# MaartenGr/PolyFuzz

Measured on NVIDIA H100. Metric: scored string pairs/sec (TF-IDF char-trigram top-10, top-k index bit-exact vs CPU ref), higher is better.
Workload: dtype f64

## Files before the change

include/pfz.h:

```cpp
#ifndef PFZ_H
#define PFZ_H
#include <stdint.h>
#ifdef __cplusplus
extern "C" {
#endif

#define PFZ_ABI_VERSION 1

#define PFZ_FLAG_CLEAN         1
#define PFZ_FLAG_REMOVE_SPACE  2

#define PFZ_METRIC_LEV       0
#define PFZ_METRIC_INDEL     1
#define PFZ_METRIC_NORM_LEV  2
#define PFZ_METRIC_RATIO     3
#define PFZ_METRIC_JARO      4
#define PFZ_METRIC_JARO_WINKLER 5
#define PFZ_METRIC_OSA       6
#define PFZ_METRIC_NORM_OSA  7
#define PFZ_METRIC_DL        8
#define PFZ_METRIC_NORM_DL   9

int         pfz_abi_version(void);
const char *pfz_last_error(void);
int64_t     pfz_launch_count(void);
int pfz_device_info(int32_t *sm_count, int32_t *smem_per_block_optin, int32_t *cc_major, int32_t *cc_minor);

int pfz_int_alu_probe(int32_t iters, uint32_t *scratch, int64_t *lane_ops_host, void *stream);


int pfz_alphabet_mark(const uint32_t *blob, int64_t n_chars, uint8_t *present, void *stream);

#define PFZ_WARP_ROW_SLOTS 256
#define PFZ_MAX_ROW_SLOTS  8192
int pfz_ngram_rows(const uint32_t *blob, const int64_t *offsets, int32_t n_rows,
                   int32_t ngram_lo, int32_t ngram_hi, int32_t flags,
                   const uint32_t *sym_table, uint32_t base,
                   const int64_t *occ_ptr, const int32_t *long_rows, int32_t n_long,
                   uint64_t *codes, int32_t *tf, int32_t *row_cnt, void *stream);

int pfz_df_dense(const uint64_t *codes, const int64_t *occ_ptr, const int32_t *row_cnt, int32_t n_rows,
                 int32_t *df_dense, void *stream);
int pfz_vocab_compact_dense(const int32_t *df_dense, int64_t code_space, uint64_t *vocab_keys, int32_t *df,
                            int32_t *rank_dense, int32_t *n_vocab_dev, void *ws, void *stream);

int pfz_gather_codes(const uint64_t *codes, const int64_t *occ_ptr, const int32_t *row_cnt, int32_t n_rows,
                     uint64_t *keys, int64_t *cursor_dev, void *stream);
int pfz_sort_u64(uint64_t *keys, int64_t n_pow2, void *stream);
int pfz_vocab_from_sorted(const uint64_t *sorted_keys, int64_t n_keys_cap, const int64_t *n_keys_dev,
                          uint64_t *vocab_keys, int32_t *df, int32_t *n_vocab_dev, void *ws, void *stream);

int pfz_idf_lookup(const int32_t *df, const int32_t *n_vocab_dev, int64_t cap, const double *table, int64_t n_table, double *idf, void *stream);

int pfz_tfidf_emit(const uint64_t *codes, const int32_t *tf, const int64_t *occ_ptr, const int32_t *row_cnt,
                   int32_t n_rows, const int32_t *rank_dense, const uint64_t *vocab_keys, int32_t n_vocab,
                   const double *idf, int32_t *indptr, int32_t *indices, double *data, void *ws, void *stream);

int64_t pfz_scan_ws_bytes(int64_t n);


#define PFZ_INDEX_BANK_ORDER   1
#define PFZ_INDEX_BANK_ORDER32 2
int pfz_index_build(const int32_t *indptr, const int32_t *indices, const double *data, int32_t n_rows,
                    int32_t n_vocab, int32_t tile, int32_t n_tiles, int32_t flags,
                    int32_t *seg, uint16_t *post_idx, double *post_val, float *post_val32 ,
                    float *term_maxw ,
                    void *ws, void *stream);

#define PFZ_K2_LIST  1
#define PFZ_K2_DENSE 2
#define PFZ_K2_DENSE32 3
int pfz_spcos_topk(const int32_t *a_indptr, const int32_t *a_indices, const double *a_data, int32_t n_from,
                   const int32_t *seg, const uint16_t *post_idx, const double *post_val,
                   const float *post_val32, const int32_t *b_indptr, const int32_t *b_indices, const double *b_data,
                   const float *term_maxw,
                   int32_t n_vocab, int32_t tile, int32_t n_tiles, int32_t n_to,
                   int32_t k, double min_similarity, int32_t self_match,
                   int64_t from_index_base, int64_t to_index_base, int32_t n_splits,
                   const double *excl_val, const int32_t *excl_idx,
                   int32_t *top_idx, double *top_val, int32_t *row_counter, int32_t variant, void *stream);

int64_t pfz_spcos_block_ws_bytes(int32_t n_from, int64_t nnz_cap_from, int32_t n_vocab, int32_t n_splits);
int64_t pfz_spcos_block_gcnt_offset(int32_t n_from, int64_t nnz_cap_from, int32_t n_vocab, int32_t n_splits);
int pfz_index_pack_q26(const uint16_t *post_idx, const double *post_val, const int32_t *nnz_dev, void *post_pk, void *stream);
int pfz_index_pack_q15(const uint16_t *post_idx, const double *post_val, const int32_t *nnz_dev, int32_t tile, void *post_pk, void *stream);
int pfz_spcos_topk_block(const int32_t *a_indptr, const int32_t *a_indices, const double *a_data, int32_t n_from, int64_t nnz_cap_from,
                         const int32_t *seg, const void *post_pk, const int32_t *b_indptr, const int32_t *b_indices, const double *b_data,
                         int32_t n_vocab, int32_t tile, int32_t n_tiles, int32_t n_to, int32_t k, double min_similarity, int32_t self_match,
                         int64_t from_index_base, int64_t to_index_base, int32_t n_splits, int32_t block_rows, int32_t acc_bits,
                         int32_t *top_idx, double *top_val, int32_t *err_flag_dev, void *ws, void *stream);

int pfz_spcos_topk_hash(const int32_t *a_indptr, const int32_t *a_indices, const double *a_data, int32_t n_from, const int32_t *seg,
                        const void *post_pk, const int32_t *b_indptr, const int32_t *b_indices, const double *b_data, int32_t tile,
                        int32_t n_tiles, int32_t n_to, int32_t k, double min_similarity, int32_t self_match, int64_t from_index_base,
                        int64_t to_index_base, int32_t n_splits, int32_t table_slots, const double *excl_val, const int32_t *excl_idx,
                        int32_t *top_idx, double *top_val, int32_t *row_counter, int32_t *err_flag_dev, void *stream);

int pfz_topk_merge(const int32_t *idx, const double *val, int32_t n_lists, int32_t n_from, int32_t k_in,
                   int32_t k_out, int32_t *out_idx, double *out_val, void *stream);


int pfz_lev_pack(const uint32_t *to_blob, const int64_t *to_offsets, const int32_t *order, int32_t n_to,
                 const uint8_t *sym_table, const int64_t *grp_word_off, uint32_t *packed, int32_t *slen, void *stream);

int pfz_lev_argbest(const uint32_t *from_blob, const int64_t *from_offsets, int32_t n_from, const int32_t *from_ids,
                    int32_t n_ids, int32_t n_words, const uint8_t *sym_table, const uint32_t *packed,
                    const int64_t *grp_word_off, const int32_t *slen, const int32_t *sorig, int32_t n_to,
                    int32_t metric, double score_cutoff, int32_t exclude_self, int64_t self_shift, int32_t n_splits,
                    int32_t *part_idx, double *part_score, int32_t *part_dist, int32_t *matrix, int64_t matrix_ld,
                    int32_t *counter, void *stream);
int pfz_lev_merge(const int32_t *part_idx, const double *part_score, const int32_t *part_dist, int32_t n_splits,
                  int32_t n_from, int32_t *best_idx, double *best_score, int32_t *best_dist, void *stream);

int pfz_lev_topk(const uint32_t *from_blob, const int64_t *from_offsets, int32_t n_from, const int32_t *from_ids,
                 int32_t n_ids, int32_t n_words, const uint8_t *sym_table, const uint32_t *packed,
                 const int64_t *grp_word_off, const int32_t *slen, const int32_t *sorig, int32_t n_to,
                 int32_t metric, double score_cutoff, int32_t exclude_self, int64_t self_shift, int32_t n_splits,
                 int32_t k, int32_t *part_idx, double *part_score, int32_t *counter, void *stream);

int pfz_dl_argbest(const uint32_t *from_blob, const int64_t *from_offsets, int32_t n_from, const int32_t *from_ids,
                   int32_t n_ids, int32_t n_words, const uint8_t *sym_table, const uint32_t *packed,
                   const int64_t *grp_word_off, const int32_t *slen, const int32_t *sorig, int32_t n_to,
                   int32_t metric, double score_cutoff, int32_t exclude_self, int64_t self_shift, int32_t n_splits,
                   int32_t *part_idx, double *part_score, int32_t *part_dist, int32_t *matrix, int64_t matrix_ld,
                   const double *gate, int32_t *counter, void *stream);
int pfz_dl_topk(const uint32_t *from_blob, const int64_t *from_offsets, int32_t n_from, const int32_t *from_ids,
                int32_t n_ids, int32_t n_words, const uint8_t *sym_table, const uint32_t *packed,
                const int64_t *grp_word_off, const int32_t *slen, const int32_t *sorig, int32_t n_to,
                int32_t metric, double score_cutoff, int32_t exclude_self, int64_t self_shift, int32_t n_splits,
                int32_t k, int32_t *part_idx, double *part_score, const double *gate, int32_t *counter, void *stream);

int pfz_fuzz_argbest(const void *const *ptrs, int32_t n_ptrs, int32_t n_from, int32_t n_ids, int32_t n_words, int32_t n_to,
                     int32_t scorer, double score_cutoff, int32_t exclude_self, int64_t self_shift, int32_t n_splits, void *stream);

int pfz_tok_side(const int32_t *blob, const int64_t *offsets, int32_t n, int64_t n_chars, int32_t *n_all, int32_t *vocab_blob,
                 int64_t *vocab_off, int32_t *tok_ptr, int32_t *tok_ids, int64_t *s_off, int32_t *s_blob, int64_t *u_off,
                 int32_t *u_blob, int64_t *counts_host, void *stream);
int pfz_tok_union(const int32_t *a_blob, const int64_t *a_off, int32_t n_a, const int32_t *b_blob, const int64_t *b_off, int32_t n_b,
                  int32_t *map_a, int32_t *map_b, int32_t *u_blob, int64_t *u_off, int32_t *n_u, void *stream);
int pfz_tok_remap(const int32_t *tok_ptr, const int32_t *ids_in, int32_t n, const int32_t *map, int32_t *ids_out, uint64_t *sig,
                  void *stream);

int pfz_fuzz_topk(const void *const *ptrs, int32_t n_ptrs, int32_t n_from, int32_t n_ids, int32_t n_words, int32_t n_to,
                  int32_t scorer, double score_cutoff, int32_t exclude_self, int64_t self_shift, int32_t n_splits, int32_t k,
                  void *stream);


int pfz_rows_to_bf16(const void *x, int32_t is_f64, int64_t ld, int32_t n_rows, int32_t d, int32_t d_pad,
                     int32_t normalize, void *out_bf16, void *stream);

int pfz_dense_cos_topk(const void *x_bf16, const void *y_bf16, int32_t n_from, int32_t n_to, int32_t d, int32_t k,
                       double min_similarity, int32_t self_match, int64_t from_index_base, int64_t to_index_base,
                       int32_t n_splits, int32_t *top_idx, double *top_val, void *stream);

int pfz_rows_prep_exact(const void *x, int32_t is_f64, int64_t ld, int32_t n_rows, int32_t d, int32_t d_pad,
                        double *out_f64, void *out_f16, double *norm16, double *err16, double *maxima, void *stream);

int pfz_dense_cos_topk_f16(const void *x_f16, const void *y_f16, int32_t n_from, int32_t n_to, int32_t d, int32_t k,
                           double min_similarity, int32_t self_match, int64_t from_index_base, int64_t to_index_base,
                           int32_t n_splits, int32_t *top_idx, double *top_val, void *stream);

int pfz_dense_exact_rescore(const double *x_f64, const double *y_f64, int32_t n_from, int32_t n_to, int32_t d_pad, int32_t k,
                            int32_t k_cand, const int32_t *cand_idx, const double *cand_val, const double *x_norm16,
                            const double *x_err16, const double *y_maxima, double min_similarity, int32_t self_match,
                            int64_t from_index_base, int64_t to_index_base, int32_t *top_idx, double *top_val,
                            int32_t *fb_rows, int32_t *fb_count, void *stream);

int64_t pfz_dense_exact_fallback_ws_bytes(int32_t n_from, int32_t n_to, int32_t k);
int pfz_dense_exact_fallback(const double *x_f64, const double *y_f64, int32_t n_from, int32_t n_to, int32_t d_pad, int32_t k,
                             double min_similarity, int32_t self_match, int64_t from_index_base, int64_t to_index_base,
                             const int32_t *fb_rows, const int32_t *fb_count, int32_t *top_idx, double *top_val, void *ws,
                             void *stream);

int pfz_dense_topn_bound(const int32_t *list_idx, const double *list_val, int32_t n_lists, int32_t n_from, int32_t k_list,
                         int32_t k, int32_t exact, const double *x_norm16, const double *x_err16, const double *y_maxima,
                         int32_t d_pad, double min_similarity, float *row_thr, void *stream);

int pfz_dense_cos_cand(const void *x_bf16, const void *y_bf16, int32_t n_from, int32_t n_to, int32_t d, double min_similarity,
                       const float *row_thr, int64_t to_index_base, int32_t n_splits, int32_t cap, int32_t *cand_idx,
                       double *cand_val, int32_t *cand_count, void *stream);
int pfz_dense_cos_cand_f16(const void *x_f16, const void *y_f16, int32_t n_from, int32_t n_to, int32_t d, double min_similarity,
                           const float *row_thr, int64_t to_index_base, int32_t n_splits, int32_t cap, int32_t *cand_idx,
                           double *cand_val, int32_t *cand_count, void *stream);

int pfz_dense_topn_exact_rescore(const double *x_f64, const double *y_f64, int32_t n_rows, int32_t d_pad, const int32_t *row_map,
                                 int64_t to_index_base, int32_t cap, const int32_t *cand_idx, double *cand_val,
                                 const int32_t *cand_count, void *stream);

int pfz_dense_topn_select(const int32_t *cand_idx, const double *cand_val, const int32_t *cand_count, int32_t n_rows, int32_t cap,
                          int32_t k, double min_similarity, int32_t self_match, int64_t from_index_base, const int32_t *row_map,
                          int32_t *top_idx, double *top_val, void *stream);

int pfz_frame_tail_count(const int32_t *top_idx, const double *top_val, int32_t n, int32_t k, const int64_t *to_offsets, double *sims,
                         int32_t *lens_pos, uint32_t *bitmap, void *ws, void *stream);
int pfz_frame_tail_copy(const int32_t *top_idx, int32_t n, int32_t k, const int32_t *to_blob, const int64_t *to_offsets, const int32_t *pos,
                        int64_t *offsets, uint8_t *data, void *stream);

#ifdef __cplusplus
}
#endif
#endif
```

polyfuzz_b200/_lib.py:

```python
import ctypes
import os

_HERE = os.path.dirname(os.path.abspath(__file__))
_LIB_PATH = os.path.join(_HERE, "libpfz.so")
_lib = None

c_i32, c_i64, c_u32, c_f64, c_vp = ctypes.c_int32, ctypes.c_int64, ctypes.c_uint32, ctypes.c_double, ctypes.c_void_p

_PROTOS = {
    "pfz_abi_version": [],
    "pfz_last_error": [],
    "pfz_launch_count": [],
    "pfz_device_info": [c_vp, c_vp, c_vp, c_vp],
    "pfz_scan_ws_bytes": [c_i64],
    "pfz_int_alu_probe": [c_i32, c_vp, c_vp, c_vp],
    "pfz_alphabet_mark": [c_vp, c_i64, c_vp, c_vp],
    "pfz_ngram_rows": [c_vp, c_vp, c_i32, c_i32, c_i32, c_i32, c_vp, c_u32, c_vp, c_vp, c_i32, c_vp, c_vp, c_vp, c_vp],
    "pfz_df_dense": [c_vp, c_vp, c_vp, c_i32, c_vp, c_vp],
    "pfz_vocab_compact_dense": [c_vp, c_i64, c_vp, c_vp, c_vp, c_vp, c_vp, c_vp],
    "pfz_gather_codes": [c_vp, c_vp, c_vp, c_i32, c_vp, c_vp, c_vp],
    "pfz_sort_u64": [c_vp, c_i64, c_vp],
    "pfz_vocab_from_sorted": [c_vp, c_i64, c_vp, c_vp, c_vp, c_vp, c_vp, c_vp],
    "pfz_idf_lookup": [c_vp, c_vp, c_i64, c_vp, c_i64, c_vp, c_vp],
    "pfz_tfidf_emit": [c_vp, c_vp, c_vp, c_vp, c_i32, c_vp, c_vp, c_i32, c_vp, c_vp, c_vp, c_vp, c_vp, c_vp],
    "pfz_index_build": [c_vp, c_vp, c_vp, c_i32, c_i32, c_i32, c_i32, c_i32, c_vp, c_vp, c_vp, c_vp, c_vp, c_vp, c_vp],
    "pfz_spcos_topk": [c_vp, c_vp, c_vp, c_i32, c_vp, c_vp, c_vp, c_vp, c_vp, c_vp, c_vp, c_vp, c_i32, c_i32, c_i32, c_i32, c_i32, c_f64, c_i32,
                       c_i64, c_i64, c_i32, c_vp, c_vp, c_vp, c_vp, c_vp, c_i32, c_vp],
    "pfz_topk_merge": [c_vp, c_vp, c_i32, c_i32, c_i32, c_i32, c_vp, c_vp, c_vp],
    "pfz_spcos_topk_hash": [c_vp, c_vp, c_vp, c_i32, c_vp, c_vp, c_vp, c_vp, c_vp, c_i32, c_i32, c_i32, c_i32, c_f64, c_i32, c_i64, c_i64, c_i32,
                            c_i32, c_vp, c_vp, c_vp, c_vp, c_vp, c_vp, c_vp],
    "pfz_spcos_block_ws_bytes": [c_i32, c_i64, c_i32, c_i32],
    "pfz_spcos_block_gcnt_offset": [c_i32, c_i64, c_i32, c_i32],
    "pfz_index_pack_q26": [c_vp, c_vp, c_vp, c_vp, c_vp],
    "pfz_index_pack_q15": [c_vp, c_vp, c_vp, c_i32, c_vp, c_vp],
    "pfz_spcos_topk_block": [c_vp, c_vp, c_vp, c_i32, c_i64, c_vp, c_vp, c_vp, c_vp, c_vp, c_i32, c_i32, c_i32, c_i32, c_i32, c_f64, c_i32,
                             c_i64, c_i64, c_i32, c_i32, c_i32, c_vp, c_vp, c_vp, c_vp, c_vp],
    "pfz_lev_pack": [c_vp, c_vp, c_vp, c_i32, c_vp, c_vp, c_vp, c_vp, c_vp],
    "pfz_lev_argbest": [c_vp, c_vp, c_i32, c_vp, c_i32, c_i32, c_vp, c_vp, c_vp, c_vp, c_vp, c_i32, c_i32, c_f64, c_i32, c_i64,
                        c_i32, c_vp, c_vp, c_vp, c_vp, c_i64, c_vp, c_vp],
    "pfz_lev_merge": [c_vp, c_vp, c_vp, c_i32, c_i32, c_vp, c_vp, c_vp, c_vp],
    "pfz_fuzz_argbest": [c_vp, c_i32, c_i32, c_i32, c_i32, c_i32, c_i32, c_f64, c_i32, c_i64, c_i32, c_vp],
    "pfz_lev_topk": [c_vp, c_vp, c_i32, c_vp, c_i32, c_i32, c_vp, c_vp, c_vp, c_vp, c_vp, c_i32, c_i32, c_f64, c_i32, c_i64,
                     c_i32, c_i32, c_vp, c_vp, c_vp, c_vp],
    "pfz_dl_argbest": [c_vp, c_vp, c_i32, c_vp, c_i32, c_i32, c_vp, c_vp, c_vp, c_vp, c_vp, c_i32, c_i32, c_f64, c_i32, c_i64,
                       c_i32, c_vp, c_vp, c_vp, c_vp, c_i64, c_vp, c_vp, c_vp],
    "pfz_dl_topk": [c_vp, c_vp, c_i32, c_vp, c_i32, c_i32, c_vp, c_vp, c_vp, c_vp, c_vp, c_i32, c_i32, c_f64, c_i32, c_i64,
                    c_i32, c_i32, c_vp, c_vp, c_vp, c_vp, c_vp],
    "pfz_fuzz_topk":[c_vp, c_i32, c_i32, c_i32, c_i32, c_i32, c_i32, c_f64, c_i32, c_i64, c_i32, c_i32, c_vp],
    "pfz_tok_side": [c_vp, c_vp, c_i32, c_i64, c_vp, c_vp, c_vp, c_vp, c_vp, c_vp, c_vp, c_vp, c_vp, c_vp, c_vp],
    "pfz_tok_union": [c_vp, c_vp, c_i32, c_vp, c_vp, c_i32, c_vp, c_vp, c_vp, c_vp, c_vp, c_vp],
    "pfz_tok_remap": [c_vp, c_vp, c_i32, c_vp, c_vp, c_vp, c_vp],
    "pfz_frame_tail_count": [c_vp, c_vp, c_i32, c_i32, c_vp, c_vp, c_vp, c_vp, c_vp, c_vp],
    "pfz_frame_tail_copy": [c_vp, c_i32, c_i32, c_vp, c_vp, c_vp, c_vp, c_vp, c_vp],
    "pfz_rows_to_bf16": [c_vp, c_i32, c_i64, c_i32, c_i32, c_i32, c_i32, c_vp, c_vp],
    "pfz_dense_cos_topk": [c_vp, c_vp, c_i32, c_i32, c_i32, c_i32, c_f64, c_i32, c_i64, c_i64, c_i32, c_vp, c_vp, c_vp],
    "pfz_rows_prep_exact": [c_vp, c_i32, c_i64, c_i32, c_i32, c_i32, c_vp, c_vp, c_vp, c_vp, c_vp, c_vp],
    "pfz_dense_cos_topk_f16": [c_vp, c_vp, c_i32, c_i32, c_i32, c_i32, c_f64, c_i32, c_i64, c_i64, c_i32, c_vp, c_vp, c_vp],
    "pfz_dense_exact_rescore": [c_vp, c_vp, c_i32, c_i32, c_i32, c_i32, c_i32, c_vp, c_vp, c_vp, c_vp, c_vp, c_f64, c_i32, c_i64, c_i64,
                                c_vp, c_vp, c_vp, c_vp, c_vp],
    "pfz_dense_exact_fallback_ws_bytes": [c_i32, c_i32, c_i32],
    "pfz_dense_exact_fallback": [c_vp, c_vp, c_i32, c_i32, c_i32, c_i32, c_f64, c_i32, c_i64, c_i64, c_vp, c_vp, c_vp, c_vp, c_vp, c_vp],
    "pfz_dense_topn_bound": [c_vp, c_vp, c_i32, c_i32, c_i32, c_i32, c_i32, c_vp, c_vp, c_vp, c_i32, c_f64, c_vp, c_vp],
    "pfz_dense_cos_cand": [c_vp, c_vp, c_i32, c_i32, c_i32, c_f64, c_vp, c_i64, c_i32, c_i32, c_vp, c_vp, c_vp, c_vp],
    "pfz_dense_cos_cand_f16": [c_vp, c_vp, c_i32, c_i32, c_i32, c_f64, c_vp, c_i64, c_i32, c_i32, c_vp, c_vp, c_vp, c_vp],
    "pfz_dense_topn_exact_rescore": [c_vp, c_vp, c_i32, c_i32, c_vp, c_i64, c_i32, c_vp, c_vp, c_vp, c_vp],
    "pfz_dense_topn_select": [c_vp, c_vp, c_vp, c_i32, c_i32, c_i32, c_f64, c_i32, c_i64, c_vp, c_vp, c_vp, c_vp],
}
_RESTYPES = {"pfz_last_error": ctypes.c_char_p, "pfz_scan_ws_bytes": c_i64, "pfz_launch_count": c_i64, "pfz_spcos_block_ws_bytes": c_i64,
             "pfz_spcos_block_gcnt_offset": c_i64,
             "pfz_dense_exact_fallback_ws_bytes": c_i64}


def exported_names():
    return list(_PROTOS)


def lib_path():
    return _LIB_PATH


def load():
    global _lib
    if _lib is not None:
        return _lib
    if not os.path.exists(_LIB_PATH):
        raise RuntimeError(f"{_LIB_PATH} not found: build it with `python -m polyfuzz_b200.build` "
                           "(polyfuzz_b200 has no CPU fallback)")
    lib = ctypes.CDLL(_LIB_PATH)
    for name, args in _PROTOS.items():
        fn = getattr(lib, name)
        fn.argtypes = args
        fn.restype = _RESTYPES.get(name, ctypes.c_int)
    _lib = lib
    return lib


def call(name, *args):
    lib = load()
    rc = getattr(lib, name)(*args)
    if rc != 0:
        raise RuntimeError(f"{name} failed: {lib.pfz_last_error().decode(errors='replace')}")


def launch_count():
    return int(load().pfz_launch_count())
```

polyfuzz_b200/csrc/pfz_core.cu:

```cuda
#include <stdarg.h>
#include "pfz_common.cuh"

namespace pfz {
static thread_local char g_err[1024] = "";
unsigned long long g_launches = 0;
void set_error(const char *fmt, ...) {
    va_list ap; va_start(ap, fmt);
    vsnprintf(g_err, sizeof(g_err), fmt, ap);
    va_end(ap);
}

constexpr int SCAN_THREADS = 512;
constexpr int SCAN_ITEMS = 8;
constexpr int SCAN_TILE = SCAN_THREADS * SCAN_ITEMS;

__global__ void __launch_bounds__(SCAN_THREADS) scan_tile_kernel(const int32_t *__restrict__ in, int32_t *__restrict__ out,
                                                               int64_t n, int32_t *__restrict__ sums) {
    __shared__ int32_t warp_tot[SCAN_THREADS / 32];
    const int64_t base = (int64_t)blockIdx.x * SCAN_TILE + (int64_t)threadIdx.x * SCAN_ITEMS;
    int32_t v[SCAN_ITEMS];
    int32_t tsum = 0;
#pragma unroll
    for (int i = 0; i < SCAN_ITEMS; ++i) {
        v[i] = (base + i < n) ? in[base + i] : 0;
        tsum += v[i];
    }
    int32_t incl = warp_incl_scan(tsum);
    const int lane = threadIdx.x & 31, w = threadIdx.x >> 5;
    if (lane == 31) warp_tot[w] = incl;
    __syncthreads();
    if (w == 0) {
        int32_t t = (lane < SCAN_THREADS / 32) ? warp_tot[lane] : 0;
        int32_t ti = warp_incl_scan(t);
        if (lane < SCAN_THREADS / 32) warp_tot[lane] = ti - t;
        if (lane == 31 && sums) sums[blockIdx.x] = ti;
    }
    __syncthreads();
    int32_t run = warp_tot[w] + incl - tsum;
#pragma unroll
    for (int i = 0; i < SCAN_ITEMS; ++i) {
        if (base + i < n) out[base + i] = run;
        run += v[i];
    }
}

__global__ void __launch_bounds__(SCAN_THREADS) scan_add_kernel(int32_t *__restrict__ out, int64_t n,
                                                              const int32_t *__restrict__ offs) {
    const int32_t add = offs[blockIdx.x];
    const int64_t base = (int64_t)blockIdx.x * SCAN_TILE + (int64_t)threadIdx.x * SCAN_ITEMS;
#pragma unroll
    for (int i = 0; i < SCAN_ITEMS; ++i)
        if (base + i < n) out[base + i] += add;
}

static int64_t n_tiles_of(int64_t n) { return (n + SCAN_TILE - 1) / SCAN_TILE; }

int scan_exclusive_i32(const int32_t *in, int32_t *out, int64_t n, void *ws, cudaStream_t st) {
    if (n <= 0) return 0;
    const int64_t nt = n_tiles_of(n);
    if (nt == 1) {
        scan_tile_kernel<<<1, SCAN_THREADS, 0, st>>>(in, out, n, nullptr);
        PFZ_LAUNCH_OK();
        return 0;
    }
    int32_t *sums = reinterpret_cast<int32_t *>(ws);
    char *next_ws = reinterpret_cast<char *>(ws) + ((nt * 4 + 255) / 256) * 256;
    scan_tile_kernel<<<(unsigned)nt, SCAN_THREADS, 0, st>>>(in, out, n, sums);
    PFZ_LAUNCH_OK();
    if (scan_exclusive_i32(sums, sums, nt, next_ws, st)) return 1;
    scan_add_kernel<<<(unsigned)nt, SCAN_THREADS, 0, st>>>(out, n, sums);
    PFZ_LAUNCH_OK();
    return 0;
}

__global__ void __launch_bounds__(256) int_alu_probe_kernel(uint32_t *__restrict__ out, int iters, uint32_t seed) {
    uint32_t a[8];
    const uint32_t b = seed ^ (threadIdx.x * 2654435761u), c = seed * 3u + blockIdx.x;
#pragma unroll
    for (int i = 0; i < 8; ++i) a[i] = b + i * 977u;
    for (int it = 0; it < iters; ++it) {
#pragma unroll
        for (int u = 0; u < 4; ++u) {
#pragma unroll
            for (int i = 0; i < 8; ++i) asm volatile("lop3.b32 %0, %0, %1, %2, 0x96;" : "+r"(a[i]) : "r"(b), "r"(c));
#pragma unroll
            for (int i = 0; i < 8; ++i) asm volatile("add.u32 %0, %0, %1;" : "+r"(a[i]) : "r"(c));
        }
    }
    uint32_t x = 0;
#pragma unroll
    for (int i = 0; i < 8; ++i) x ^= a[i];
    out[(size_t)blockIdx.x * blockDim.x + threadIdx.x] = x;
}
}

extern "C" {

int pfz_int_alu_probe(int32_t iters, uint32_t *scratch, int64_t *lane_ops_host, void *stream) {
    int dev = 0, sms = 0;
    PFZ_CUDA_OK(cudaGetDevice(&dev));
    PFZ_CUDA_OK(cudaDeviceGetAttribute(&sms, cudaDevAttrMultiProcessorCount, dev));
    const int blocks = sms * 8;
    pfz::int_alu_probe_kernel<<<blocks, 256, 0, pfz::as_stream(stream)>>>(scratch, iters, 12345u);
    PFZ_LAUNCH_OK();
    if (lane_ops_host) *lane_ops_host = (int64_t)blocks * 256 * (int64_t)iters * 64;
    return 0;
}

int pfz_abi_version(void) { return PFZ_ABI_VERSION; }
const char *pfz_last_error(void) { return pfz::g_err; }
int64_t pfz_launch_count(void) { return (int64_t)__atomic_load_n(&pfz::g_launches, __ATOMIC_RELAXED); }

int64_t pfz_scan_ws_bytes(int64_t n) {
    int64_t total = 256;
    while (n > pfz::SCAN_TILE) {
        n = pfz::n_tiles_of(n);
        total += ((n * 4 + 255) / 256) * 256;
    }
    return total;
}

int pfz_device_info(int32_t *sm_count, int32_t *smem_optin, int32_t *cc_major, int32_t *cc_minor) {
    int dev = 0;
    PFZ_CUDA_OK(cudaGetDevice(&dev));
    int v = 0;
    PFZ_CUDA_OK(cudaDeviceGetAttribute(&v, cudaDevAttrMultiProcessorCount, dev)); *sm_count = v;
    PFZ_CUDA_OK(cudaDeviceGetAttribute(&v, cudaDevAttrMaxSharedMemoryPerBlockOptin, dev)); *smem_optin = v;
    PFZ_CUDA_OK(cudaDeviceGetAttribute(&v, cudaDevAttrComputeCapabilityMajor, dev)); *cc_major = v;
    PFZ_CUDA_OK(cudaDeviceGetAttribute(&v, cudaDevAttrComputeCapabilityMinor, dev)); *cc_minor = v;
    return 0;
}
}
```

polyfuzz_b200/csrc/pfz_spcos.cu:

```cuda
#include <stdlib.h>
#include "pfz_common.cuh"

namespace pfz {

__global__ void index_count_kernel(const int32_t *__restrict__ indptr, const int32_t *__restrict__ indices, int n_rows, int tile, int n_tiles,
                                   int32_t *__restrict__ cnt) {
    const int lane = lane_id();
    const int gw = (blockIdx.x * blockDim.x + threadIdx.x) >> 5, nw = (gridDim.x * blockDim.x) >> 5;
    for (int r = gw; r < n_rows; r += nw) {
        const int tau = r / tile;
        for (int p = indptr[r] + lane; p < indptr[r + 1]; p += 32)
            atomicAdd(&cnt[(int64_t)indices[p] * n_tiles + tau], 1);
    }
}

__global__ void index_fill_kernel(const int32_t *__restrict__ indptr, const int32_t *__restrict__ indices, const double *__restrict__ data,
                                  int n_rows, int tile, int n_tiles, const int32_t *__restrict__ seg, int32_t *__restrict__ cur,
                                  uint16_t *__restrict__ post_idx, double *__restrict__ post_val, int *__restrict__ term_maxw_bits) {
    const int lane = lane_id();
    const int gw = (blockIdx.x * blockDim.x + threadIdx.x) >> 5, nw = (gridDim.x * blockDim.x) >> 5;
    for (int r = gw; r < n_rows; r += nw) {
        const int tau = r / tile;
        for (int p = indptr[r] + lane; p < indptr[r + 1]; p += 32) {
            const int64_t c = (int64_t)indices[p] * n_tiles + tau;
            const int pos = seg[c] + atomicAdd(&cur[c], 1);
            post_idx[pos] = (uint16_t)(r - tau * tile);
            post_val[pos] = data[p];
            if (term_maxw_bits) atomicMax(&term_maxw_bits[indices[p]], __float_as_int(__double2float_ru(data[p])));
        }
    }
}

constexpr int BANK_ORDER_MAX = 512;
template <int MOD>
__global__ void __launch_bounds__(128) index_bank_order_kernel(const int32_t *__restrict__ seg, int64_t ncell, uint16_t *__restrict__ post_idx,
                                                               double *__restrict__ post_val) {
    __shared__ uint16_t s_idx[4][BANK_ORDER_MAX];
    __shared__ uint16_t s_rank[4][BANK_ORDER_MAX];
    __shared__ double s_val[4][BANK_ORDER_MAX];
    __shared__ int s_cnt[4][MOD];
    const int lane = lane_id(), w = threadIdx.x >> 5;
    const int64_t gw = ((int64_t)blockIdx.x * blockDim.x + threadIdx.x) >> 5, nw = ((int64_t)gridDim.x * blockDim.x) >> 5;
    for (int64_t c0 = gw * 32; c0 < ncell; c0 += nw * 32) {
        int s = 0, len = 0;
        if (c0 + lane < ncell) { s = seg[c0 + lane]; len = seg[c0 + lane + 1] - s; }
        unsigned todo = __ballot_sync(FULL, len > MOD && len <= BANK_ORDER_MAX);
        while (todo) {
            const int src = __ffs(todo) - 1; todo &= todo - 1;
            const int cs = __shfl_sync(FULL, s, src), cl = __shfl_sync(FULL, len, src);
            if (lane < MOD) s_cnt[w][lane] = 0;
            __syncwarp();
            for (int q = lane; q < cl; q += 32) {
                const uint16_t j = post_idx[cs + q];
                s_idx[w][q] = j; s_val[w][q] = post_val[cs + q];
                s_rank[w][q] = (uint16_t)atomicAdd(&s_cnt[w][j & (MOD - 1)], 1);
            }
            __syncwarp();
            int cnt[MOD];
#pragma unroll
            for (int r = 0; r < MOD; ++r) cnt[r] = s_cnt[w][r];
            for (int q = lane; q < cl; q += 32) {
                const int r = s_idx[w][q] & (MOD - 1), i = s_rank[w][q];
                int pos = 0;
#pragma unroll
                for (int r2 = 0; r2 < MOD; ++r2) pos += min(cnt[r2], i) + ((r2 < r && cnt[r2] > i) ? 1 : 0);
                post_idx[cs + pos] = s_idx[w][q];
                post_val[cs + pos] = s_val[w][q];
            }
            __syncwarp();
        }
    }
}

__global__ void to_f32_kernel(const double *__restrict__ x, int64_t n_minus, const int32_t *__restrict__ n_ptr, float *__restrict__ y) {
    const int64_t n = n_ptr ? (int64_t)*n_ptr : n_minus;
    for (int64_t i = (int64_t)blockIdx.x * blockDim.x + threadIdx.x; i < n; i += (int64_t)gridDim.x * blockDim.x) y[i] = (float)x[i];
}

__device__ __forceinline__ bool key_before(double sa, int ia, double sb, int ib) {
    return (sa > sb) || (sa == sb && ia < ib);
}

struct SpcosParams {
    const int32_t *a_indptr; const int32_t *a_indices; const double *a_data; int n_from;
    const int32_t *seg; const uint16_t *post_idx; const double *post_val;
    const float *post_val32; const int32_t *b_indptr; const int32_t *b_indices; const double *b_data;
    const float *term_maxw; float prune_alpha;
    int n_vocab, tile, n_tiles, n_to;
    int k; double min_sim; int self_match; int64_t from_base, to_base;
    int n_splits; const double *excl_val; const int32_t *excl_idx;
    int32_t *top_idx; double *top_val; int32_t *row_counter;
};

template <int WARPS>
__global__ void __launch_bounds__(WARPS * 32) spcos_list_kernel(const SpcosParams P) {
    extern __shared__ __align__(16) unsigned char dyn[];
    const int lane = lane_id();
    const int w = threadIdx.x >> 5;
    const unsigned lt = (1u << lane) - 1u;
    double *acc = reinterpret_cast<double *>(dyn) + (size_t)w * P.tile;
    uint16_t *touched = reinterpret_cast<uint16_t *>(dyn + (size_t)WARPS * P.tile * 8) + (size_t)w * P.tile;
    for (int q = lane; q < P.tile; q += 32) acc[q] = 0.0;
    __syncwarp();

    const int split = blockIdx.y;
    const int tiles_per = (P.n_tiles + P.n_splits - 1) / P.n_splits;
    const int tau_lo = split * tiles_per;
    const int tau_hi = min(P.n_tiles, tau_lo + tiles_per);
    int32_t *counter = P.row_counter + split;

    for (;;) {
        int i = 0;
        if (lane == 0) i = atomicAdd(counter, 1);
        i = __shfl_sync(FULL, i, 0);
        if (i >= P.n_from) break;

        const int a0 = P.a_indptr[i];
        const int m = P.a_indptr[i + 1] - a0;
        double tv = P.min_sim; int ti = -1;
        double kv = P.min_sim; int ki = -1;
        double xv = 0.0; int xi = -1; bool has_x = false;
        if (P.excl_val) { xv = P.excl_val[i]; xi = P.excl_idx[i]; has_x = xi >= 0; }
        const int64_t self_j = P.from_base + i - P.to_base;

        for (int tau = tau_lo; tau < tau_hi; ++tau) {
            int ntouched = 0;
            for (int tb = 0; tb < m; tb += 32) {
                const int kk = tb + lane;
                int s = 0, len = 0; double v = 0.0;
                if (kk < m) {
                    const int t = P.a_indices[a0 + kk];
                    v = P.a_data[a0 + kk];
                    const int64_t c = (int64_t)t * P.n_tiles + tau;
                    s = P.seg[c];
                    len = P.seg[c + 1] - s;
                }
                unsigned live = __ballot_sync(FULL, len > 0);
                while (live) {
                    const int src = __ffs(live) - 1; live &= live - 1;
                    const int ss = __shfl_sync(FULL, s, src);
                    const int sl = __shfl_sync(FULL, len, src);
                    const double sv = shfl_d(v, src);
                    for (int c0 = 0; c0 < sl; c0 += 32) {
                        const int q = c0 + lane;
                        bool first = false; int jl = 0;
                        if (q < sl) {
                            jl = P.post_idx[ss + q];
                            const double prod = __dmul_rn(sv, P.post_val[ss + q]);
                            const double old = acc[jl];
                            acc[jl] = __dadd_rn(old, prod);
                            first = (old == 0.0);
                        }
                        const unsigned fm = __ballot_sync(FULL, first);
                        if (first) touched[ntouched + __popc(fm & lt)] = (uint16_t)jl;
                        ntouched += __popc(fm);
                    }
                    __syncwarp();
                }
            }
            for (int c0 = 0; c0 < ntouched; c0 += 32) {
                const int q = c0 + lane;
                double sc = 0.0; int j = -1; bool cand = false;
                if (q < ntouched) {
                    const int jl = touched[q];
                    sc = acc[jl];
                    acc[jl] = 0.0;
                    const int jloc = tau * P.tile + jl;
                    j = (int)(P.to_base + jloc);
                    cand = key_before(sc, j, kv, ki);
                    if (P.self_match && (int64_t)jloc == self_j) cand = false;
                    if (has_x && !key_before(xv, xi, sc, j)) cand = false;
                }
                unsigned cm = __ballot_sync(FULL, cand);
                while (cm) {
                    const int src = __ffs(cm) - 1; cm &= cm - 1;
                    const double cs = shfl_d(sc, src);
                    const int cj = __shfl_sync(FULL, j, src);
                    if (!key_before(cs, cj, kv, ki)) continue;
                    const bool stays = (lane < P.k) && key_before(tv, ti, cs, cj);
                    const int pos = __popc(__ballot_sync(FULL, stays));
                    const double uv = __shfl_up_sync(FULL, tv, 1);
                    const int ui = __shfl_up_sync(FULL, ti, 1);
                    if (lane > pos) { tv = uv; ti = ui; }
                    else if (lane == pos) { tv = cs; ti = cj; }
                    kv = shfl_d(tv, P.k - 1);
                    ki = __shfl_sync(FULL, ti, P.k - 1);
                }
            }
            __syncwarp();
        }
        if (lane < P.k) {
            const size_t o = ((size_t)split * P.n_from + i) * P.k + lane;
            P.top_idx[o] = ti;
            P.top_val[o] = (ti >= 0) ? tv : 0.0;
        }
    }
}


struct __align__(16) WorkItem { int off; int cnt; double v; };

__device__ __forceinline__ unsigned smem_u32(const void *p) { return (unsigned)__cvta_generic_to_shared(p); }
__device__ __forceinline__ void lds_item(unsigned a, unsigned &off, int &cnt, double &v) {
    unsigned lo, hi;
    asm volatile("ld.shared.v4.b32 {%0, %1, %2, %3}, [%4];" : "=r"(off), "=r"(cnt), "=r"(lo), "=r"(hi) : "r"(a) : "memory");
    v = __hiloint2double((int)hi, (int)lo);
}
__device__ __forceinline__ void ldg_posting(const uint16_t *pi, const double *pv, int lane, int cnt, unsigned dummy, unsigned &jl, double &w) {
    asm volatile("{ .reg .pred p; setp.lt.s32 p, %2, %3; mov.u32 %0, %4; mov.f64 %1, 0d0000000000000000;\n\t"
                 "@p ld.global.nc.u16 %0, [%5]; @p ld.global.nc.f64 %1, [%6]; }"
                 : "=&r"(jl), "=&d"(w) : "r"(lane), "r"(cnt), "r"(dummy), "l"(pi), "l"(pv) : "memory");
}
__device__ __forceinline__ void rmw_posting(unsigned acc_s, unsigned flags_s, unsigned row, unsigned dummy, double v, double w, double thr,
                                            unsigned &any) {
    asm volatile("{ .reg .pred p, q, r; .reg .f64 o, n, pr; .reg .b16 one; .reg .u32 a, f;\n\t"
                 "setp.ne.u32 p, %3, %4; mov.f64 o, 0d0000000000000000;\n\t"
                 "shl.b32 a, %3, 3; add.u32 a, a, %1; add.u32 f, %2, %3;\n\t"
                 "@p ld.shared.f64 o, [a];\n\t"
                 "mul.rn.f64 pr, %5, %6; add.rn.f64 n, o, pr;\n\t"
                 "@p st.shared.f64 [a], n;\n\t"
                 "setp.gt.f64 q, o, %7; setp.gt.and.f64 r, n, %7, !q; mov.b16 one, 1;\n\t"
                 "@r st.shared.u8 [f], one; selp.u32 %0, 1, %0, r; }"
                 : "+r"(any) : "r"(acc_s), "r"(flags_s), "r"(row), "r"(dummy), "d"(v), "d"(w), "d"(thr) : "memory");
}
// ... 258 lines not shown
                                    if (lane > pos) lv = up; else if (lane == pos) lv = ca;
                                    kth = __shfl_sync(FULL, lv, K - 1);
                                    a = (lane == src) ? -2.f : a;
                                    cm = __ballot_sync(FULL, a > kth);
                                }
                            }
                        }
                        gate = fmaxf(gate, float_floor(fmax((double)kth - K2_MARGIN - (double)ub_ne, 0.0)));
                    }
                }
                for (int w00 = 0; w00 < T; w00 += 512) {
                  uint4 fb = make_uint4(0u, 0u, 0u, 0u);
                  const int q16 = w00 + lane * 16;
                  if (q16 < T) {
                      fb = *reinterpret_cast<const uint4 *>(flags + q16);
                      if (fb.x | fb.y | fb.z | fb.w) *reinterpret_cast<uint4 *>(flags + q16) = make_uint4(0u, 0u, 0u, 0u);
                  }
                  if (!__any_sync(FULL, (fb.x | fb.y | fb.z | fb.w) != 0u)) continue;
#pragma unroll
                  for (int wsel = 0; wsel < 4; ++wsel) {
                    unsigned bits = wsel == 0 ? fb.x : wsel == 1 ? fb.y : wsel == 2 ? fb.z : fb.w;
                    const int q4 = q16 + wsel * 4;
                    while (__ballot_sync(FULL, bits != 0u)) {
                        if (APPROX) {
                            bool take = false; int jloc = 0;
                            if (bits) {
                                const int b8 = (__ffs(bits) - 1) >> 3; bits &= ~(0xffu << (b8 * 8));
                                const int jl = q4 + b8;
                                jloc = tau * T + jl;
                                take = reinterpret_cast<const float *>(acc)[jl] > gate;
                            }
                            const unsigned tm = __ballot_sync(FULL, take);
                            if (take) cand[ncand + __popc(tm & ((1u << lane) - 1u))] = jloc;
                            ncand += __popc(tm);
                            __syncwarp();
                            if (ncand >= 32) {
                                score_round(32);
                                __syncwarp();
                                const int rest = ncand - 32;
                                int mv = 0;
                                if (lane < rest) mv = cand[32 + lane];
                                __syncwarp();
                                if (lane < rest) cand[lane] = mv;
                                ncand = rest;
                                __syncwarp();
                            }
                            continue;
                        }
                        double sc = 0.0; int j = -1; bool cnd = false;
                        if (bits) {
                            const int b8 = (__ffs(bits) - 1) >> 3; bits &= ~(0xffu << (b8 * 8));
                            const int jl = q4 + b8;
                            const int jloc = tau * T + jl;
                            sc = acc[jl];
                            j = (int)(P.to_base + jloc);
                            cnd = key_before(sc, j, kv, ki);
                            if (P.self_match && (int64_t)jloc == self_j) cnd = false;
                            if (has_x && !key_before(xv, xi, sc, j)) cnd = false;
                        }
                        unsigned cm = __ballot_sync(FULL, cnd);
                        while (cm) {
                            const int src = __ffs(cm) - 1;
                            const double cs = shfl_d(sc, src);
                            const int cjx = __shfl_sync(FULL, j, src);
                            const bool stays = (lane < K) && key_before(tv, ti, cs, cjx);
                            const int pos = __popc(__ballot_sync(FULL, stays));
                            const double uv = __shfl_up_sync(FULL, tv, 1);
                            const int ui = __shfl_up_sync(FULL, ti, 1);
                            if (lane > pos) { tv = uv; ti = ui; }
                            else if (lane == pos) { tv = cs; ti = cjx; }
                            kv = shfl_d(tv, K - 1);
                            ki = __shfl_sync(FULL, ti, K - 1);
                            cnd = cnd && lane != src && key_before(sc, j, kv, ki);
                            cm = __ballot_sync(FULL, cnd);
                        }
                    }
                  }
                }
                thr = (ki >= 0) ? __longlong_as_double(__double_as_longlong(kv) - 1) : fmax(kv, 0.0);
            }
            __syncwarp();
            {
                double2 *a2 = reinterpret_cast<double2 *>(acc);
                const double2 z = make_double2(0.0, 0.0);
                for (int q = lane; q < (T * ES >> 4); q += 32) a2[q] = z;
            }
            __syncwarp();
        }
        if (APPROX && ncand > 0) { __syncwarp(); score_round(ncand); __syncwarp(); }
        if (lane < K) {
            const size_t o = ((size_t)split * P.n_from + i) * K + lane;
            P.top_idx[o] = ti;
            P.top_val[o] = (ti >= 0) ? tv : 0.0;
        }
    }
}

__global__ void __launch_bounds__(256) topk_merge_kernel(const int32_t *__restrict__ idx, const double *__restrict__ val, int n_lists, int n_from,
                                                         int k_in, int k_out, int32_t *__restrict__ out_idx, double *__restrict__ out_val) {
    const int lane = lane_id();
    const int gw = (blockIdx.x * blockDim.x + threadIdx.x) >> 5, nw = (gridDim.x * blockDim.x) >> 5;
    for (int i = gw; i < n_from; i += nw) {
        double tv = 0.0; int ti = -1;
        double kv = 0.0; int ki = -1; bool full = false;
        int filled = 0;
        for (int l = 0; l < n_lists; ++l) {
            const size_t b = ((size_t)l * n_from + i) * k_in;
            for (int c0 = 0; c0 < k_in; c0 += 32) {
                const int q = c0 + lane;
                double sc = 0.0; int j = -1;
                if (q < k_in) { j = idx[b + q]; sc = val[b + q]; }
                unsigned cm = __ballot_sync(FULL, j >= 0);
                while (cm) {
                    const int src = __ffs(cm) - 1; cm &= cm - 1;
                    const double cs = shfl_d(sc, src);
                    const int cj = __shfl_sync(FULL, j, src);
                    if (full && !key_before(cs, cj, kv, ki)) continue;
                    const bool stays = (lane < filled) && key_before(tv, ti, cs, cj);
                    const int pos = __popc(__ballot_sync(FULL, stays));
                    const double uv = __shfl_up_sync(FULL, tv, 1);
                    const int ui = __shfl_up_sync(FULL, ti, 1);
                    if (lane > pos) { tv = uv; ti = ui; }
                    else if (lane == pos) { tv = cs; ti = cj; }
                    if (filled < k_out) ++filled;
                    full = filled == k_out;
                    kv = shfl_d(tv, k_out - 1);
                    ki = __shfl_sync(FULL, ti, k_out - 1);
                }
            }
        }
        if (lane < k_out) {
            const bool ok = lane < filled;
            out_idx[(size_t)i * k_out + lane] = ok ? ti : -1;
            out_val[(size_t)i * k_out + lane] = ok ? tv : 0.0;
        }
    }
}

static int grid_for2(int64_t work_items, int threads, int cap) {
    int64_t g = (work_items + threads - 1) / threads;
    if (g < 1) g = 1;
    if (g > cap) g = cap;
    return (int)g;
}

}

using namespace pfz;

extern "C" {

int pfz_index_build(const int32_t *indptr, const int32_t *indices, const double *data, int32_t n_rows, int32_t n_vocab, int32_t tile,
                    int32_t n_tiles, int32_t flags, int32_t *seg, uint16_t *post_idx, double *post_val, float *post_val32, float *term_maxw,
                    void *ws, void *stream) {
    PFZ_REQUIRE(tile > 0 && tile <= 65536, "pfz_index_build: tile %d out of range (1..65536)", tile);
    PFZ_REQUIRE((int64_t)n_tiles * tile >= n_rows, "pfz_index_build: n_tiles*tile < n_rows");
    const int64_t ncell = (int64_t)n_vocab * n_tiles;
    PFZ_REQUIRE(ncell + 1 < (1ll << 31), "pfz_index_build: n_vocab*n_tiles = %lld too large", (long long)ncell);
    cudaStream_t st = as_stream(stream);
    int32_t *cur = reinterpret_cast<int32_t *>(ws);
    void *sws = reinterpret_cast<char *>(ws) + ((((size_t)ncell + 1) * 4 + 255) / 256) * 256;
    PFZ_CUDA_OK(cudaMemsetAsync(seg, 0, ((size_t)ncell + 1) * 4, st));
    if (n_rows > 0) {
        index_count_kernel<<<grid_for2((int64_t)n_rows * 32, 256, SM_COUNT * 16), 256, 0, st>>>(indptr, indices, n_rows, tile, n_tiles, seg);
        PFZ_LAUNCH_OK();
    }
    if (scan_exclusive_i32(seg, seg, ncell + 1, sws, st)) return 1;
    if (n_rows > 0) {
        PFZ_CUDA_OK(cudaMemsetAsync(cur, 0, ((size_t)ncell + 1) * 4, st));
        if (term_maxw) PFZ_CUDA_OK(cudaMemsetAsync(term_maxw, 0, (size_t)n_vocab * 4, st));
        index_fill_kernel<<<grid_for2((int64_t)n_rows * 32, 256, SM_COUNT * 16), 256, 0, st>>>(indptr, indices, data, n_rows, tile, n_tiles, seg, cur,
                                                                                            post_idx, post_val, reinterpret_cast<int *>(term_maxw));
        PFZ_LAUNCH_OK();
        if (flags & PFZ_INDEX_BANK_ORDER32) {
            index_bank_order_kernel<32><<<grid_for2(ncell, 128, SM_COUNT * 16), 128, 0, st>>>(seg, ncell, post_idx, post_val);
            PFZ_LAUNCH_OK();
        } else if (flags & PFZ_INDEX_BANK_ORDER) {
            index_bank_order_kernel<16><<<grid_for2(ncell, 128, SM_COUNT * 16), 128, 0, st>>>(seg, ncell, post_idx, post_val);
            PFZ_LAUNCH_OK();
        }
        if (post_val32) {
            to_f32_kernel<<<SM_COUNT * 8, 256, 0, st>>>(post_val, 0, seg + ncell, post_val32);
            PFZ_LAUNCH_OK();
        }
    }
    return 0;
}

int pfz_spcos_topk(const int32_t *a_indptr, const int32_t *a_indices, const double *a_data, int32_t n_from, const int32_t *seg,
                   const uint16_t *post_idx, const double *post_val, const float *post_val32, const int32_t *b_indptr,
                   const int32_t *b_indices, const double *b_data, const float *term_maxw, int32_t n_vocab, int32_t tile, int32_t n_tiles, int32_t n_to, int32_t k,
                   double min_similarity, int32_t self_match, int64_t from_index_base, int64_t to_index_base, int32_t n_splits,
                   const double *excl_val, const int32_t *excl_idx, int32_t *top_idx, double *top_val, int32_t *row_counter,
                   int32_t variant, void *stream) {
    PFZ_REQUIRE(k >= 1 && k <= 32, "pfz_spcos_topk: k=%d unsupported (1..32 per call; page with excl_* for more)", k);
    PFZ_REQUIRE(tile > 0 && tile <= 65536 && (tile % 64) == 0, "pfz_spcos_topk: tile %d must be a multiple of 64 in 64..65536", tile);
    PFZ_REQUIRE(n_splits >= 1 && n_splits <= n_tiles, "pfz_spcos_topk: n_splits %d out of range", n_splits);
    PFZ_REQUIRE(variant == PFZ_K2_LIST || variant == PFZ_K2_DENSE || variant == PFZ_K2_DENSE32, "pfz_spcos_topk: unknown variant %d", variant);
    PFZ_REQUIRE(variant != PFZ_K2_DENSE32 || (post_val32 && b_indptr && b_indices && b_data),
                "pfz_spcos_topk: PFZ_K2_DENSE32 needs post_val32 and the to-matrix CSR");
    if (n_from <= 0) return 0;
    cudaStream_t st = as_stream(stream);
    int dev = 0, sms = 0, smem_max = 0;
    PFZ_CUDA_OK(cudaGetDevice(&dev));
    PFZ_CUDA_OK(cudaDeviceGetAttribute(&sms, cudaDevAttrMultiProcessorCount, dev));
    PFZ_CUDA_OK(cudaDeviceGetAttribute(&smem_max, cudaDevAttrMaxSharedMemoryPerBlockOptin, dev));
    PFZ_CUDA_OK(cudaMemsetAsync(row_counter, 0, sizeof(int32_t) * (size_t)n_splits, st));
    const char *env_a = getenv("PFZ_K2_PRUNE_ALPHA");
    const float prune_alpha = env_a ? (float)atof(env_a) : 0.0f;
    SpcosParams P{a_indptr, a_indices, a_data, n_from, seg, post_idx, post_val, post_val32, b_indptr, b_indices, b_data, term_maxw, prune_alpha,
                  n_vocab, tile, n_tiles, n_to, k, min_similarity, self_match,
                  from_index_base, to_index_base, n_splits, excl_val, excl_idx, top_idx, top_val, row_counter};
    auto launch = [&](auto kernel, int warps, size_t smem) -> int {
        PFZ_REQUIRE(smem <= (size_t)smem_max, "pfz_spcos_topk: tile %d needs %zu B shared memory > %d available", tile, smem, smem_max);
        PFZ_CUDA_OK(cudaFuncSetAttribute(kernel, cudaFuncAttributeMaxDynamicSharedMemorySize, (int)smem));
        int occ = 0;
        PFZ_CUDA_OK(cudaOccupancyMaxActiveBlocksPerMultiprocessor(&occ, kernel, warps * 32, smem));
        if (occ < 1) occ = 1;
        int gx = sms * occ;
        const int need = (n_from + warps - 1) / warps;
        if (gx > need) gx = need;
        if (n_splits > 1) { gx = (gx + n_splits - 1) / n_splits; if (gx < 1) gx = 1; }
        kernel<<<dim3(gx, n_splits), warps * 32, smem, st>>>(P);
        PFZ_LAUNCH_OK();
        return 0;
    };
    if (variant == PFZ_K2_LIST) {
        constexpr int WARPS = 8;
        return launch(spcos_list_kernel<WARPS>, WARPS, (size_t)WARPS * tile * 10);
    }
    constexpr int WARPS = 2;
    const int es = variant == PFZ_K2_DENSE32 ? 4 : 8;
    auto arena_of = [&](int D) { return (((size_t)(tile + 4) * es + (size_t)((tile >> 5) + 32 + 2 * D) * sizeof(WorkItem) + (size_t)tile + 16 + 256) + 15) & ~(size_t)15; };
    const char *env_d = getenv("PFZ_K2_DEPTH");
    const int depth = env_d ? atoi(env_d) : 4;
    if (variant == PFZ_K2_DENSE32) {
        if (prune_alpha > 0.f && term_maxw) return launch(spcos_dense_kernel<WARPS, 4, true, true>, WARPS, (size_t)WARPS * arena_of(4));
        if (depth == 8) return launch(spcos_dense_kernel<WARPS, 8, true, false>, WARPS, (size_t)WARPS * arena_of(8));
        if (depth == 6) return launch(spcos_dense_kernel<WARPS, 6, true, false>, WARPS, (size_t)WARPS * arena_of(6));
        if (depth == 3) return launch(spcos_dense_kernel<WARPS, 3, true, false>, WARPS, (size_t)WARPS * arena_of(3));
        if (depth == 2) return launch(spcos_dense_kernel<WARPS, 2, true, false>, WARPS, (size_t)WARPS * arena_of(2));
        return launch(spcos_dense_kernel<WARPS, 4, true, false>, WARPS, (size_t)WARPS * arena_of(4));
    }
    if (depth == 8) return launch(spcos_dense_kernel<WARPS, 8, false, false>, WARPS, (size_t)WARPS * arena_of(8));
    return launch(spcos_dense_kernel<WARPS, 4, false, false>, WARPS, (size_t)WARPS * arena_of(4));
}

int pfz_topk_merge(const int32_t *idx, const double *val, int32_t n_lists, int32_t n_from, int32_t k_in, int32_t k_out, int32_t *out_idx,
                   double *out_val, void *stream) {
    PFZ_REQUIRE(k_out >= 1 && k_out <= 32, "pfz_topk_merge: k_out=%d unsupported (1..32)", k_out);
    PFZ_REQUIRE(n_lists >= 1 && k_in >= 1, "pfz_topk_merge: bad n_lists/k_in");
    if (n_from <= 0) return 0;
    topk_merge_kernel<<<grid_for2((int64_t)n_from * 32, 256, SM_COUNT * 16), 256, 0, as_stream(stream)>>>(idx, val, n_lists, n_from, k_in, k_out, out_idx, out_val);
    PFZ_LAUNCH_OK();
    return 0;
}
}
```

polyfuzz_b200/csrc/pfz_spcos_block.cu:

```cuda
#include <stdlib.h>
#include "pfz_common.cuh"

namespace pfz {

constexpr double K2B_SCALE = 67108864.0;
constexpr unsigned K2B_MARGIN_Q = 672u;
constexpr int RANK_CAP = 16383;

struct __align__(16) BlockDesc { int pos0; int nrows; int base; int nterms; };

__global__ void blk_term_key_kernel(const int32_t *__restrict__ seg, int n_vocab, int n_tiles, uint64_t *__restrict__ keys, int64_t n_pad) {
    for (int64_t t = (int64_t)blockIdx.x * blockDim.x + threadIdx.x; t < n_pad; t += (int64_t)gridDim.x * blockDim.x) {
        uint64_t k = ~0ull;
        if (t < n_vocab) {
            const uint32_t df = (uint32_t)(seg[(t + 1) * n_tiles] - seg[t * n_tiles]);
            k = ((uint64_t)(0xffffffffu - df) << 32) | (uint32_t)t;
        }
        keys[t] = k;
    }
}
__global__ void blk_term_rank_kernel(const uint64_t *__restrict__ keys, int n_vocab, int32_t *__restrict__ rank) {
    for (int i = blockIdx.x * blockDim.x + threadIdx.x; i < n_vocab; i += gridDim.x * blockDim.x)
        rank[(uint32_t)(keys[i] & 0xffffffffu)] = min(i, RANK_CAP);
}
__global__ void blk_row_key_kernel(const int32_t *__restrict__ indptr, const int32_t *__restrict__ indices, const int32_t *__restrict__ rank,
                                   int n_from, uint64_t *__restrict__ keys, int64_t n_pad) {
    for (int64_t r = (int64_t)blockIdx.x * blockDim.x + threadIdx.x; r < n_pad; r += (int64_t)gridDim.x * blockDim.x) {
        uint64_t k = ~0ull;
        if (r < n_from) {
            int r1 = RANK_CAP, r2 = RANK_CAP, r3 = RANK_CAP;
            for (int p = indptr[r]; p < indptr[r + 1]; ++p) {
                const int x = rank[indices[p]];
                if (x < r1) { r3 = r2; r2 = r1; r1 = x; }
                else if (x < r2) { r3 = r2; r2 = x; }
                else if (x < r3) r3 = x;
            }
            k = ((uint64_t)r1 << 50) | ((uint64_t)r2 << 36) | ((uint64_t)r3 << 22) | (uint64_t)r;
        }
        keys[r] = k;
    }
}
__global__ void blk_perm_kernel(const uint64_t *__restrict__ keys, const int32_t *__restrict__ indptr, int n_from, int32_t *__restrict__ perm,
                                int32_t *__restrict__ nnz_perm) {
    for (int p = blockIdx.x * blockDim.x + threadIdx.x; p <= n_from; p += gridDim.x * blockDim.x) {
        if (p == n_from) { nnz_perm[p] = 0; continue; }
        const int r = (int)(keys[p] & 0x3fffffull);
        perm[p] = r;
        nnz_perm[p] = indptr[r + 1] - indptr[r];
    }
}

template <int BF>
__global__ void __launch_bounds__(128) blk_table_kernel(const int32_t *__restrict__ indptr, const int32_t *__restrict__ indices,
                                                        const double *__restrict__ data, int n_from, const int32_t *__restrict__ perm,
                                                        const int32_t *__restrict__ pos_ptr, int row_stride_bytes, int32_t *__restrict__ blk_terms,
                                                        int32_t *__restrict__ blk_fvdesc, uint2 *__restrict__ blk_fv, BlockDesc *__restrict__ descs,
                                                        int n_groups, int32_t *__restrict__ err_flag) {
    constexpr int FV_CAP = BF * 64;
    constexpr int WPB = BF == 16 ? 2 : 4;
    __shared__ uint32_t s_key[WPB][FV_CAP];
    __shared__ uint32_t s_val[WPB][FV_CAP];
    const int lane = lane_id(), w = threadIdx.x >> 5;
    const unsigned lt = (1u << lane) - 1u;
    if (w >= WPB) return;
    uint32_t *keys = s_key[w]; uint32_t *vals = s_val[w];
    for (int g = blockIdx.x * WPB + w; g < n_groups; g += gridDim.x * WPB) {
        const int p0 = g * BF, p1 = min(n_from, p0 + BF);
        const int total = pos_ptr[p1] - pos_ptr[p0];
        const int nsub = total <= FV_CAP ? 1 : 2;
        for (int sub = 0; sub < 2; ++sub) {
            BlockDesc d; d.pos0 = 0; d.nrows = 0; d.base = 0; d.nterms = 0;
            if (sub < nsub) {
                const int q0 = nsub == 1 ? p0 : min(p1, p0 + sub * (BF / 2));
                const int q1 = nsub == 1 ? p1 : min(p1, q0 + BF / 2);
                const int base = pos_ptr[q0];
                const int cnt = pos_ptr[q1] - base;
                if (cnt > FV_CAP) { if (lane == 0) atomicExch(err_flag, 1); }
                else if (q1 > q0) {
                    for (int f = 0; f < q1 - q0; ++f) {
                        const int row = perm[q0 + f];
                        const int a0 = indptr[row], m = indptr[row + 1] - a0, o = pos_ptr[q0 + f] - base;
                        for (int e = lane; e < m; e += 32) {
                            keys[o + e] = ((uint32_t)indices[a0 + e] << 4) | (uint32_t)f;
                            const double x = floor(data[a0 + e] * 4294967296.0);
                            vals[o + e] = x >= 4294967295.0 ? 0xffffffffu : (uint32_t)(unsigned long long)x;
                        }
                    }
                    int P = 1;
                    while (P < cnt) P <<= 1;
                    for (int e = cnt + lane; e < P; e += 32) { keys[e] = 0xffffffffu; vals[e] = 0u; }
                    __syncwarp();
                    for (int k = 2; k <= P; k <<= 1) {
                        for (int j = k >> 1; j > 0; j >>= 1) {
                            for (int t = lane; t < (P >> 1); t += 32) {
                                const int i = ((t & ~(j - 1)) << 1) | (t & (j - 1));
                                const int ix = i | j;
                                const uint32_t a = keys[i], b = keys[ix];
                                const bool up = (i & k) == 0;
                                if ((a > b) == up) { keys[i] = b; keys[ix] = a; const uint32_t va = vals[i]; vals[i] = vals[ix]; vals[ix] = va; }
                            }
                            __syncwarp();
                        }
                    }
                    int nd = 0;
                    for (int e0 = 0; e0 < cnt; e0 += 32) {
                        const int e = e0 + lane;
                        bool head = false; uint32_t term = 0;
                        if (e < cnt) {
                            const uint32_t key = keys[e];
                            term = key >> 4;
                            head = (e == 0) || (keys[e - 1] >> 4) != term;
                            blk_fv[base + e] = make_uint2((key & 15u) * (uint32_t)row_stride_bytes, vals[e]);
                        }
                        const unsigned hm = __ballot_sync(FULL, head);
                        if (head) {
                            int len = 1;
                            while (e + len < cnt && (keys[e + len] >> 4) == term) ++len;
                            const int u = nd + __popc(hm & lt);
                            blk_terms[base + u] = (int32_t)term;
                            blk_fvdesc[base + u] = (e << 5) | len;
                        }
                        nd += __popc(hm);
                    }
                    d.pos0 = q0; d.nrows = q1 - q0; d.base = base; d.nterms = nd;
                    __syncwarp();
                }
            }
            if (lane == 0) descs[2 * g + sub] = d;
        }
    }
}

__global__ void blk_pack_kernel(const uint16_t *__restrict__ post_idx, const double *__restrict__ post_val, const int32_t *__restrict__ nnz_ptr,
                                uint2 *__restrict__ post_pk) {
    const int64_t n = *nnz_ptr;
    for (int64_t i = (int64_t)blockIdx.x * blockDim.x + threadIdx.x; i < n; i += (int64_t)gridDim.x * blockDim.x)
        post_pk[i] = make_uint2((uint32_t)post_idx[i], (uint32_t)__double2ll_rn(post_val[i] * 67108864.0));
}

__global__ void blk_pack15_kernel(const uint16_t *__restrict__ post_idx, const double *__restrict__ post_val, const int32_t *__restrict__ nnz_ptr,
                                  int half_tile, uint2 *__restrict__ post_pk) {
    const int64_t n = *nnz_ptr;
    for (int64_t i = (int64_t)blockIdx.x * blockDim.x + threadIdx.x; i < n; i += (int64_t)gridDim.x * blockDim.x) {
        const uint32_t j = post_idx[i];
        const bool hi = j >= (uint32_t)half_tile;
        const uint32_t w15 = (uint32_t)max(1ll, __double2ll_rn(post_val[i] * 32768.0));
        post_pk[i] = make_uint2(((hi ? j - (uint32_t)half_tile : j) << 2) | ((hi ? 0x3244u : 0x4432u) << 16), w15);
    }
}

struct BlockParams {
    const int32_t *a_indptr; const int32_t *a_indices; const double *a_data; int n_from;
    const int32_t *perm; const BlockDesc *descs; int n_desc;
    const int32_t *blk_terms; const int32_t *blk_fvdesc; const uint2 *blk_fv;
    const int32_t *seg; const uint2 *post_pk;
    const int32_t *b_indptr; const int32_t *b_indices; const double *b_data;
    int tile, n_tiles, n_to, k; double min_sim; int self_match; int64_t from_base, to_base; int n_splits;
    int32_t *top_idx; double *top_val; int32_t *counter;
    int32_t *glist; int32_t *gcnt; int gcap;
};

__device__ __forceinline__ unsigned sm_u32(const void *p) { return (unsigned)__cvta_generic_to_shared(p); }
__device__ __forceinline__ void red_add_u32(unsigned a, unsigned v) {
    asm volatile("red.shared.add.u32 [%0], %1;" :: "r"(a), "r"(v));
}
__device__ __forceinline__ bool blk_key_before(double sa, int ia, double sb, int ib) { return (sa > sb) || (sa == sb && ia < ib); }
__device__ __noinline__ double blk_exact_dot(const int32_t *__restrict__ ai, const double *__restrict__ av, int an,
                                  const int32_t *__restrict__ bi, const double *__restrict__ bv, int bn) {
    double s = 0.0;
    int p = 0;
    for (int c0 = 0; c0 < bn && p < an; c0 += 32) {
        int ci[32]; double cv[32];
        const int nc = min(32, bn - c0);
#pragma unroll 8
        for (int q = 0; q < nc; ++q) { ci[q] = bi[c0 + q]; cv[q] = bv[c0 + q]; }
#pragma unroll 1
        for (int q = 0; q < nc; ++q) {
            const int cb = ci[q];
            while (p < an && ai[p] < cb) ++p;
            if (p < an && ai[p] == cb) { s = __dadd_rn(s, __dmul_rn(av[p], cv[q])); ++p; }
        }
    }
    return s;
}
__device__ __forceinline__ unsigned warp_sort_desc_u32(unsigned x, int lane) {
#pragma unroll
    for (int k = 2; k <= 32; k <<= 1) {
#pragma unroll
        for (int j = k >> 1; j > 0; j >>= 1) {
            const unsigned o = __shfl_xor_sync(FULL, x, j);
            const bool keep_max = ((lane & j) == 0) == ((lane & k) == 0);
            x = keep_max ? max(x, o) : min(x, o);
        }
    }
    return x;
}

#ifndef PFZ_B3_ICAP_PER_ROW
#define PFZ_B3_ICAP_PER_ROW 64
#endif
#ifndef PFZ_B3_MIN_CTAS
#define PFZ_B3_MIN_CTAS(BF) (16 / (BF))
#endif
constexpr int B3_ICAP_PER_ROW = PFZ_B3_ICAP_PER_ROW;
constexpr int B3_QCAP = 128;
#ifndef PFZ_B3_DEPTH
#define PFZ_B3_DEPTH 3
#endif
constexpr int B3_DEPTH = PFZ_B3_DEPTH;

struct __align__(16) B3Item { int off; int cnt; unsigned fva; int nf; };
struct __align__(16) B3Ctx {
    const int32_t *a_indptr; const int32_t *a_indices; const double *a_data;
    const int32_t *b_indptr; const int32_t *b_indices; const double *b_data;
    int64_t to_base; double scale; int K; int T; int TW; int gcap;
    int32_t *glist; int64_t grow0;
};
struct __align__(16) B3Row {
    double tv[32]; int ti[32];
    unsigned av[32];
    int cand[B3_QCAP];
    int row, self_loc, ncand; unsigned thr, akth, MQ, gate; int gcount;
};

__device__ __forceinline__ void blk_exact_rounds(const int32_t *__restrict__ a_indptr, const int32_t *__restrict__ a_indices, const double *__restrict__ a_data,
                                                 const int32_t *__restrict__ b_indptr, const int32_t *__restrict__ b_indices, const double *__restrict__ b_data,
                                                 int64_t to_base, int K, int row, int self_loc, const int *cand, int ncand, double &tv, int &ti, double &kv, int &ki) {
    const int lane = threadIdx.x & 31;
    const int a0 = a_indptr[row], m = a_indptr[row + 1] - a0;
    kv = shfl_d(tv, K - 1); ki = __shfl_sync(FULL, ti, K - 1);
    while (ncand > 0) {
        const int n_round = min(32, ncand), off = ncand - n_round;
        double sc = 0.0; int j = -1; bool cnd = false;
        if (lane < n_round) {
            const int jloc = cand[off + lane];
            const int b0 = b_indptr[jloc];
            sc = blk_exact_dot(a_indices + a0, a_data + a0, m, b_indices + b0, b_data + b0, b_indptr[jloc + 1] - b0);
            j = (int)(to_base + jloc);
            cnd = blk_key_before(sc, j, kv, ki) && jloc != self_loc;
        }
        unsigned cm = __ballot_sync(FULL, cnd);
        while (cm) {
            const int src = __ffs(cm) - 1;
            const double cs = shfl_d(sc, src);
            const int cj = __shfl_sync(FULL, j, src);
            const bool stays = (lane < K) && blk_key_before(tv, ti, cs, cj);
            const int pos = __popc(__ballot_sync(FULL, stays));
            const double uv = __shfl_up_sync(FULL, tv, 1);
            const int ui = __shfl_up_sync(FULL, ti, 1);
            if (lane > pos) { tv = uv; ti = ui; }
            else if (lane == pos) { tv = cs; ti = cj; }
            kv = shfl_d(tv, K - 1);
            ki = __shfl_sync(FULL, ti, K - 1);
            cnd = cnd && lane != src && blk_key_before(sc, j, kv, ki);
            cm = __ballot_sync(FULL, cnd);
        }
        ncand = off;
    }
}
__device__ __noinline__ void blk3_drain(const B3Ctx *cx, B3Row *rs) {
    const int lane = threadIdx.x & 31;
    double tv = rs->tv[lane]; int ti = rs->ti[lane];
    double kv; int ki;
    blk_exact_rounds(cx->a_indptr, cx->a_indices, cx->a_data, cx->b_indptr, cx->b_indices, cx->b_data, cx->to_base, cx->K, rs->row, rs->self_loc,
                     rs->cand, rs->ncand, tv, ti, kv, ki);
    rs->tv[lane] = tv; rs->ti[lane] = ti;
    if (lane == 0) {
        rs->ncand = 0;
        if (ki >= 0) {
            const double y = kv * cx->scale - (double)rs->MQ;
            const unsigned t = y <= 0.0 ? 0u : (unsigned)__double2ll_rd(y);
            if (t > rs->thr) rs->thr = t;
        }
    }
    __syncwarp();
}
__device__ __noinline__ void blk3_flush(const B3Ctx *cx, B3Row *rs) {
    const int lane = threadIdx.x & 31;
    const int ncand = rs->ncand, g = rs->gcount;
    if (g + ncand <= cx->gcap) {
        int32_t *dst = cx->glist + (size_t)(cx->grow0 + rs->row) * cx->gcap + g;
        for (int q = lane; q < ncand; q += 32) dst[q] = rs->cand[q];
        __syncwarp();
        if (lane == 0) { rs->gcount = g + ncand; rs->ncand = 0; }
        __syncwarp();
    } else blk3_drain(cx, rs);
}

template <bool P16>
__device__ __forceinline__ unsigned blk3_wmax(const uint4 &v) {
    if (!P16) return max(max(v.x, v.y), max(v.z, v.w));
    const unsigned m2 = __vmaxu2(__vmaxu2(v.x, v.y), __vmaxu2(v.z, v.w));
    return max(m2 & 0xffffu, m2 >> 16);
}

__device__ __forceinline__ uint4 lds128(unsigned a) {
    uint4 v;
    asm volatile("ld.shared.v4.u32 {%0, %1, %2, %3}, [%4];" : "=r"(v.x), "=r"(v.y), "=r"(v.z), "=r"(v.w) : "r"(a));
    return v;
}
__device__ __forceinline__ void sts128_zero(unsigned a) {
    asm volatile("st.shared.v4.u32 [%0], {%1, %1, %1, %1};" :: "r"(a), "r"(0u));
}
// ... 322 lines not shown
                    const int sb = P.blk_terms[D.base + u] * n_tiles + tau;
                    const unsigned fvd = (unsigned)P.blk_fvdesc[D.base + u];
                    const int s = seg[sb], len = seg[sb + 1] - s;
                    for (int c = 0; c < len; c += 32) {
                        uint2 pk = make_uint2(0u, 0u);
                        if (lane < len - c) pk = __ldg(pk_lane + s + c);
                        blk3_process<P16>(lane, len - c, fv_s + ((fvd >> 5) << 3), (int)(fvd & 31u), pk, acc_s, dump_s);
                    }
                }
            }
            B3_TICK(2);
            __syncthreads();
            B3_TICK(3);
            if (has_row) {
                if (stau == tau) {
                    if (lane == 0) {
                        const int sjl = rs->self_loc - stau * T;
                        if (P16) acc[(size_t)w * RW + (sjl >= TW ? sjl - TW : sjl)] &= (sjl >= TW ? 0x0000ffffu : 0xffff0000u);
                        else acc[(size_t)w * RW + sjl] = 0u;
                    }
                    __syncwarp();
                }
                blk3_scan_row<P16>(cx, rs, acc_s + (unsigned)(w * RW) * 4u, tau * T);
            }
        }
        B3_TICK(4);
        if (has_row) {
            __syncwarp();
            blk3_flush(cx, rs);
            const size_t ro = (size_t)split * P.n_from + rs->row;
            if (lane < P.k) {
                const int ti = rs->ti[lane];
                P.top_idx[ro * P.k + lane] = ti;
                P.top_val[ro * P.k + lane] = (ti >= 0) ? rs->tv[lane] : 0.0;
            }
            if (lane == 0) P.gcnt[ro] = rs->gcount;
        }
        B3_TICK(5);
        __syncthreads();
        B3_TICK(6);
    }
}

struct ExactParams {
    const int32_t *a_indptr; const int32_t *a_indices; const double *a_data;
    const int32_t *b_indptr; const int32_t *b_indices; const double *b_data;
    const int32_t *glist; const int32_t *gcnt; int gcap; int n_from; int n_splits; int n_to; int k; double min_sim; int self_match;
    int64_t from_base, to_base; int32_t *top_idx; double *top_val;
};
constexpr int EX_ROW_CAP = 128;
constexpr int EX_HASH = 2 * EX_ROW_CAP;
__device__ __forceinline__ unsigned ex_slot(int t) { return ((unsigned)t * 0x9E3779B1u) >> 24; }
constexpr int EX_CHUNK = 8;
__global__ void __launch_bounds__(256) blk_exact_kernel(const ExactParams P) {
    static_assert(EX_HASH == 256, "ex_slot() yields 8 bits");
    __shared__ int s_hk[8][EX_HASH];
    __shared__ double s_hv[8][EX_HASH];
    const int lane = threadIdx.x & 31, wl = threadIdx.x >> 5;
    const int64_t gw = (int64_t)blockIdx.x * 8 + wl;
    if (gw >= (int64_t)P.n_splits * P.n_from) return;
    const int n = P.gcnt[gw];
    if (n == 0) return;
    const int row = (int)(gw % P.n_from), K = P.k;
    const int64_t self_j = P.from_base + row - P.to_base;
    const int self_loc = (P.self_match && self_j >= 0 && self_j < (int64_t)P.n_to) ? (int)self_j : -1;
    double tv = P.min_sim; int ti = -1;
    if (lane < K) { ti = P.top_idx[gw * K + lane]; if (ti >= 0) tv = P.top_val[gw * K + lane]; }
    double kv; int ki;
    const int a0 = P.a_indptr[row], m = P.a_indptr[row + 1] - a0;
    const int32_t *cand = P.glist + (size_t)gw * P.gcap;
    if (m > EX_ROW_CAP) {
        blk_exact_rounds(P.a_indptr, P.a_indices, P.a_data, P.b_indptr, P.b_indices, P.b_data, P.to_base, K, row, self_loc, cand, n, tv, ti, kv, ki);
    } else {
        int *hk = s_hk[wl]; double *hv = s_hv[wl];
        for (int s2 = lane; s2 < EX_HASH; s2 += 32) hk[s2] = -1;
        __syncwarp();
        for (int e = lane; e < m; e += 32) {
            const int t = P.a_indices[a0 + e];
            const double x = P.a_data[a0 + e];
            unsigned sl = ex_slot(t);
            while (atomicCAS(&hk[sl], -1, t) != -1) sl = (sl + 1) & (EX_HASH - 1);
            hv[sl] = x;
        }
        __syncwarp();
        kv = shfl_d(tv, K - 1); ki = __shfl_sync(FULL, ti, K - 1);
        int left = n;
        while (left > 0) {
            const int n_round = min(32, left), off = left - n_round;
            double sc = 0.0; int j = -1; bool cnd = false;
            if (lane < n_round) {
                const int jloc = cand[off + lane];
                const int b0 = P.b_indptr[jloc], b1 = P.b_indptr[jloc + 1];
                for (int q = b0; q < b1; q += EX_CHUNK) {
                    int t[EX_CHUNK]; double wgt[EX_CHUNK];
#pragma unroll
                    for (int u = 0; u < EX_CHUNK; ++u) { t[u] = -1; wgt[u] = 0.0; if (q + u < b1) { t[u] = P.b_indices[q + u]; wgt[u] = P.b_data[q + u]; } }
#pragma unroll
                    for (int u = 0; u < EX_CHUNK; ++u) {
                        if (t[u] < 0) break;
                        unsigned sl = ex_slot(t[u]);
                        int k;
                        while ((k = hk[sl]) != t[u] && k != -1) sl = (sl + 1) & (EX_HASH - 1);
                        if (k == t[u]) sc = __dadd_rn(sc, __dmul_rn(hv[sl], wgt[u]));
                    }
                }
                j = (int)(P.to_base + jloc);
                cnd = blk_key_before(sc, j, kv, ki) && jloc != self_loc;
            }
            unsigned cm = __ballot_sync(FULL, cnd);
            while (cm) {
                const int src = __ffs(cm) - 1;
                const double cs = shfl_d(sc, src);
                const int cj = __shfl_sync(FULL, j, src);
                const bool stays = (lane < K) && blk_key_before(tv, ti, cs, cj);
                const int pos = __popc(__ballot_sync(FULL, stays));
                const double uv = __shfl_up_sync(FULL, tv, 1);
                const int ui = __shfl_up_sync(FULL, ti, 1);
                if (lane > pos) { tv = uv; ti = ui; }
                else if (lane == pos) { tv = cs; ti = cj; }
                kv = shfl_d(tv, K - 1);
                ki = __shfl_sync(FULL, ti, K - 1);
                cnd = cnd && lane != src && blk_key_before(sc, j, kv, ki);
                cm = __ballot_sync(FULL, cnd);
            }
            left = off;
        }
    }
    if (lane < K) { P.top_idx[gw * K + lane] = ti; P.top_val[gw * K + lane] = (ti >= 0) ? tv : 0.0; }
}

template <int BF, bool P16>
static int launch_blk3(const BlockParams &P, int n_groups, int sms, int smem_max, cudaStream_t st) {
    size_t arena = (blk3_arena_bytes<BF, P16>(P.tile) + 15) & ~(size_t)15;
    { const char *e = getenv("PFZ_BLOCK_PAD_SMEM"); if (e) arena += (size_t)atoi(e); }
    PFZ_REQUIRE(arena <= (size_t)smem_max, "pfz_spcos_topk_block: tile %d x %d rows needs %zu B shared memory > %d available", P.tile, BF, arena, smem_max);
    PFZ_CUDA_OK(cudaFuncSetAttribute(spcos_blk3_kernel<BF, P16>, cudaFuncAttributeMaxDynamicSharedMemorySize, (int)arena));
    int occ = 0;
    PFZ_CUDA_OK(cudaOccupancyMaxActiveBlocksPerMultiprocessor(&occ, spcos_blk3_kernel<BF, P16>, BF * 32, arena));
    if (occ < 1) occ = 1;
    int gx = sms * occ;
    if (gx > 2 * n_groups) gx = 2 * n_groups;
    if (P.n_splits > 1) { gx = (gx + P.n_splits - 1) / P.n_splits; if (gx < 1) gx = 1; }
    spcos_blk3_kernel<BF, P16><<<dim3(gx, P.n_splits), BF * 32, arena, st>>>(P);
    PFZ_LAUNCH_OK();
    return 0;
}

static int blk_grid(int64_t work, int threads, int cap) {
    int64_t g = (work + threads - 1) / threads;
    if (g < 1) g = 1;
    if (g > cap) g = cap;
    return (int)g;
}
static int64_t pow2_at_least(int64_t n) { int64_t p = 2; while (p < n) p <<= 1; return p; }
static size_t align256(size_t x) { return (x + 255) & ~(size_t)255; }

struct BlockWs {
    size_t term_keys, term_rank, row_keys, perm, pos_ptr, scan_ws, blk_terms, blk_fvdesc, blk_fv, descs, counters, gcnt, glist, total;
};
constexpr int B3_GCAP = 192;
static BlockWs block_ws_layout(int64_t n_from, int64_t nnz_cap, int64_t n_vocab, int n_splits) {
    BlockWs L; size_t o = 0;
    const int64_t vp = pow2_at_least(n_vocab), np = pow2_at_least(n_from);
    const int64_t n_groups = (n_from + 3) / 4;
    L.term_keys = o; o += align256((size_t)vp * 8);
    L.term_rank = o; o += align256((size_t)(n_vocab + 1) * 4);
    L.row_keys = o; o += align256((size_t)np * 8);
    L.perm = o; o += align256((size_t)(n_from + 1) * 4);
    L.pos_ptr = o; o += align256((size_t)(n_from + 2) * 4);
    L.scan_ws = o; o += align256((size_t)pfz_scan_ws_bytes(n_from + 2));
    L.blk_terms = o; o += align256((size_t)(nnz_cap + 1) * 4);
    L.blk_fvdesc = o; o += align256((size_t)(nnz_cap + 1) * 4);
    L.blk_fv = o; o += align256((size_t)(nnz_cap + 1) * 8);
    L.descs = o; o += align256((size_t)(2 * n_groups + 1) * sizeof(BlockDesc));
    L.counters = o; o += align256((size_t)(n_splits + 1) * 4);
    L.gcnt = o; o += align256((size_t)n_splits * (size_t)n_from * 4);
    L.glist = o; o += align256((size_t)n_splits * (size_t)n_from * B3_GCAP * 4);
    L.total = o;
    return L;
}

}

using namespace pfz;

extern "C" {

int64_t pfz_spcos_block_ws_bytes(int32_t n_from, int64_t nnz_cap_from, int32_t n_vocab, int32_t n_splits) {
    return (int64_t)block_ws_layout(n_from, nnz_cap_from, n_vocab, n_splits).total;
}

int64_t pfz_spcos_block_gcnt_offset(int32_t n_from, int64_t nnz_cap_from, int32_t n_vocab, int32_t n_splits) {
    return (int64_t)block_ws_layout(n_from, nnz_cap_from, n_vocab, n_splits).gcnt;
}

int pfz_index_pack_q26(const uint16_t *post_idx, const double *post_val, const int32_t *nnz_dev, void *post_pk, void *stream) {
    blk_pack_kernel<<<SM_COUNT * 8, 256, 0, as_stream(stream)>>>(post_idx, post_val, nnz_dev, reinterpret_cast<uint2 *>(post_pk));
    PFZ_LAUNCH_OK();
    return 0;
}

int pfz_index_pack_q15(const uint16_t *post_idx, const double *post_val, const int32_t *nnz_dev, int32_t tile, void *post_pk, void *stream) {
    PFZ_REQUIRE(tile >= 256 && tile <= 8192 && (tile % 256) == 0, "pfz_index_pack_q15: tile %d must be a multiple of 256 in 256..8192", tile);
    blk_pack15_kernel<<<SM_COUNT * 8, 256, 0, as_stream(stream)>>>(post_idx, post_val, nnz_dev, tile / 2, reinterpret_cast<uint2 *>(post_pk));
    PFZ_LAUNCH_OK();
    return 0;
}

int pfz_spcos_topk_block(const int32_t *a_indptr, const int32_t *a_indices, const double *a_data, int32_t n_from, int64_t nnz_cap_from,
                         const int32_t *seg, const void *post_pk, const int32_t *b_indptr, const int32_t *b_indices, const double *b_data,
                         int32_t n_vocab, int32_t tile, int32_t n_tiles, int32_t n_to, int32_t k, double min_similarity, int32_t self_match,
                         int64_t from_index_base, int64_t to_index_base, int32_t n_splits, int32_t block_rows, int32_t acc_bits, int32_t *top_idx,
                         double *top_val, int32_t *err_flag_dev, void *ws, void *stream) {
    PFZ_REQUIRE(k >= 1 && k <= 32, "pfz_spcos_topk_block: k=%d unsupported (1..32)", k);
    PFZ_REQUIRE(tile >= 128 && tile <= 4096 && (tile % 128) == 0, "pfz_spcos_topk_block: tile %d must be a multiple of 128 in 128..4096", tile);
    PFZ_REQUIRE(block_rows == 4 || block_rows == 8 || block_rows == 16, "pfz_spcos_topk_block: block_rows %d must be 4, 8 or 16", block_rows);
    PFZ_REQUIRE(acc_bits == 32 || (acc_bits == 16 && tile % 256 == 0), "pfz_spcos_topk_block: acc_bits %d must be 32, or 16 with a tile that is a multiple of 256", acc_bits);
    PFZ_REQUIRE(n_splits >= 1 && n_splits <= n_tiles, "pfz_spcos_topk_block: n_splits %d out of range", n_splits);
    PFZ_REQUIRE(n_from < (1 << 22), "pfz_spcos_topk_block: n_from %d exceeds the 22-bit row id of the clustering key", n_from);
    PFZ_REQUIRE(n_vocab < (1 << 28), "pfz_spcos_topk_block: n_vocab too large");
    if (n_from <= 0) return 0;
    cudaStream_t st = as_stream(stream);
    int dev = 0, sms = 0, smem_max = 0;
    PFZ_CUDA_OK(cudaGetDevice(&dev));
    PFZ_CUDA_OK(cudaDeviceGetAttribute(&sms, cudaDevAttrMultiProcessorCount, dev));
    PFZ_CUDA_OK(cudaDeviceGetAttribute(&smem_max, cudaDevAttrMaxSharedMemoryPerBlockOptin, dev));
    const BlockWs L = block_ws_layout(n_from, nnz_cap_from, n_vocab, n_splits);
    char *w = reinterpret_cast<char *>(ws);
    uint64_t *term_keys = reinterpret_cast<uint64_t *>(w + L.term_keys);
    int32_t *term_rank = reinterpret_cast<int32_t *>(w + L.term_rank);
    uint64_t *row_keys = reinterpret_cast<uint64_t *>(w + L.row_keys);
    int32_t *perm = reinterpret_cast<int32_t *>(w + L.perm);
    int32_t *pos_ptr = reinterpret_cast<int32_t *>(w + L.pos_ptr);
    int32_t *blk_terms = reinterpret_cast<int32_t *>(w + L.blk_terms);
    int32_t *blk_fvdesc = reinterpret_cast<int32_t *>(w + L.blk_fvdesc);
    uint2 *blk_fv = reinterpret_cast<uint2 *>(w + L.blk_fv);
    BlockDesc *descs = reinterpret_cast<BlockDesc *>(w + L.descs);
    int32_t *counters = reinterpret_cast<int32_t *>(w + L.counters);
    const int64_t vp = pow2_at_least(n_vocab), np = pow2_at_least(n_from);
    const int n_groups = (n_from + block_rows - 1) / block_rows;

    blk_term_key_kernel<<<blk_grid(vp, 256, SM_COUNT * 8), 256, 0, st>>>(seg, n_vocab, n_tiles, term_keys, vp);
    PFZ_LAUNCH_OK();
    if (pfz_sort_u64(term_keys, vp, stream)) return 1;
    blk_term_rank_kernel<<<blk_grid(n_vocab, 256, SM_COUNT * 8), 256, 0, st>>>(term_keys, n_vocab, term_rank);
    PFZ_LAUNCH_OK();
    blk_row_key_kernel<<<blk_grid(np, 256, SM_COUNT * 16), 256, 0, st>>>(a_indptr, a_indices, term_rank, n_from, row_keys, np);
    PFZ_LAUNCH_OK();
    if (pfz_sort_u64(row_keys, np, stream)) return 1;
    blk_perm_kernel<<<blk_grid(n_from + 1, 256, SM_COUNT * 16), 256, 0, st>>>(row_keys, a_indptr, n_from, perm, pos_ptr);
    PFZ_LAUNCH_OK();
    if (scan_exclusive_i32(pos_ptr, pos_ptr, (int64_t)n_from + 1, w + L.scan_ws, st)) return 1;
    const int row_stride = tile * (acc_bits == 16 ? 2 : 4) + 128;
    if (block_rows == 4)
        blk_table_kernel<4><<<blk_grid((int64_t)n_groups * 32, 128, SM_COUNT * 16), 128, 0, st>>>(a_indptr, a_indices, a_data, n_from, perm, pos_ptr, row_stride,
                                                                                             blk_terms, blk_fvdesc, blk_fv, descs, n_groups, err_flag_dev);
    else if (block_rows == 8)
        blk_table_kernel<8><<<blk_grid((int64_t)n_groups * 32, 128, SM_COUNT * 16), 128, 0, st>>>(a_indptr, a_indices, a_data, n_from, perm, pos_ptr, row_stride,
                                                                                             blk_terms, blk_fvdesc, blk_fv, descs, n_groups, err_flag_dev);
    else
        blk_table_kernel<16><<<blk_grid((int64_t)n_groups * 32, 64, SM_COUNT * 16), 128, 0, st>>>(a_indptr, a_indices, a_data, n_from, perm, pos_ptr, row_stride,
                                                                                              blk_terms, blk_fvdesc, blk_fv, descs, n_groups, err_flag_dev);
    PFZ_LAUNCH_OK();
    PFZ_CUDA_OK(cudaMemsetAsync(counters, 0, sizeof(int32_t) * (size_t)n_splits, st));
    BlockParams P{a_indptr, a_indices, a_data, n_from, perm, descs, 2 * n_groups, blk_terms, blk_fvdesc, blk_fv, seg,
                  reinterpret_cast<const uint2 *>(post_pk), b_indptr, b_indices, b_data, tile, n_tiles, n_to, k, min_similarity, self_match,
                  from_index_base, to_index_base, n_splits, top_idx, top_val, counters,
                  reinterpret_cast<int32_t *>(w + L.glist), reinterpret_cast<int32_t *>(w + L.gcnt), B3_GCAP};
    int rc;
    if (block_rows == 4) rc = acc_bits == 16 ? launch_blk3<4, true>(P, n_groups, sms, smem_max, st) : launch_blk3<4, false>(P, n_groups, sms, smem_max, st);
    else if (acc_bits == 16) rc = block_rows == 8 ? launch_blk3<8, true>(P, n_groups, sms, smem_max, st) : launch_blk3<16, true>(P, n_groups, sms, smem_max, st);
    else rc = block_rows == 8 ? launch_blk3<8, false>(P, n_groups, sms, smem_max, st) : launch_blk3<16, false>(P, n_groups, sms, smem_max, st);
    if (rc) return rc;
    ExactParams E{a_indptr, a_indices, a_data, b_indptr, b_indices, b_data, P.glist, P.gcnt, B3_GCAP, n_from, n_splits, n_to, k, min_similarity,
                  self_match, from_index_base, to_index_base, top_idx, top_val};
    const int64_t n_warps = (int64_t)n_splits * n_from;
    blk_exact_kernel<<<(unsigned)((n_warps + 7) / 8), 256, 0, st>>>(E);
    PFZ_LAUNCH_OK();
    return 0;
}

#ifdef PFZ_B3_TIMING
int pfz_debug_b3_cycles(unsigned long long *out8, int32_t reset) {
    PFZ_CUDA_OK(cudaDeviceSynchronize());
    PFZ_CUDA_OK(cudaMemcpyFromSymbol(out8, g_b3_cycles, sizeof(unsigned long long) * 8));
    if (reset) { unsigned long long z[8] = {0}; PFZ_CUDA_OK(cudaMemcpyToSymbol(g_b3_cycles, z, sizeof(z))); }
    return 0;
}
#endif
}
```

polyfuzz_b200/csrc/pfz_tfidf.cu:

```cuda
#include "pfz_common.cuh"

namespace pfz {

constexpr uint64_t KEY_PAD = ~0ull;
constexpr uint32_t SYM_UNKNOWN = 0xffffffffu;
constexpr uint32_t SYM_SPACE = 1u;
constexpr int MAX_N = 8;

__device__ __forceinline__ uint32_t clean_symbol(uint32_t c) {
    if (c >= 'A' && c <= 'Z') c += 32;
    if (c >= 'a' && c <= 'z') return 12u + (c - 'a');
    if (c >= '0' && c <= '9') return 2u + (c - '0');
    if (c == ' ') return SYM_SPACE;
    if (c == 0x0130u) return 12u + ('i' - 'a');
    if (c == 0x212Au) return 12u + ('k' - 'a');
    return 0u;
}

template <bool CLEAN>
__device__ void process_row(const uint32_t *__restrict__ blob, int64_t beg, int L, int lo, int hi, bool remove_space,
                            const uint32_t *__restrict__ sym_table, uint64_t base, uint32_t *sym, uint64_t *keys,
                            int cap_keys, uint64_t *__restrict__ out_codes, int32_t *__restrict__ out_tf,
                            int32_t *out_cnt) {
    const int lane = lane_id();
    const unsigned lt = (1u << lane) - 1u;
    int Lc = 0;
    if (CLEAN) {
        int kept = 0;
        for (int p0 = 0; p0 < L; p0 += 32) {
            int p = p0 + lane;
            uint32_t s = (p < L) ? clean_symbol(blob[beg + p]) : 0u;
            unsigned m = __ballot_sync(FULL, s != 0u);
            if (s != 0u) sym[kept + __popc(m & lt)] = s;
            kept += __popc(m);
        }
        __syncwarp();
        int last_ns = -1;
        for (int p0 = 0; p0 < kept; p0 += 32) {
            int p = p0 + lane;
            bool ns = (p < kept) && sym[p] != SYM_SPACE;
            unsigned m = __ballot_sync(FULL, ns);
            if (m) last_ns = p0 + 31 - __clz(m);
        }
        int outn = 0;
        for (int p0 = 0; p0 < kept; p0 += 32) {
            int p = p0 + lane;
            uint32_t s = (p < kept) ? sym[p] : 0u;
            uint32_t prev = (p > 0 && p < kept) ? sym[p - 1] : SYM_SPACE;
            __syncwarp();
            bool keep = (p < kept) && (s != SYM_SPACE || (prev != SYM_SPACE && p < last_ns));
            unsigned m = __ballot_sync(FULL, keep);
            if (keep) sym[outn + __popc(m & lt)] = s;
            outn += __popc(m);
            __syncwarp();
        }
        Lc = outn;
    } else {
        for (int p0 = 0; p0 < L; p0 += 32) {
            int p = p0 + lane;
            if (p < L) {
                uint32_t c = blob[beg + p];
                sym[p] = (c < 0x110000u) ? sym_table[c] : SYM_UNKNOWN;
            }
        }
        Lc = L;
        __syncwarp();
    }

    uint64_t pw[MAX_N];
    {
        uint64_t q = 1;
#pragma unroll
        for (int d = MAX_N - 1; d >= 0; --d) {
            if (d < hi) { pw[d] = q; q *= base; } else pw[d] = 0;
        }
    }
    const uint32_t space_sym = CLEAN ? SYM_SPACE : sym_table[0x20];
    int cnt = 0;
    for (int n = lo; n <= hi; ++n) {
        const int nst = Lc - n + 1;
        for (int i0 = 0; i0 < nst; i0 += 32) {
            int i = i0 + lane;
            bool ok = i < nst;
            uint64_t code = 0;
            if (ok) {
#pragma unroll
                for (int d = 0; d < MAX_N; ++d) {
                    if (d < n) {
                        uint32_t s = sym[i + d];
                        if (s == SYM_UNKNOWN || (remove_space && s == space_sym)) ok = false;
                        code += (uint64_t)s * pw[d];
                    }
                }
            }
            unsigned m = __ballot_sync(FULL, ok);
            if (ok) keys[cnt + __popc(m & lt)] = code;
            cnt += __popc(m);
        }
    }
    int P = 1;
    while (P < cnt) P <<= 1;
    if (P > cap_keys) P = cap_keys;
    for (int q = cnt + lane; q < P; q += 32) keys[q] = KEY_PAD;
    __syncwarp();
    for (int k = 2; k <= P; k <<= 1) {
        for (int j = k >> 1; j > 0; j >>= 1) {
            for (int t = lane; t < (P >> 1); t += 32) {
                int i = ((t & ~(j - 1)) << 1) | (t & (j - 1));
                int ix = i | j;
                uint64_t a = keys[i], b = keys[ix];
                bool up = (i & k) == 0;
                if ((a > b) == up) { keys[i] = b; keys[ix] = a; }
            }
            __syncwarp();
        }
    }
    int nd = 0;
    for (int q0 = 0; q0 < cnt; q0 += 32) {
        int q = q0 + lane;
        bool head = false;
        uint64_t c = 0;
        if (q < cnt) { c = keys[q]; head = (q == 0) || keys[q - 1] != c; }
        unsigned m = __ballot_sync(FULL, head);
        if (head) {
            int len = 1;
            while (q + len < cnt && keys[q + len] == c) ++len;
            int pos = nd + __popc(m & lt);
            out_codes[pos] = c;
            out_tf[pos] = len;
        }
        nd += __popc(m);
    }
    if (lane == 0) *out_cnt = nd;
}

template <bool CLEAN>
__global__ void __launch_bounds__(256) ngram_rows_warp_kernel(const uint32_t *__restrict__ blob, const int64_t *__restrict__ offsets,
                                                              int n_rows, int lo, int hi, int remove_space,
                                                              const uint32_t *__restrict__ sym_table, uint64_t base,
                                                              const int64_t *__restrict__ occ_ptr, uint64_t *__restrict__ codes,
                                                              int32_t *__restrict__ tf, int32_t *__restrict__ row_cnt) {
    constexpr int WPB = 8;
    constexpr int CAP = PFZ_WARP_ROW_SLOTS;
    __shared__ uint64_t s_keys[WPB][CAP];
    __shared__ uint32_t s_sym[WPB][CAP + MAX_N];
    const int w = threadIdx.x >> 5;
    for (int r = blockIdx.x * WPB + w; r < n_rows; r += gridDim.x * WPB) {
        const int64_t o0 = occ_ptr[r];
        const int64_t slots = occ_ptr[r + 1] - o0;
        if (slots > CAP) continue;
        const int64_t beg = offsets[r];
        const int L = (int)(offsets[r + 1] - beg);
        if (slots == 0) { if (lane_id() == 0) row_cnt[r] = 0; continue; }
        process_row<CLEAN>(blob, beg, L, lo, hi, remove_space != 0, sym_table, base, s_sym[w], s_keys[w], CAP,
                           codes + o0, tf + o0, row_cnt + r);
        __syncwarp();
    }
}

template <bool CLEAN>
__global__ void __launch_bounds__(32) ngram_rows_long_kernel(const uint32_t *__restrict__ blob, const int64_t *__restrict__ offsets,
                                                             const int32_t *__restrict__ long_rows, int n_long, int lo, int hi,
                                                             int remove_space, const uint32_t *__restrict__ sym_table, uint64_t base,
                                                             const int64_t *__restrict__ occ_ptr, uint64_t *__restrict__ codes,
                                                             int32_t *__restrict__ tf, int32_t *__restrict__ row_cnt) {
    extern __shared__ __align__(16) unsigned char dyn[];
    uint64_t *s_keys = reinterpret_cast<uint64_t *>(dyn);
    uint32_t *s_sym = reinterpret_cast<uint32_t *>(dyn + (size_t)PFZ_MAX_ROW_SLOTS * 8);
    for (int q = blockIdx.x; q < n_long; q += gridDim.x) {
        const int r = long_rows[q];
        const int64_t o0 = occ_ptr[r];
        const int64_t beg = offsets[r];
        const int L = (int)(offsets[r + 1] - beg);
        process_row<CLEAN>(blob, beg, L, lo, hi, remove_space != 0, sym_table, base, s_sym, s_keys, PFZ_MAX_ROW_SLOTS,
                           codes + o0, tf + o0, row_cnt + r);
        __syncwarp();
    }
}

__global__ void alphabet_mark_kernel(const uint32_t *__restrict__ blob, int64_t n, uint8_t *__restrict__ present) {
    for (int64_t i = (int64_t)blockIdx.x * blockDim.x + threadIdx.x; i < n; i += (int64_t)gridDim.x * blockDim.x) {
        uint32_t c = blob[i];
        if (c < 0x110000u) present[c] = 1;
    }
}

__global__ void __launch_bounds__(256) df_dense_kernel(const uint64_t *__restrict__ codes, const int64_t *__restrict__ occ_ptr,
                                                       const int32_t *__restrict__ row_cnt, int n_rows, int32_t *__restrict__ df_dense) {
    const int lane = lane_id();
    const int gw = (blockIdx.x * blockDim.x + threadIdx.x) >> 5, nw = (gridDim.x * blockDim.x) >> 5;
    for (int r = gw; r < n_rows; r += nw) {
        const int64_t o0 = occ_ptr[r];
        const int c = row_cnt[r];
        for (int q = lane; q < c; q += 32) atomicAdd(&df_dense[codes[o0 + q]], 1);
    }
}

__global__ void flag_positive_kernel(const int32_t *__restrict__ df_dense, int64_t n, int32_t *__restrict__ flag) {
    for (int64_t i = (int64_t)blockIdx.x * blockDim.x + threadIdx.x; i < n; i += (int64_t)gridDim.x * blockDim.x)
        flag[i] = df_dense[i] > 0;
}

__global__ void vocab_compact_kernel(const int32_t *__restrict__ df_dense, int64_t n, int32_t *__restrict__ rank,
                                     uint64_t *__restrict__ vocab_keys, int32_t *__restrict__ df, int32_t *__restrict__ n_vocab) {
    for (int64_t i = (int64_t)blockIdx.x * blockDim.x + threadIdx.x; i < n; i += (int64_t)gridDim.x * blockDim.x) {
        const int32_t d = df_dense[i];
        const int32_t pos = rank[i];
        if (i == n - 1) *n_vocab = pos + (d > 0);
        if (d > 0) { vocab_keys[pos] = (uint64_t)i; df[pos] = d; }
        else rank[i] = -1;
    }
}

__global__ void __launch_bounds__(256) gather_codes_kernel(const uint64_t *__restrict__ codes, const int64_t *__restrict__ occ_ptr,
                                                           const int32_t *__restrict__ row_cnt, int n_rows, uint64_t *__restrict__ keys,
                                                           unsigned long long *__restrict__ cursor) {
    const int lane = lane_id();
    const int gw = (blockIdx.x * blockDim.x + threadIdx.x) >> 5, nw = (gridDim.x * blockDim.x) >> 5;
    for (int r = gw; r < n_rows; r += nw) {
        const int64_t o0 = occ_ptr[r];
        const int c = row_cnt[r];
        if (c == 0) continue;
        unsigned long long dst = 0;
        if (lane == 0) dst = atomicAdd(cursor, (unsigned long long)c);
        dst = __shfl_sync(FULL, dst, 0);
        for (int q = lane; q < c; q += 32) keys[dst + q] = codes[o0 + q];
    }
}

__global__ void idf_lookup_kernel(const int32_t *__restrict__ df, const int32_t *__restrict__ n_vocab, int64_t cap, const double *__restrict__ table,
                                  int64_t n_table, double *__restrict__ idf) {
    const int64_t nv = min((int64_t)*n_vocab, cap);
    for (int64_t i = (int64_t)blockIdx.x * blockDim.x + threadIdx.x; i < nv; i += (int64_t)gridDim.x * blockDim.x) {
        const int64_t d = df[i];
        idf[i] = table[d < n_table ? d : n_table - 1];
    }
}

constexpr int BS_TILE = 4096;
constexpr int BS_THREADS = 512;

__global__ void __launch_bounds__(BS_THREADS) bitonic_local_kernel(uint64_t *__restrict__ keys, int64_t n, int64_t k_first, int64_t k_last,
                                                                   int64_t j_first) {
    __shared__ uint64_t s[BS_TILE];
    const int64_t base = (int64_t)blockIdx.x * BS_TILE;
    for (int t = threadIdx.x; t < BS_TILE; t += BS_THREADS) s[t] = (base + t < n) ? keys[base + t] : KEY_PAD;
    __syncthreads();
    for (int64_t k = k_first; k <= k_last; k <<= 1) {
        int64_t j0 = (k == k_first) ? j_first : (k >> 1);
        for (int64_t j = j0; j > 0; j >>= 1) {
            for (int t = threadIdx.x; t < BS_TILE / 2; t += BS_THREADS) {
                int i = ((t & ~((int)j - 1)) << 1) | (t & ((int)j - 1));
                int ix = i | (int)j;
                uint64_t a = s[i], b = s[ix];
                bool up = ((base + i) & k) == 0;
                if ((a > b) == up) { s[i] = b; s[ix] = a; }
            }
            __syncthreads();
        }
    }
    for (int t = threadIdx.x; t < BS_TILE; t += BS_THREADS) if (base + t < n) keys[base + t] = s[t];
}

__global__ void bitonic_global_kernel(uint64_t *__restrict__ keys, int64_t n, int64_t k, int64_t j) {
    for (int64_t t = (int64_t)blockIdx.x * blockDim.x + threadIdx.x; t < (n >> 1); t += (int64_t)gridDim.x * blockDim.x) {
        int64_t i = ((t & ~(j - 1)) << 1) | (t & (j - 1));
        int64_t ix = i | j;
        uint64_t a = keys[i], b = keys[ix];
        bool up = (i & k) == 0;
        if ((a > b) == up) { keys[i] = b; keys[ix] = a; }
    }
}

__global__ void sorted_heads_kernel(const uint64_t *__restrict__ keys, int64_t cap, const int64_t *__restrict__ n_keys, int32_t *__restrict__ flag) {
    const int64_t n = *n_keys;
    for (int64_t i = (int64_t)blockIdx.x * blockDim.x + threadIdx.x; i < cap; i += (int64_t)gridDim.x * blockDim.x)
        flag[i] = (i < n) && (i == 0 || keys[i] != keys[i - 1]);
}

__global__ void sorted_compact_kernel(const uint64_t *__restrict__ keys, int64_t cap, const int64_t *__restrict__ n_keys,
                                      const int32_t *__restrict__ pos, uint64_t *__restrict__ vocab_keys, int32_t *__restrict__ head_at,
                                      int32_t *__restrict__ n_vocab) {
    const int64_t n = *n_keys;
    for (int64_t i = (int64_t)blockIdx.x * blockDim.x + threadIdx.x; i < cap; i += (int64_t)gridDim.x * blockDim.x) {
        bool head = (i < n) && (i == 0 || keys[i] != keys[i - 1]);
        if (head) { vocab_keys[pos[i]] = keys[i]; head_at[pos[i]] = (int32_t)i; }
        if (i == cap - 1) { int32_t v = pos[i] + (head ? 1 : 0); *n_vocab = v; }
    }
}

__global__ void head_diff_kernel(const int32_t *__restrict__ head_at, const int32_t *__restrict__ n_vocab, const int64_t *__restrict__ n_keys,
                                 int32_t *__restrict__ df, int64_t cap) {
    const int32_t V = *n_vocab;
    for (int64_t i = (int64_t)blockIdx.x * blockDim.x + threadIdx.x; i < V && i < cap; i += (int64_t)gridDim.x * blockDim.x) {
        int32_t nxt = (i + 1 < V) ? head_at[i + 1] : (int32_t)(*n_keys);
        df[i] = nxt - head_at[i];
    }
}

__device__ __forceinline__ int32_t lookup_col(uint64_t code, const int32_t *__restrict__ rank_dense, const uint64_t *__restrict__ vocab_keys,
                                              int32_t n_vocab) {
    if (rank_dense) return rank_dense[code];
    int32_t lo = 0, hi = n_vocab;
    while (lo < hi) {
        int32_t mid = (lo + hi) >> 1;
        if (vocab_keys[mid] < code) lo = mid + 1; else hi = mid;
    }
    return (lo < n_vocab && vocab_keys[lo] == code) ? lo : -1;
}

__global__ void __launch_bounds__(256) emit_count_kernel(const uint64_t *__restrict__ codes, const int64_t *__restrict__ occ_ptr,
                                                         const int32_t *__restrict__ row_cnt, int n_rows, const int32_t *__restrict__ rank_dense,
                                                         const uint64_t *__restrict__ vocab_keys, int32_t n_vocab, int32_t *__restrict__ row_nnz) {
    const int lane = lane_id();
    const int gw = (blockIdx.x * blockDim.x + threadIdx.x) >> 5, nw = (gridDim.x * blockDim.x) >> 5;
    for (int r = gw; r <= n_rows; r += nw) {
        if (r == n_rows) { if (lane == 0) row_nnz[r] = 0; continue; }
        const int64_t o0 = occ_ptr[r];
        const int c = row_cnt[r];
        int tot = 0;
        for (int q0 = 0; q0 < c; q0 += 32) {
            int q = q0 + lane;
            bool ok = (q < c) && lookup_col(codes[o0 + q], rank_dense, vocab_keys, n_vocab) >= 0;
            tot += __popc(__ballot_sync(FULL, ok));
        }
        if (lane == 0) row_nnz[r] = tot;
    }
}

__global__ void __launch_bounds__(256) emit_write_kernel(const uint64_t *__restrict__ codes, const int32_t *__restrict__ tf,
                                                         const int64_t *__restrict__ occ_ptr, const int32_t *__restrict__ row_cnt, int n_rows,
                                                         const int32_t *__restrict__ rank_dense, const uint64_t *__restrict__ vocab_keys,
                                                         int32_t n_vocab, const double *__restrict__ idf, const int32_t *__restrict__ indptr,
                                                         int32_t *__restrict__ indices, double *__restrict__ data) {
    const int lane = lane_id();
    const unsigned lt = (1u << lane) - 1u;
    const int gw = (blockIdx.x * blockDim.x + threadIdx.x) >> 5, nw = (gridDim.x * blockDim.x) >> 5;
    for (int r = gw; r < n_rows; r += nw) {
        const int64_t o0 = occ_ptr[r];
        const int c = row_cnt[r];
        const int32_t w0 = indptr[r];
        double ss = 0.0;
        for (int q0 = 0; q0 < c; q0 += 32) {
            int q = q0 + lane;
            int32_t col = (q < c) ? lookup_col(codes[o0 + q], rank_dense, vocab_keys, n_vocab) : -1;
            double x2 = 0.0;
            if (col >= 0) { double x = __dmul_rn((double)tf[o0 + q], idf[col]); x2 = __dmul_rn(x, x); }
            unsigned m = __ballot_sync(FULL, col >= 0);
            while (m) {
                int l = __ffs(m) - 1; m &= m - 1;
                ss = __dadd_rn(ss, shfl_d(x2, l));
            }
        }
        const double norm = __dsqrt_rn(ss);
        int wrote = 0;
        for (int q0 = 0; q0 < c; q0 += 32) {
            int q = q0 + lane;
            int32_t col = (q < c) ? lookup_col(codes[o0 + q], rank_dense, vocab_keys, n_vocab) : -1;
            unsigned m = __ballot_sync(FULL, col >= 0);
            if (col >= 0) {
                double x = __dmul_rn((double)tf[o0 + q], idf[col]);
                int p = w0 + wrote + __popc(m & lt);
                indices[p] = col;
                data[p] = (norm != 0.0) ? __ddiv_rn(x, norm) : x;
            }
            wrote += __popc(m);
        }
    }
}

static int grid_for(int64_t work_items, int threads, int cap = SM_COUNT * 16) {
    int64_t g = (work_items + threads - 1) / threads;
    if (g < 1) g = 1;
    if (g > cap) g = cap;
    return (int)g;
}

}

using namespace pfz;

extern "C" {

int pfz_alphabet_mark(const uint32_t *blob, int64_t n_chars, uint8_t *present, void *stream) {
    if (n_chars <= 0) return 0;
    alphabet_mark_kernel<<<grid_for(n_chars, 256), 256, 0, as_stream(stream)>>>(blob, n_chars, present);
    PFZ_LAUNCH_OK();
    return 0;
}

int pfz_ngram_rows(const uint32_t *blob, const int64_t *offsets, int32_t n_rows, int32_t lo, int32_t hi, int32_t flags,
                   const uint32_t *sym_table, uint32_t base, const int64_t *occ_ptr, const int32_t *long_rows, int32_t n_long,
                   uint64_t *codes, int32_t *tf, int32_t *row_cnt, void *stream) {
    PFZ_REQUIRE(lo >= 1 && hi >= lo && hi <= MAX_N, "pfz_ngram_rows: n-gram range (%d,%d) unsupported (1 <= lo <= hi <= %d)", lo, hi, MAX_N);
    const bool clean = flags & PFZ_FLAG_CLEAN;
    PFZ_REQUIRE(clean || sym_table, "pfz_ngram_rows: raw mode needs sym_table");
    {
        long double cs = 1; for (int i = 0; i < hi; ++i) cs *= (long double)base;
        PFZ_REQUIRE(cs < 18446744073709551615.0L, "pfz_ngram_rows: alphabet %u ^ n %d exceeds 64-bit n-gram codes", base, hi);
    }
    if (n_rows <= 0) return 0;
    const int rs = (flags & PFZ_FLAG_REMOVE_SPACE) ? 1 : 0;
    cudaStream_t st = as_stream(stream);
    int grid = grid_for((int64_t)n_rows * 32, 256, SM_COUNT * 8);
    if (clean) ngram_rows_warp_kernel<true><<<grid, 256, 0, st>>>(blob, offsets, n_rows, lo, hi, rs, sym_table, base, occ_ptr, codes, tf, row_cnt);
    else       ngram_rows_warp_kernel<false><<<grid, 256, 0, st>>>(blob, offsets, n_rows, lo, hi, rs, sym_table, base, occ_ptr, codes, tf, row_cnt);
    PFZ_LAUNCH_OK();
    if (n_long > 0) {
        PFZ_REQUIRE(long_rows, "pfz_ngram_rows: n_long > 0 but long_rows is NULL");
        const size_t smem = (size_t)PFZ_MAX_ROW_SLOTS * 8 + ((size_t)PFZ_MAX_ROW_SLOTS + MAX_N + 8) * 4;
        if (clean) {
            PFZ_CUDA_OK(cudaFuncSetAttribute(ngram_rows_long_kernel<true>, cudaFuncAttributeMaxDynamicSharedMemorySize, (int)smem));
            ngram_rows_long_kernel<true><<<n_long < 592 ? n_long : 592, 32, smem, st>>>(blob, offsets, long_rows, n_long, lo, hi, rs, sym_table, base, occ_ptr, codes, tf, row_cnt);
        } else {
            PFZ_CUDA_OK(cudaFuncSetAttribute(ngram_rows_long_kernel<false>, cudaFuncAttributeMaxDynamicSharedMemorySize, (int)smem));
            ngram_rows_long_kernel<false><<<n_long < 592 ? n_long : 592, 32, smem, st>>>(blob, offsets, long_rows, n_long, lo, hi, rs, sym_table, base, occ_ptr, codes, tf, row_cnt);
        }
        PFZ_LAUNCH_OK();
    }
    return 0;
}

int pfz_df_dense(const uint64_t *codes, const int64_t *occ_ptr, const int32_t *row_cnt, int32_t n_rows, int32_t *df_dense, void *stream) {
    if (n_rows <= 0) return 0;
    df_dense_kernel<<<grid_for((int64_t)n_rows * 32, 256), 256, 0, as_stream(stream)>>>(codes, occ_ptr, row_cnt, n_rows, df_dense);
    PFZ_LAUNCH_OK();
    return 0;
}

int pfz_vocab_compact_dense(const int32_t *df_dense, int64_t code_space, uint64_t *vocab_keys, int32_t *df, int32_t *rank_dense,
                            int32_t *n_vocab_dev, void *ws, void *stream) {
    PFZ_REQUIRE(code_space > 0 && code_space < (1ll << 31), "pfz_vocab_compact_dense: bad code space %lld", (long long)code_space);
    cudaStream_t st = as_stream(stream);
    flag_positive_kernel<<<grid_for(code_space, 256), 256, 0, st>>>(df_dense, code_space, rank_dense);
    PFZ_LAUNCH_OK();
    if (scan_exclusive_i32(rank_dense, rank_dense, code_space, ws, st)) return 1;
    vocab_compact_kernel<<<grid_for(code_space, 256), 256, 0, st>>>(df_dense, code_space, rank_dense, vocab_keys, df, n_vocab_dev);
    PFZ_LAUNCH_OK();
    return 0;
}

int pfz_gather_codes(const uint64_t *codes, const int64_t *occ_ptr, const int32_t *row_cnt, int32_t n_rows, uint64_t *keys,
                     int64_t *cursor_dev, void *stream) {
    if (n_rows <= 0) return 0;
    gather_codes_kernel<<<grid_for((int64_t)n_rows * 32, 256), 256, 0, as_stream(stream)>>>(codes, occ_ptr, row_cnt, n_rows, keys,
                                                                                             reinterpret_cast<unsigned long long *>(cursor_dev));
    PFZ_LAUNCH_OK();
    return 0;
}

int pfz_idf_lookup(const int32_t *df, const int32_t *n_vocab_dev, int64_t cap, const double *table, int64_t n_table, double *idf, void *stream) {
    if (cap <= 0) return 0;
    PFZ_REQUIRE(n_table >= 1, "pfz_idf_lookup: empty table");
    idf_lookup_kernel<<<grid_for(cap, 256), 256, 0, as_stream(stream)>>>(df, n_vocab_dev, cap, table, n_table, idf);
    PFZ_LAUNCH_OK();
    return 0;
}

int pfz_sort_u64(uint64_t *keys, int64_t n, void *stream) {
    PFZ_REQUIRE(n > 0 && (n & (n - 1)) == 0, "pfz_sort_u64: n=%lld must be a power of two", (long long)n);
    cudaStream_t st = as_stream(stream);
    const int64_t nblk = (n + BS_TILE - 1) / BS_TILE;
    const int64_t kloc = n < BS_TILE ? n : BS_TILE;
    bitonic_local_kernel<<<(unsigned)nblk, BS_THREADS, 0, st>>>(keys, n, 2, kloc, 1);
    PFZ_LAUNCH_OK();
    for (int64_t k = (int64_t)BS_TILE * 2; k <= n; k <<= 1) {
        int64_t j = k >> 1;
        for (; j >= BS_TILE; j >>= 1) {
            bitonic_global_kernel<<<grid_for(n >> 1, 256, SM_COUNT * 32), 256, 0, st>>>(keys, n, k, j);
            PFZ_LAUNCH_OK();
        }
        bitonic_local_kernel<<<(unsigned)nblk, BS_THREADS, 0, st>>>(keys, n, k, k, j);
        PFZ_LAUNCH_OK();
    }
    return 0;
}

int pfz_vocab_from_sorted(const uint64_t *sorted_keys, int64_t cap, const int64_t *n_keys_dev, uint64_t *vocab_keys, int32_t *df,
                          int32_t *n_vocab_dev, void *ws, void *stream) {
    PFZ_REQUIRE(cap > 0 && cap < (1ll << 31), "pfz_vocab_from_sorted: bad capacity %lld", (long long)cap);
    cudaStream_t st = as_stream(stream);
    int32_t *pos = reinterpret_cast<int32_t *>(ws);
    int32_t *head_at = pos + cap;
    void *sws = reinterpret_cast<char *>(ws) + (((size_t)cap * 8 + 255) / 256) * 256;
    sorted_heads_kernel<<<grid_for(cap, 256), 256, 0, st>>>(sorted_keys, cap, n_keys_dev, pos);
    PFZ_LAUNCH_OK();
    if (scan_exclusive_i32(pos, pos, cap, sws, st)) return 1;
    sorted_compact_kernel<<<grid_for(cap, 256), 256, 0, st>>>(sorted_keys, cap, n_keys_dev, pos, vocab_keys, head_at, n_vocab_dev);
    PFZ_LAUNCH_OK();
    head_diff_kernel<<<grid_for(cap, 256), 256, 0, st>>>(head_at, n_vocab_dev, n_keys_dev, df, cap);
    PFZ_LAUNCH_OK();
    return 0;
}

int pfz_tfidf_emit(const uint64_t *codes, const int32_t *tf, const int64_t *occ_ptr, const int32_t *row_cnt, int32_t n_rows,
                   const int32_t *rank_dense, const uint64_t *vocab_keys, int32_t n_vocab, const double *idf, int32_t *indptr,
                   int32_t *indices, double *data, void *ws, void *stream) {
    PFZ_REQUIRE(n_rows >= 0, "pfz_tfidf_emit: n_rows < 0");
    cudaStream_t st = as_stream(stream);
    emit_count_kernel<<<grid_for((int64_t)(n_rows + 1) * 32, 256), 256, 0, st>>>(codes, occ_ptr, row_cnt, n_rows, rank_dense, vocab_keys, n_vocab, indptr);
    PFZ_LAUNCH_OK();
    if (scan_exclusive_i32(indptr, indptr, (int64_t)n_rows + 1, ws, st)) return 1;
    if (n_rows > 0) {
        emit_write_kernel<<<grid_for((int64_t)n_rows * 32, 256), 256, 0, st>>>(codes, tf, occ_ptr, row_cnt, n_rows, rank_dense, vocab_keys, n_vocab,
                                                                                  idf, indptr, indices, data);
        PFZ_LAUNCH_OK();
    }
    return 0;
}
}
```

polyfuzz_b200/engine.py:

```python
import ctypes
import os

import numpy as np
import torch

from . import _lib
from .strings import pack_utf32, pack_strings, ngram_slot_bounds

FLAG_CLEAN, FLAG_REMOVE_SPACE = 1, 2
WARP_ROW_SLOTS, MAX_ROW_SLOTS = 256, 8192
DENSE_CODE_SPACE_MAX = 1 << 24
CLEAN_BASE = 38
N_CODE_POINTS = 0x110000


def _dev():
    if not torch.cuda.is_available():
        raise RuntimeError("polyfuzz_b200 needs a CUDA device (sm_90a); there is no CPU fallback")
    return torch.device("cuda", torch.cuda.current_device())


def _stream():
    return ctypes.c_void_p(torch.cuda.current_stream().cuda_stream)


def _p(t):
    return ctypes.c_void_p(t.data_ptr()) if t is not None else ctypes.c_void_p(0)


class _PinnedPool:

    def __init__(self):
        self.free = []

    def take(self, nbytes):
        best = None
        for i, (buf, ev) in enumerate(self.free):
            if buf.numel() >= nbytes and (best is None or buf.numel() < self.free[best][0].numel()):
                best = i
        if best is not None:
            buf, ev = self.free.pop(best)
            if ev is not None:
                ev.synchronize()
            return buf
        size = max(1 << 16, 1 << int(nbytes - 1).bit_length())
        return torch.empty(size, dtype=torch.uint8).pin_memory()

    def give(self, buf, ev):
        if len(self.free) < 16:
            self.free.append((buf, ev))


_PINNED = _PinnedPool()
_PINNED_OUT = _PinnedPool()


def _to_dev(arr, dtype=None):
    dev = _dev()
    arr = np.ascontiguousarray(arr)
    t = torch.from_numpy(arr)
    if dtype is not None:
        t = t.view(dtype)
    if t.numel() == 0:
        return torch.empty(0, dtype=t.dtype, device=dev)
    nbytes = arr.nbytes
    stage = _PINNED.take(nbytes)
    stage[:nbytes].copy_(torch.from_numpy(arr.reshape(-1).view(np.uint8)))
    out = torch.empty(t.shape, dtype=t.dtype, device=dev)
    out.view(torch.uint8).reshape(-1).copy_(stage[:nbytes], non_blocking=True)
    ev = torch.cuda.Event(); ev.record()
    _PINNED.give(stage, ev)
    return out


def _ws(nbytes):
    return torch.empty(max(int(nbytes), 256), dtype=torch.uint8, device=_dev())


class CsrMatrix:

    def __init__(self, indptr, indices, data, n_rows, n_cols):
        self.indptr, self.indices, self.data = indptr, indices, data
        self.n_rows, self.n_cols = n_rows, n_cols

    def to_scipy(self):
        import scipy.sparse as sp
        ip = self.indptr.cpu().numpy()
        nnz = int(ip[-1]) if len(ip) else 0
        return sp.csr_matrix((self.data[:nnz].cpu().numpy(), self.indices[:nnz].cpu().numpy(), ip),
                             shape=(self.n_rows, self.n_cols))

    @staticmethod
    def from_scipy(m):
        m = m.tocsr(); m.sort_indices()
        return CsrMatrix(_to_dev(m.indptr.astype(np.int32)), _to_dev(m.indices.astype(np.int32)),
                         _to_dev(m.data.astype(np.float64)), m.shape[0], m.shape[1])


class StagedStrings:
    __slots__ = ("n", "n_chars", "d_blob", "d_off", "occ_ptr", "d_long", "n_long", "cap", "h2d_bytes", "lo", "hi", "max_slots",
                 "ascii", "host_blob", "host_off")


def stage_strings(strings, lo, hi):
    blob, offsets, _arrow = pack_strings(strings)
    slots, occ = ngram_slot_bounds(offsets, lo, hi)
    if len(slots) and slots.max() > MAX_ROW_SLOTS:
        r = int(slots.argmax())
        raise ValueError(f"string {r} has {int(slots[r])} n-gram slots; the vectoriser supports at most "
                         f"{MAX_ROW_SLOTS} per string")
    long_rows = np.nonzero(slots > WARP_ROW_SLOTS)[0].astype(np.int32)
    S = StagedStrings()
    S.n, S.n_chars, S.cap, S.lo, S.hi = len(strings), int(blob.size), int(occ[-1]), lo, hi
    S.max_slots = int(slots.max()) if len(slots) else 0
    S.ascii = blob.dtype == np.uint8
    S.host_blob, S.host_off = (blob, offsets) if S.ascii else (None, None)
    if blob.size == 0:
        S.d_blob = torch.zeros(1, dtype=torch.int32, device=_dev())
    elif blob.dtype == np.uint8:
        S.d_blob = _to_dev(blob).to(torch.int32)
    else:
        S.d_blob = _to_dev(blob.view(np.int32), torch.int32)
    S.d_off = _to_dev(offsets)
    S.occ_ptr = _to_dev(occ)
    S.n_long = len(long_rows)
    S.d_long = _to_dev(long_rows) if S.n_long else None
    S.h2d_bytes = blob.nbytes + offsets.nbytes + occ.nbytes + long_rows.nbytes
    return S


_IDF_TABLES = {}


def _idf_table(n_docs):
    key = (int(n_docs), torch.cuda.current_device())
    t = _IDF_TABLES.get(key)
    if t is None:
        tab = np.log((n_docs + 1.0) / (np.arange(0, n_docs + 1, dtype=np.float64) + 1.0)) + 1.0
        if len(_IDF_TABLES) > 8:
            _IDF_TABLES.clear()
        t = _IDF_TABLES[key] = _to_dev(tab)
    return t


class _Rows:
    __slots__ = ("n", "occ_ptr", "codes", "tf", "row_cnt", "cap", "_keep")


class NgramTfidf:

    def __init__(self, n_gram_range=(3, 3), clean_string=True, remove_space_ngrams=True):
        lo, hi = int(n_gram_range[0]), int(n_gram_range[1])
        if not (1 <= lo <= hi <= 8):
            raise ValueError(f"n_gram_range {n_gram_range} unsupported (1 <= lo <= hi <= 8)")
        self.lo, self.hi = lo, hi
        self.clean = bool(clean_string)
        self.remove_space = bool(remove_space_ngrams)
        self.flags = (FLAG_CLEAN if self.clean else 0) | (FLAG_REMOVE_SPACE if self.remove_space else 0)
        self.base = CLEAN_BASE if self.clean else None
        self.alphabet = None
        self._h_vocab_keys = None
        self._h_idf = None
        self._h_df = None
        self._n_vocab = 0
        self._sum_df_sq = None
        self.n_fit_docs = 0
        self.max_row_nnz = 0
        self._d_sym = self._d_vocab = self._d_idf = self._d_rank = self._d_df = None

    def __getstate__(self):
        if self._n_vocab:
            self.vocab_keys, self.df, self.idf
        st = dict(self.__dict__)
        for k in ("_d_sym", "_d_vocab", "_d_idf", "_d_rank", "_d_df"):
            st[k] = None
        return st

    def __setstate__(self, st):
        self.__dict__.update(st)
        self.__dict__.setdefault("_d_df", None)

    @property
    def n_vocab(self):
        return self._n_vocab

    @property
    def vocab_keys(self):
        if self._h_vocab_keys is None and self._n_vocab and self._d_vocab is not None:
            self._h_vocab_keys = self._d_vocab[:self._n_vocab].cpu().numpy().view(np.uint64)
        return self._h_vocab_keys

    @property
    def df(self):
        if self._h_df is None and self._n_vocab and self._d_df is not None:
            self._h_df = self._d_df[:self._n_vocab].cpu().numpy().astype(np.int64)
        return self._h_df

    @property
    def idf(self):
        if self._h_idf is None and self._n_vocab and self._d_idf is not None:
            self._h_idf = self._d_idf[:self._n_vocab].cpu().numpy()
        return self._h_idf

    def code_space(self):
        return int(self.base) ** self.hi

    def vocabulary(self):
        out = []
        if self.clean:
            symbols = [None, " "] + [chr(c) for c in range(48, 58)] + [chr(c) for c in range(97, 123)]
        else:
            symbols = [None] + [chr(int(c)) for c in self.alphabet]
        for key in self.vocab_keys.tolist():
            digs = []
            for _ in range(self.hi):
                digs.append(key % self.base); key //= self.base
            out.append("".join(symbols[d] for d in reversed(digs) if d))
        return out

    def stage(self, strings):
        return stage_strings(strings, self.lo, self.hi)

    def _stage_a(self, S, d_sym, fit=False):
        R = _Rows()
        R.n, R.cap, R.occ_ptr = S.n, S.cap, S.occ_ptr
        R.codes = torch.empty(max(R.cap, 1), dtype=torch.int64, device=_dev())
        R.tf = torch.empty(max(R.cap, 1), dtype=torch.int32, device=_dev())
        R.row_cnt = torch.zeros(max(R.n, 1), dtype=torch.int32, device=_dev())
        _lib.call("pfz_ngram_rows", _p(S.d_blob), _p(S.d_off), R.n, self.lo, self.hi, self.flags, _p(d_sym),
                  int(self.base), _p(R.occ_ptr), _p(S.d_long), S.n_long, _p(R.codes), _p(R.tf), _p(R.row_cnt),
                  _stream())
        R._keep = S
        if not fit:
            bound = S.max_slots
            if bound > DENSE32_MAX_ROW_NNZ and R.n:
                bound = int(R.row_cnt[:R.n].max().item())
            self.max_row_nnz = max(self.max_row_nnz, bound)
        return R

    def _fit_alphabet(self, staged, comm=None):
        present = torch.zeros(N_CODE_POINTS, dtype=torch.uint8, device=_dev())
        for S in staged:
            if S.n_chars:
                _lib.call("pfz_alphabet_mark", _p(S.d_blob), S.n_chars, _p(present), _stream())
        if comm is not None:
            comm.all_reduce_max(present)
        self.alphabet = np.nonzero(present.cpu().numpy())[0].astype(np.uint32)
        self.base = len(self.alphabet) + 1

    def _sym_table(self):
        if self.clean:
            return None
        if self._d_sym is None:
            tab = np.full(N_CODE_POINTS, 0xFFFFFFFF, dtype=np.uint32)
            tab[self.alphabet] = np.arange(1, len(self.alphabet) + 1, dtype=np.uint32)
            self._d_sym = _to_dev(tab.view(np.int32), torch.int32)
        return self._d_sym

    def fit_rows(self, lists):
        return self.fit_staged([self.stage(l) for l in lists])

    def fit_staged(self, staged, counted=None, comm=None, n_docs_total=None):
        if counted is None:
            counted = [True] * len(staged)
        if not self.clean:
            self._d_sym = None
            self._fit_alphabet(staged, comm)
        if self.code_space() >= 2 ** 64:
            raise ValueError(f"alphabet of {self.base - 1} symbols with {self.hi}-grams exceeds 64-bit n-gram codes")
        d_sym = self._sym_table()
        rows = [self._stage_a(S, d_sym, fit=True) for S in staged]
        n_docs = sum(r.n for r, c in zip(rows, counted) if c)
        dev = _dev()
        d_nv = torch.zeros(1, dtype=torch.int32, device=dev)
        cs = self.code_space()
        total_cap = sum(r.cap for r in rows)
        if comm is not None:
            if cs > DENSE_CODE_SPACE_MAX:
                raise NotImplementedError("multi-GPU fit needs an n-gram code space <= 2^24 (e.g. cleaned n <= 4)")
            if n_docs_total is not None:
                n_docs, total_cap_all = int(n_docs_total), cs
            else:
                meta = torch.tensor([n_docs, total_cap], dtype=torch.int64, device=dev)
                comm.all_reduce_sum(meta)
                n_docs, total_cap_all = int(meta[0].item()), int(meta[1].item())
        else:
            total_cap_all = total_cap
        if total_cap_all == 0:
            raise ValueError("empty vocabulary; perhaps the documents only contain stop words")
        if cs <= DENSE_CODE_SPACE_MAX:
            df_dense = torch.zeros(cs, dtype=torch.int32, device=dev)
            for r, c in zip(rows, counted):
                if c:
                    _lib.call("pfz_df_dense", _p(r.codes), _p(r.occ_ptr), _p(r.row_cnt), r.n, _p(df_dense), _stream())
            if comm is not None:
                comm.all_reduce_sum(df_dense)
            vmax = min(cs, total_cap_all)
            d_vocab = torch.empty(vmax, dtype=torch.int64, device=dev)
            d_df = torch.empty(vmax, dtype=torch.int32, device=dev)
            d_rank = torch.empty(cs, dtype=torch.int32, device=dev)
            ws = _ws(_lib.load().pfz_scan_ws_bytes(cs))
            _lib.call("pfz_vocab_compact_dense", _p(df_dense), cs, _p(d_vocab), _p(d_df), _p(d_rank), _p(d_nv), _p(ws), _stream())
        else:
            cap2 = 1 << max(int(total_cap - 1).bit_length(), 1)
            keys = torch.full((cap2,), -1, dtype=torch.int64, device=dev)
            cursor = torch.zeros(1, dtype=torch.int64, device=dev)
            for r in rows:
                _lib.call("pfz_gather_codes", _p(r.codes), _p(r.occ_ptr), _p(r.row_cnt), r.n, _p(keys), _p(cursor), _stream())
            _lib.call("pfz_sort_u64", _p(keys), cap2, _stream())
            d_vocab = torch.empty(total_cap, dtype=torch.int64, device=dev)
            d_df = torch.empty(total_cap, dtype=torch.int32, device=dev)
            d_rank = None
            ws = _ws(cap2 * 8 + 256 + _lib.load().pfz_scan_ws_bytes(cap2))
            _lib.call("pfz_vocab_from_sorted", _p(keys), cap2, _p(cursor), _p(d_vocab), _p(d_df), _p(d_nv), _p(ws), _stream())
        d_tab = _idf_table(n_docs)
        d_idf = torch.empty(d_df.numel(), dtype=torch.float64, device=dev)
        _lib.call("pfz_idf_lookup", _p(d_df), _p(d_nv), int(d_df.numel()), _p(d_tab), int(d_tab.numel()), _p(d_idf), _stream())
        dfv = d_df.double()
        vmask = torch.arange(d_df.numel(), device=dev) < d_nv
        mx = torch.stack([r.row_cnt[:r.n].max() if r.n else torch.zeros((), dtype=torch.int32, device=dev) for r in rows]).max()
        stats = torch.stack([d_nv[0].double(), torch.where(vmask, dfv * dfv, torch.zeros_like(dfv)).sum(), mx.double()]).cpu().numpy()
        V = int(stats[0])
        if V == 0:
            raise ValueError("empty vocabulary; perhaps the documents only contain stop words")
        self._n_vocab = V
        self._sum_df_sq = float(stats[1])
        self.max_row_nnz = max(self.max_row_nnz, int(stats[2]))
        self._h_vocab_keys = self._h_df = self._h_idf = None
        self.n_fit_docs = n_docs
        self._d_vocab = d_vocab[:V]
        self._d_df = d_df[:V]
        self._d_rank = d_rank
        self._d_idf = d_idf[:V]
        return rows

    def _ensure_device_state(self):
        if not self._n_vocab:
            raise ValueError("vectoriser is not fitted")
        if self._d_vocab is None:
            self._d_vocab = _to_dev(self._h_vocab_keys.view(np.int64))
            self._d_idf = _to_dev(self._h_idf)
            self._d_df = _to_dev(self._h_df.astype(np.int32))
            self._d_rank = None
            cs = self.code_space()
            if cs <= DENSE_CODE_SPACE_MAX:
                rank = np.full(cs, -1, dtype=np.int32)
                rank[self.vocab_keys.astype(np.int64)] = np.arange(len(self.vocab_keys), dtype=np.int32)
                self._d_rank = _to_dev(rank)

    def rows(self, strings):
        self._ensure_device_state()
        return self._stage_a(strings if isinstance(strings, StagedStrings) else self.stage(strings), self._sym_table())

    def emit(self, R):
        self._ensure_device_state()
        dev = _dev()
        indptr = torch.empty(R.n + 1, dtype=torch.int32, device=dev)
        indices = torch.empty(max(R.cap, 1), dtype=torch.int32, device=dev)
        data = torch.empty(max(R.cap, 1), dtype=torch.float64, device=dev)
        ws = _ws(_lib.load().pfz_scan_ws_bytes(R.n + 1))
        _lib.call("pfz_tfidf_emit", _p(R.codes), _p(R.tf), _p(R.occ_ptr), _p(R.row_cnt), R.n, _p(self._d_rank),
                  _p(self._d_vocab), self.n_vocab, _p(self._d_idf), _p(indptr), _p(indices), _p(data), _p(ws), _stream())
        return CsrMatrix(indptr, indices, data, R.n, self.n_vocab)

    def density(self):
        if not self.n_fit_docs or not self._n_vocab:
            return None
        if self._sum_df_sq is None:
            d = self.df.astype(np.float64)
            self._sum_df_sq = float((d * d).sum())
        return self._sum_df_sq / float(self.n_fit_docs) ** 2

    def fit(self, strings):
        self.fit_rows([strings])
        return self

    def transform(self, strings):
        return self.emit(self.rows(strings))


DEFAULT_TILE = {"list": int(os.environ.get("PFZ_TILE_LIST", "512")), "dense": int(os.environ.get("PFZ_TILE_DENSE", "1024")),
                "dense32": int(os.environ.get("PFZ_TILE_DENSE32", "1024")), "block": int(os.environ.get("PFZ_TILE_BLOCK", "4096")),
                "hash": 65536}
BLOCK_TILE_STEP, BLOCK_TILE_MAX = 128, 4096
BLOCK_ROWS = int(os.environ.get("PFZ_BLOCK_ROWS", "8"))
BLOCK_ACC_BITS = int(os.environ.get("PFZ_BLOCK_ACC_BITS", "16"))


class SparseIndex:

    def __init__(self, csr: CsrMatrix, tile=None, variant="list"):
        n = csr.n_rows
        self.variant = variant
        if tile is None:
            tile = DEFAULT_TILE[variant]
            if variant == "block" and BLOCK_ACC_BITS != 16:
                tile //= 2
        tile = max(64, min(int(tile), ((max(n, 1) + 63) // 64) * 64))
        self.acc_bits = 32
        if variant == "block":
            self.acc_bits = 16 if BLOCK_ACC_BITS == 16 else 32
            step = BLOCK_TILE_STEP * (2 if self.acc_bits == 16 else 1)
            tile = min(BLOCK_TILE_MAX, max(step, (tile + step - 1) // step * step))
        self.tile = tile
        self.n_to = n
        self.n_vocab = csr.n_cols
        self.n_tiles = max(1, (n + tile - 1) // tile)
        ncell = self.n_vocab * self.n_tiles
        dev = _dev()
        self.seg = torch.empty(ncell + 1, dtype=torch.int32, device=dev)
        cap = max(csr.indices.numel(), 1)
        self.post_idx = torch.empty(cap, dtype=torch.int16, device=dev)
        self.post_val = torch.empty(cap, dtype=torch.float64, device=dev)
        f32 = variant in ("dense32", "block")
        self.post_val32 = torch.empty(cap, dtype=torch.float32, device=dev) if f32 else None
        self.term_maxw = torch.empty(max(self.n_vocab, 1), dtype=torch.float32, device=dev) if variant == "dense32" else None
        self.post_pk = torch.empty((cap, 2), dtype=torch.int32, device=dev) if variant in ("block", "hash") else None
        self.csr = csr
        ws = _ws((ncell + 1) * 4 + 512 + _lib.load().pfz_scan_ws_bytes(ncell + 1))
        flags = 0
        if os.environ.get("PFZ_BANK_ORDER", "1") != "0" and variant != "hash":
            flags = 2 if f32 else 1
        _lib.call("pfz_index_build", _p(csr.indptr), _p(csr.indices), _p(csr.data), n, self.n_vocab, tile,
                  self.n_tiles, flags, _p(self.seg), _p(self.post_idx), _p(self.post_val), _p(self.post_val32), _p(self.term_maxw), _p(ws), _stream())
        if variant in ("block", "hash") and n > 0:
            if self.acc_bits == 16:
                _lib.call("pfz_index_pack_q15", _p(self.post_idx), _p(self.post_val), ctypes.c_void_p(self.seg.data_ptr() + 4 * ncell), tile, _p(self.post_pk), _stream())
            else:
                _lib.call("pfz_index_pack_q26", _p(self.post_idx), _p(self.post_val), ctypes.c_void_p(self.seg.data_ptr() + 4 * ncell), _p(self.post_pk), _stream())


DENSE32_MAX_ROW_NNZ = 128


HASH_MIN_ROWS = int(os.environ.get("PFZ_HASH_MIN_ROWS", "32768"))
HASH_MAX_ROW_NNZ = 256


def choose_variant(density, max_row_nnz=None, n_to=None):
    if density is None or density < DENSE_MIN_DENSITY:
        if (density is not None and n_to is not None and n_to >= HASH_MIN_ROWS and max_row_nnz is not None
                and max_row_nnz <= HASH_MAX_ROW_NNZ and SPARSE_VARIANT == "hash"):
            return "hash"
        return "list"
    if DENSE_VARIANT in ("dense32", "block") and (max_row_nnz is None or max_row_nnz > DENSE32_MAX_ROW_NNZ):
        return "dense"
    return DENSE_VARIANT


def _auto_splits(n_from, n_tiles, sm_count=132):
    want = sm_count * 32
    if n_from >= want:
        return 1
    return max(1, min(n_tiles, (want + max(n_from, 1) - 1) // max(n_from, 1)))


K2_LIST, K2_DENSE, K2_DENSE32 = 1, 2, 3
DENSE_MIN_DENSITY = float(os.environ.get("PFZ_DENSE_MIN_DENSITY", "0.03"))
DENSE_VARIANT = os.environ.get("PFZ_DENSE_VARIANT", "block")
SPARSE_VARIANT = os.environ.get("PFZ_SPARSE_VARIANT", "hash")
K2_VARIANT = {"list": K2_LIST, "dense": K2_DENSE, "dense32": K2_DENSE32}
HASH_SLOTS = int(os.environ.get("PFZ_HASH_SLOTS", "0"))


def _hash_slots(index):
    return HASH_SLOTS if HASH_SLOTS else 2048
BLOCK_MAX_ROWS = (1 << 22) - 1


def _spcos_block(a, index, k, min_similarity, self_match, from_index_base, to_index_base, n_splits):
    dev = _dev()
    n_from = a.n_rows
    nnz_cap = int(a.indices.numel())
    ws = _ws(_lib.load().pfz_spcos_block_ws_bytes(n_from, nnz_cap, index.n_vocab, n_splits))
    err = torch.zeros(1, dtype=torch.int32, device=dev)
    ti = torch.empty((n_splits, max(n_from, 1), k), dtype=torch.int32, device=dev)
    tv = torch.empty((n_splits, max(n_from, 1), k), dtype=torch.float64, device=dev)
    _lib.call("pfz_spcos_topk_block", _p(a.indptr), _p(a.indices), _p(a.data), n_from, nnz_cap, _p(index.seg), _p(index.post_pk),
              _p(index.csr.indptr), _p(index.csr.indices), _p(index.csr.data), index.n_vocab, index.tile, index.n_tiles, index.n_to, k,
              float(min_similarity), int(bool(self_match)), int(from_index_base), int(to_index_base), n_splits, BLOCK_ROWS, index.acc_bits, _p(ti), _p(tv), _p(err),
              _p(ws), _stream())
    if n_splits > 1:
        oi = torch.empty((max(n_from, 1), k), dtype=torch.int32, device=dev)
        ov = torch.empty((max(n_from, 1), k), dtype=torch.float64, device=dev)
        _lib.call("pfz_topk_merge", _p(ti), _p(tv), n_splits, n_from, k, k, _p(oi), _p(ov), _stream())
    else:
        oi, ov = ti[0], tv[0]
    return oi[:n_from], ov[:n_from], err


def spcos_topk(a: CsrMatrix, index: SparseIndex, k, min_similarity=0.0, self_match=False, from_index_base=0,
               to_index_base=0, n_splits=None, variant="auto"):
    if variant == "auto":
        variant = index.variant
    dev = _dev()
    n_from = a.n_rows
    k = int(k)
    if k < 1:
        raise ValueError("top_n must be >= 1")
    if n_splits is None:
        n_splits = _auto_splits(n_from, index.n_tiles)
    n_splits = max(1, min(int(n_splits), index.n_tiles))
    if variant == "block":
        if index.post_pk is None:
            raise ValueError("the index was not built for the block variant")
        if k <= 32 and n_from <= BLOCK_MAX_ROWS:
            oi, ov, err = _spcos_block(a, index, k, min_similarity, self_match, from_index_base, to_index_base, n_splits)
            index._block_err = err
            return oi, ov
        variant = "dense32"
    counter = torch.zeros(n_splits, dtype=torch.int32, device=dev)
    if variant == "hash" and index.post_pk is None:
        raise ValueError("the index was not built for the hash variant")
    err = torch.zeros(1, dtype=torch.int32, device=dev) if variant == "hash" else None
    pages = []
    excl_v = excl_i = None
    remaining = k
    while remaining > 0:
        kp = min(32, remaining)
        ti = torch.empty((n_splits, max(n_from, 1), kp), dtype=torch.int32, device=dev)
        tv = torch.empty((n_splits, max(n_from, 1), kp), dtype=torch.float64, device=dev)
        if variant == "dense32" and index.post_val32 is None:
            raise ValueError("the index was not built for the dense32 variant")
        if variant == "hash":
            _lib.call("pfz_spcos_topk_hash", _p(a.indptr), _p(a.indices), _p(a.data), n_from, _p(index.seg), _p(index.post_pk),
                      _p(index.csr.indptr), _p(index.csr.indices), _p(index.csr.data), index.tile, index.n_tiles, index.n_to, kp,
                      float(min_similarity), int(bool(self_match)), int(from_index_base), int(to_index_base), n_splits, _hash_slots(index),
                      _p(excl_v), _p(excl_i), _p(ti), _p(tv), _p(counter), _p(err), _stream())
            index._hash_err = err
        else:
          _lib.call("pfz_spcos_topk", _p(a.indptr), _p(a.indices), _p(a.data), n_from, _p(index.seg), _p(index.post_idx),
                  _p(index.post_val), _p(index.post_val32), _p(index.csr.indptr), _p(index.csr.indices), _p(index.csr.data),
                  _p(index.term_maxw), index.n_vocab, index.tile, index.n_tiles, index.n_to, kp, float(min_similarity),
                  int(bool(self_match)), int(from_index_base), int(to_index_base), n_splits, _p(excl_v), _p(excl_i),
                  _p(ti), _p(tv), _p(counter), K2_VARIANT[variant], _stream())
        if n_splits > 1:
            oi = torch.empty((max(n_from, 1), kp), dtype=torch.int32, device=dev)
            ov = torch.empty((max(n_from, 1), kp), dtype=torch.float64, device=dev)
            _lib.call("pfz_topk_merge", _p(ti), _p(tv), n_splits, n_from, kp, kp, _p(oi), _p(ov), _stream())
        else:
            oi, ov = ti[0], tv[0]
        pages.append((oi, ov))
        remaining -= kp
        if remaining > 0:
            excl_v = ov[:, -1].contiguous(); excl_i = oi[:, -1].contiguous()
            done = excl_i < 0
            excl_v = torch.where(done, torch.full_like(excl_v, float("-inf")), excl_v)
            excl_i = torch.where(done, torch.full_like(excl_i, 2 ** 31 - 1), excl_i)
    if len(pages) == 1:
        oi, ov = pages[0]
    else:
        oi = torch.cat([p[0] for p in pages], dim=1); ov = torch.cat([p[1] for p in pages], dim=1)
    return oi[:n_from], ov[:n_from]


def topk_merge(idx, val, k_out):
    n_lists, n_from, k_in = idx.shape
    dev = idx.device
    oi = torch.empty((n_from, k_out), dtype=torch.int32, device=dev)
    ov = torch.empty((n_from, k_out), dtype=torch.float64, device=dev)
    _lib.call("pfz_topk_merge", _p(idx.contiguous()), _p(val.contiguous()), n_lists, n_from, k_in, k_out, _p(oi), _p(ov), _stream())
    return oi, ov
```

Baseline: 958.4 billion.

## Trim launches and syncs across fit, emit, index build and block search

Several unrelated overhead cuts land together. The hand-written multi-pass scan becomes a single cub ExclusiveSum call. The fit statistics come from one fused kernel that writes to pinned host memory, replacing a chain of torch reductions and a .cpu() copy. tfidf_emit skips its count kernel when every row is known to be in the vocabulary. Posting packing and the cursor memset move into index_build, and the float32 value copy is built lazily only when the dense32 fallback needs it. The block path also changes how term keys are built and sorted (partly elided), which adds cub dependencies and some correctness risk in the new key encoding.

Measured after the change: 999.6 billion, median of 6. +4.3%, better.

```diff
diff --git a/include/pfz.h b/include/pfz.h
--- a/include/pfz.h
+++ b/include/pfz.h
@@ -52,20 +52,27 @@
 
 int pfz_idf_lookup(const int32_t *df, const int32_t *n_vocab_dev, int64_t cap, const double *table, int64_t n_table, double *idf, void *stream);
 
+int pfz_fit_stats(const int32_t *df, const int32_t *n_vocab_dev, int64_t cap, const int32_t *row_cnt_a, int32_t n_a,
+                  const int32_t *row_cnt_b, int32_t n_b, int64_t *stats_dev, int64_t *stats_host, void *stream);
+
 int pfz_tfidf_emit(const uint64_t *codes, const int32_t *tf, const int64_t *occ_ptr, const int32_t *row_cnt,
                    int32_t n_rows, const int32_t *rank_dense, const uint64_t *vocab_keys, int32_t n_vocab,
-                   const double *idf, int32_t *indptr, int32_t *indices, double *data, void *ws, void *stream);
+                   const double *idf, int32_t all_in_vocab, int32_t *indptr, int32_t *indices, double *data, void *ws,
+                   void *stream);
 
 int64_t pfz_scan_ws_bytes(int64_t n);
 
 
 #define PFZ_INDEX_BANK_ORDER   1
 #define PFZ_INDEX_BANK_ORDER32 2
+#define PFZ_INDEX_PACK_Q15     4
+#define PFZ_INDEX_PACK_Q26     8
 int pfz_index_build(const int32_t *indptr, const int32_t *indices, const double *data, int32_t n_rows,
                     int32_t n_vocab, int32_t tile, int32_t n_tiles, int32_t flags,
                     int32_t *seg, uint16_t *post_idx, double *post_val, float *post_val32 ,
                     float *term_maxw ,
-                    void *ws, void *stream);
+                    void *post_pk , void *ws, void *stream);
+int pfz_index_val32(const double *post_val, const int32_t *nnz_dev, float *post_val32, void *stream);
 
 #define PFZ_K2_LIST  1
 #define PFZ_K2_DENSE 2
@@ -82,8 +89,7 @@
 
 int64_t pfz_spcos_block_ws_bytes(int32_t n_from, int64_t nnz_cap_from, int32_t n_vocab, int32_t n_splits);
 int64_t pfz_spcos_block_gcnt_offset(int32_t n_from, int64_t nnz_cap_from, int32_t n_vocab, int32_t n_splits);
-int pfz_index_pack_q26(const uint16_t *post_idx, const double *post_val, const int32_t *nnz_dev, void *post_pk, void *stream);
-int pfz_index_pack_q15(const uint16_t *post_idx, const double *post_val, const int32_t *nnz_dev, int32_t tile, void *post_pk, void *stream);
+int64_t pfz_spcos_block_perm_offset(int32_t n_from, int64_t nnz_cap_from, int32_t n_vocab, int32_t n_splits);
 int pfz_spcos_topk_block(const int32_t *a_indptr, const int32_t *a_indices, const double *a_data, int32_t n_from, int64_t nnz_cap_from,
                          const int32_t *seg, const void *post_pk, const int32_t *b_indptr, const int32_t *b_indices, const double *b_data,
                          int32_t n_vocab, int32_t tile, int32_t n_tiles, int32_t n_to, int32_t k, double min_similarity, int32_t self_match,
diff --git a/polyfuzz_b200/_lib.py b/polyfuzz_b200/_lib.py
--- a/polyfuzz_b200/_lib.py
+++ b/polyfuzz_b200/_lib.py
@@ -22,8 +22,10 @@
     "pfz_sort_u64": [c_vp, c_i64, c_vp],
     "pfz_vocab_from_sorted": [c_vp, c_i64, c_vp, c_vp, c_vp, c_vp, c_vp, c_vp],
     "pfz_idf_lookup": [c_vp, c_vp, c_i64, c_vp, c_i64, c_vp, c_vp],
-    "pfz_tfidf_emit": [c_vp, c_vp, c_vp, c_vp, c_i32, c_vp, c_vp, c_i32, c_vp, c_vp, c_vp, c_vp, c_vp, c_vp],
-    "pfz_index_build": [c_vp, c_vp, c_vp, c_i32, c_i32, c_i32, c_i32, c_i32, c_vp, c_vp, c_vp, c_vp, c_vp, c_vp, c_vp],
+    "pfz_fit_stats": [c_vp, c_vp, c_i64, c_vp, c_i32, c_vp, c_i32, c_vp, c_vp, c_vp],
+    "pfz_tfidf_emit": [c_vp, c_vp, c_vp, c_vp, c_i32, c_vp, c_vp, c_i32, c_vp, c_i32, c_vp, c_vp, c_vp, c_vp, c_vp],
+    "pfz_index_build": [c_vp, c_vp, c_vp, c_i32, c_i32, c_i32, c_i32, c_i32, c_vp, c_vp, c_vp, c_vp, c_vp, c_vp, c_vp, c_vp],
+    "pfz_index_val32": [c_vp, c_vp, c_vp, c_vp],
     "pfz_spcos_topk": [c_vp, c_vp, c_vp, c_i32, c_vp, c_vp, c_vp, c_vp, c_vp, c_vp, c_vp, c_vp, c_i32, c_i32, c_i32, c_i32, c_i32, c_f64, c_i32,
                        c_i64, c_i64, c_i32, c_vp, c_vp, c_vp, c_vp, c_vp, c_i32, c_vp],
     "pfz_topk_merge": [c_vp, c_vp, c_i32, c_i32, c_i32, c_i32, c_vp, c_vp, c_vp],
@@ -31,8 +33,7 @@
                             c_i32, c_vp, c_vp, c_vp, c_vp, c_vp, c_vp, c_vp],
     "pfz_spcos_block_ws_bytes": [c_i32, c_i64, c_i32, c_i32],
     "pfz_spcos_block_gcnt_offset": [c_i32, c_i64, c_i32, c_i32],
-    "pfz_index_pack_q26": [c_vp, c_vp, c_vp, c_vp, c_vp],
-    "pfz_index_pack_q15": [c_vp, c_vp, c_vp, c_i32, c_vp, c_vp],
+    "pfz_spcos_block_perm_offset": [c_i32, c_i64, c_i32, c_i32],
     "pfz_spcos_topk_block": [c_vp, c_vp, c_vp, c_i32, c_i64, c_vp, c_vp, c_vp, c_vp, c_vp, c_i32, c_i32, c_i32, c_i32, c_i32, c_f64, c_i32,
                              c_i64, c_i64, c_i32, c_i32, c_i32, c_vp, c_vp, c_vp, c_vp, c_vp],
     "pfz_lev_pack": [c_vp, c_vp, c_vp, c_i32, c_vp, c_vp, c_vp, c_vp, c_vp],
@@ -67,7 +68,7 @@
     "pfz_dense_topn_select": [c_vp, c_vp, c_vp, c_i32, c_i32, c_i32, c_f64, c_i32, c_i64, c_vp, c_vp, c_vp, c_vp],
 }
 _RESTYPES = {"pfz_last_error": ctypes.c_char_p, "pfz_scan_ws_bytes": c_i64, "pfz_launch_count": c_i64, "pfz_spcos_block_ws_bytes": c_i64,
-             "pfz_spcos_block_gcnt_offset": c_i64,
+             "pfz_spcos_block_gcnt_offset": c_i64, "pfz_spcos_block_perm_offset": c_i64,
              "pfz_dense_exact_fallback_ws_bytes": c_i64}
 
 
diff --git a/polyfuzz_b200/csrc/pfz_core.cu b/polyfuzz_b200/csrc/pfz_core.cu
--- a/polyfuzz_b200/csrc/pfz_core.cu
+++ b/polyfuzz_b200/csrc/pfz_core.cu
@@ -1,4 +1,5 @@
 #include <stdarg.h>
+#include <cub/device/device_scan.cuh>
 #include "pfz_common.cuh"
 
 namespace pfz {
@@ -10,65 +11,16 @@
     va_end(ap);
 }
 
-constexpr int SCAN_THREADS = 512;
-constexpr int SCAN_ITEMS = 8;
-constexpr int SCAN_TILE = SCAN_THREADS * SCAN_ITEMS;
-
-__global__ void __launch_bounds__(SCAN_THREADS) scan_tile_kernel(const int32_t *__restrict__ in, int32_t *__restrict__ out,
-                                                               int64_t n, int32_t *__restrict__ sums) {
-    __shared__ int32_t warp_tot[SCAN_THREADS / 32];
-    const int64_t base = (int64_t)blockIdx.x * SCAN_TILE + (int64_t)threadIdx.x * SCAN_ITEMS;
-    int32_t v[SCAN_ITEMS];
-    int32_t tsum = 0;
-#pragma unroll
-    for (int i = 0; i < SCAN_ITEMS; ++i) {
-        v[i] = (base + i < n) ? in[base + i] : 0;
-        tsum += v[i];
-    }
-    int32_t incl = warp_incl_scan(tsum);
-    const int lane = threadIdx.x & 31, w = threadIdx.x >> 5;
-    if (lane == 31) warp_tot[w] = incl;
-    __syncthreads();
-    if (w == 0) {
-        int32_t t = (lane < SCAN_THREADS / 32) ? warp_tot[lane] : 0;
-        int32_t ti = warp_incl_scan(t);
-        if (lane < SCAN_THREADS / 32) warp_tot[lane] = ti - t;
-        if (lane == 31 && sums) sums[blockIdx.x] = ti;
-    }
-    __syncthreads();
-    int32_t run = warp_tot[w] + incl - tsum;
-#pragma unroll
-    for (int i = 0; i < SCAN_ITEMS; ++i) {
-        if (base + i < n) out[base + i] = run;
-        run += v[i];
-    }
+static size_t scan_temp_bytes(int64_t n) {
+    size_t bytes = 0;
+    if (n > 0 && cub::DeviceScan::ExclusiveSum(nullptr, bytes, (const int32_t *)nullptr, (int32_t *)nullptr, n) != cudaSuccess) bytes = 0;
+    return bytes;
 }
-
-__global__ void __launch_bounds__(SCAN_THREADS) scan_add_kernel(int32_t *__restrict__ out, int64_t n,
-                                                              const int32_t *__restrict__ offs) {
-    const int32_t add = offs[blockIdx.x];
-    const int64_t base = (int64_t)blockIdx.x * SCAN_TILE + (int64_t)threadIdx.x * SCAN_ITEMS;
-#pragma unroll
-    for (int i = 0; i < SCAN_ITEMS; ++i)
-        if (base + i < n) out[base + i] += add;
-}
-
-static int64_t n_tiles_of(int64_t n) { return (n + SCAN_TILE - 1) / SCAN_TILE; }
 
 int scan_exclusive_i32(const int32_t *in, int32_t *out, int64_t n, void *ws, cudaStream_t st) {
     if (n <= 0) return 0;
-    const int64_t nt = n_tiles_of(n);
-    if (nt == 1) {
-        scan_tile_kernel<<<1, SCAN_THREADS, 0, st>>>(in, out, n, nullptr);
-        PFZ_LAUNCH_OK();
-        return 0;
-    }
-    int32_t *sums = reinterpret_cast<int32_t *>(ws);
-    char *next_ws = reinterpret_cast<char *>(ws) + ((nt * 4 + 255) / 256) * 256;
-    scan_tile_kernel<<<(unsigned)nt, SCAN_THREADS, 0, st>>>(in, out, n, sums);
-    PFZ_LAUNCH_OK();
-    if (scan_exclusive_i32(sums, sums, nt, next_ws, st)) return 1;
-    scan_add_kernel<<<(unsigned)nt, SCAN_THREADS, 0, st>>>(out, n, sums);
+    size_t bytes = scan_temp_bytes(n);
+    PFZ_CUDA_OK(cub::DeviceScan::ExclusiveSum(ws, bytes, in, out, n, st));
     PFZ_LAUNCH_OK();
     return 0;
 }
@@ -112,12 +64,8 @@
 int64_t pfz_launch_count(void) { return (int64_t)__atomic_load_n(&pfz::g_launches, __ATOMIC_RELAXED); }
 
 int64_t pfz_scan_ws_bytes(int64_t n) {
-    int64_t total = 256;
-    while (n > pfz::SCAN_TILE) {
-        n = pfz::n_tiles_of(n);
-        total += ((n * 4 + 255) / 256) * 256;
-    }
-    return total;
+    const size_t bytes = pfz::scan_temp_bytes(n);
+    return (int64_t)(bytes > 256 ? (bytes + 255) / 256 * 256 : 256);
 }
 
 int pfz_device_info(int32_t *sm_count, int32_t *smem_optin, int32_t *cc_major, int32_t *cc_minor) {
diff --git a/polyfuzz_b200/csrc/pfz_spcos.cu b/polyfuzz_b200/csrc/pfz_spcos.cu
--- a/polyfuzz_b200/csrc/pfz_spcos.cu
+++ b/polyfuzz_b200/csrc/pfz_spcos.cu
@@ -4,7 +4,8 @@
 namespace pfz {
 
 __global__ void index_count_kernel(const int32_t *__restrict__ indptr, const int32_t *__restrict__ indices, int n_rows, int tile, int n_tiles,
-                                   int32_t *__restrict__ cnt) {
+                                   int32_t *__restrict__ cnt, int32_t *__restrict__ cur, int64_t ncell) {
+    for (int64_t i = (int64_t)blockIdx.x * blockDim.x + threadIdx.x; i < ncell; i += (int64_t)gridDim.x * blockDim.x) cur[i] = 0;
     const int lane = lane_id();
     const int gw = (blockIdx.x * blockDim.x + threadIdx.x) >> 5, nw = (gridDim.x * blockDim.x) >> 5;
     for (int r = gw; r < n_rows; r += nw) {
@@ -70,6 +71,22 @@
             __syncwarp();
         }
     }
+}
+
+template <int PACK>
+__device__ __forceinline__ uint2 pack_posting(uint32_t j, double w, uint32_t half_tile) {
+    if (PACK == 26) return make_uint2(j, (uint32_t)__double2ll_rn(w * 67108864.0));
+    const bool hi = j >= half_tile;
+    const uint32_t w15 = (uint32_t)max(1ll, __double2ll_rn(w * 32768.0));
+    return make_uint2(((hi ? j - half_tile : j) << 2) | ((hi ? 0x3244u : 0x4432u) << 16), w15);
+}
+
+template <int PACK>
+__global__ void index_pack_kernel(const uint16_t *__restrict__ post_idx, const double *__restrict__ post_val, const int32_t *__restrict__ nnz_ptr,
+                                  uint32_t half_tile, uint2 *__restrict__ post_pk) {
+    const int64_t n = *nnz_ptr;
+    for (int64_t i = (int64_t)blockIdx.x * blockDim.x + threadIdx.x; i < n; i += (int64_t)gridDim.x * blockDim.x)
+        post_pk[i] = pack_posting<PACK>(post_idx[i], post_val[i], half_tile);
 }
 
 __global__ void to_f32_kernel(const double *__restrict__ x, int64_t n_minus, const int32_t *__restrict__ n_ptr, float *__restrict__ y) {
@@ -634,8 +651,14 @@
 
 int pfz_index_build(const int32_t *indptr, const int32_t *indices, const double *data, int32_t n_rows, int32_t n_vocab, int32_t tile,
                     int32_t n_tiles, int32_t flags, int32_t *seg, uint16_t *post_idx, double *post_val, float *post_val32, float *term_maxw,
-                    void *ws, void *stream) {
+                    void *post_pk, void *ws, void *stream) {
     PFZ_REQUIRE(tile > 0 && tile <= 65536, "pfz_index_build: tile %d out of range (1..65536)", tile);
+    const int pack = (flags & PFZ_INDEX_PACK_Q15) ? 15 : (flags & PFZ_INDEX_PACK_Q26) ? 26 : 0;
+    const int mod = (flags & PFZ_INDEX_BANK_ORDER32) ? 32 : (flags & PFZ_INDEX_BANK_ORDER) ? 16 : 0;
+    PFZ_REQUIRE(!((flags & PFZ_INDEX_PACK_Q15) && (flags & PFZ_INDEX_PACK_Q26)), "pfz_index_build: PFZ_INDEX_PACK_Q15 and _Q26 exclude each other");
+    PFZ_REQUIRE(pack == 0 || post_pk, "pfz_index_build: PFZ_INDEX_PACK_* needs post_pk");
+    PFZ_REQUIRE(pack != 15 || (tile >= 256 && tile <= 8192 && (tile % 256) == 0), "pfz_index_build: PFZ_INDEX_PACK_Q15 needs a tile that is a multiple of 256 in 256..8192, got %d", tile);
+    PFZ_REQUIRE(pack == 0 || mod != 16, "pfz_index_build: packed postings go with PFZ_INDEX_BANK_ORDER32 or no bank order");
     PFZ_REQUIRE((int64_t)n_tiles * tile >= n_rows, "pfz_index_build: n_tiles*tile < n_rows");
     const int64_t ncell = (int64_t)n_vocab * n_tiles;
     PFZ_REQUIRE(ncell + 1 < (1ll << 31), "pfz_index_build: n_vocab*n_tiles = %lld too large", (long long)ncell);
@@ -644,21 +667,24 @@
     void *sws = reinterpret_cast<char *>(ws) + ((((size_t)ncell + 1) * 4 + 255) / 256) * 256;
     PFZ_CUDA_OK(cudaMemsetAsync(seg, 0, ((size_t)ncell + 1) * 4, st));
     if (n_rows > 0) {
-        index_count_kernel<<<grid_for2((int64_t)n_rows * 32, 256, SM_COUNT * 16), 256, 0, st>>>(indptr, indices, n_rows, tile, n_tiles, seg);
+        index_count_kernel<<<grid_for2((int64_t)n_rows * 32, 256, SM_COUNT * 16), 256, 0, st>>>(indptr, indices, n_rows, tile, n_tiles, seg, cur, ncell);
         PFZ_LAUNCH_OK();
     }
     if (scan_exclusive_i32(seg, seg, ncell + 1, sws, st)) return 1;
     if (n_rows > 0) {
-        PFZ_CUDA_OK(cudaMemsetAsync(cur, 0, ((size_t)ncell + 1) * 4, st));
         if (term_maxw) PFZ_CUDA_OK(cudaMemsetAsync(term_maxw, 0, (size_t)n_vocab * 4, st));
         index_fill_kernel<<<grid_for2((int64_t)n_rows * 32, 256, SM_COUNT * 16), 256, 0, st>>>(indptr, indices, data, n_rows, tile, n_tiles, seg, cur,
                                                                                             post_idx, post_val, reinterpret_cast<int *>(term_maxw));
         PFZ_LAUNCH_OK();
-        if (flags & PFZ_INDEX_BANK_ORDER32) {
-            index_bank_order_kernel<32><<<grid_for2(ncell, 128, SM_COUNT * 16), 128, 0, st>>>(seg, ncell, post_idx, post_val);
+        if (mod) {
+            if (mod == 16) index_bank_order_kernel<16><<<grid_for2(ncell, 128, SM_COUNT * 16), 128, 0, st>>>(seg, ncell, post_idx, post_val);
+            else           index_bank_order_kernel<32><<<grid_for2(ncell, 128, SM_COUNT * 16), 128, 0, st>>>(seg, ncell, post_idx, post_val);
             PFZ_LAUNCH_OK();
-        } else if (flags & PFZ_INDEX_BANK_ORDER) {
-            index_bank_order_kernel<16><<<grid_for2(ncell, 128, SM_COUNT * 16), 128, 0, st>>>(seg, ncell, post_idx, post_val);
+        }
+        if (pack) {
+            uint2 *pk = reinterpret_cast<uint2 *>(post_pk);
+            if (pack == 15) index_pack_kernel<15><<<SM_COUNT * 8, 256, 0, st>>>(post_idx, post_val, seg + ncell, (uint32_t)tile / 2, pk);
+            else            index_pack_kernel<26><<<SM_COUNT * 8, 256, 0, st>>>(post_idx, post_val, seg + ncell, 0, pk);
             PFZ_LAUNCH_OK();
         }
         if (post_val32) {
@@ -666,6 +692,12 @@
             PFZ_LAUNCH_OK();
         }
     }
+    return 0;
+}
+
+int pfz_index_val32(const double *post_val, const int32_t *nnz_dev, float *post_val32, void *stream) {
+    to_f32_kernel<<<SM_COUNT * 8, 256, 0, as_stream(stream)>>>(post_val, 0, nnz_dev, post_val32);
+    PFZ_LAUNCH_OK();
     return 0;
 }
 
diff --git a/polyfuzz_b200/csrc/pfz_spcos_block.cu b/polyfuzz_b200/csrc/pfz_spcos_block.cu
--- a/polyfuzz_b200/csrc/pfz_spcos_block.cu
+++ b/polyfuzz_b200/csrc/pfz_spcos_block.cu
@@ -1,4 +1,5 @@
 #include <stdlib.h>
+#include <cub/device/device_radix_sort.cuh>
 #include "pfz_common.cuh"
 
 namespace pfz {
@@ -9,19 +10,15 @@
 
 struct __align__(16) BlockDesc { int pos0; int nrows; int base; int nterms; };
 
-__global__ void blk_term_key_kernel(const int32_t *__restrict__ seg, int n_vocab, int n_tiles, uint64_t *__restrict__ keys, int64_t n_pad) {
-    for (int64_t t = (int64_t)blockIdx.x * blockDim.x + threadIdx.x; t < n_pad; t += (int64_t)gridDim.x * blockDim.x) {
-        uint64_t k = ~0ull;
-        if (t < n_vocab) {
-            const uint32_t df = (uint32_t)(seg[(t + 1) * n_tiles] - seg[t * n_tiles]);
-            k = ((uint64_t)(0xffffffffu - df) << 32) | (uint32_t)t;
-        }
-        keys[t] = k;
-    }
-}
-__global__ void blk_term_rank_kernel(const uint64_t *__restrict__ keys, int n_vocab, int32_t *__restrict__ rank) {
+__global__ void blk_term_key_kernel(const int32_t *__restrict__ seg, int n_vocab, int n_tiles, int n_to, int term_bits, uint64_t *__restrict__ keys) {
+    for (int64_t t = (int64_t)blockIdx.x * blockDim.x + threadIdx.x; t < n_vocab; t += (int64_t)gridDim.x * blockDim.x) {
+        const uint32_t df = (uint32_t)(seg[(t + 1) * n_tiles] - seg[t * n_tiles]);
+        keys[t] = ((uint64_t)((uint32_t)n_to - df) << term_bits) | (uint64_t)t;
+    }
+}
+__global__ void blk_term_rank_kernel(const uint64_t *__restrict__ keys, int n_vocab, int term_bits, int32_t *__restrict__ rank) {
     for (int i = blockIdx.x * blockDim.x + threadIdx.x; i < n_vocab; i += gridDim.x * blockDim.x)
-        rank[(uint32_t)(keys[i] & 0xffffffffu)] = min(i, RANK_CAP);
+        rank[(uint32_t)(keys[i] & ((1ull << term_bits) - 1))] = min(i, RANK_CAP);
 }
 __global__ void blk_row_key_kernel(const int32_t *__restrict__ indptr, const int32_t *__restrict__ indices, const int32_t *__restrict__ rank,
                                    int n_from, uint64_t *__restrict__ keys, int64_t n_pad) {
@@ -131,24 +128,6 @@
     }
 }
 
-__global__ void blk_pack_kernel(const uint16_t *__restrict__ post_idx, const double *__restrict__ post_val, const int32_t *__restrict__ nnz_ptr,
-                                uint2 *__restrict__ post_pk) {
-    const int64_t n = *nnz_ptr;
-    for (int64_t i = (int64_t)blockIdx.x * blockDim.x + threadIdx.x; i < n; i += (int64_t)gridDim.x * blockDim.x)
-        post_pk[i] = make_uint2((uint32_t)post_idx[i], (uint32_t)__double2ll_rn(post_val[i] * 67108864.0));
-}
-
-__global__ void blk_pack15_kernel(const uint16_t *__restrict__ post_idx, const double *__restrict__ post_val, const int32_t *__restrict__ nnz_ptr,
-                                  int half_tile, uint2 *__restrict__ post_pk) {
-    const int64_t n = *nnz_ptr;
-    for (int64_t i = (int64_t)blockIdx.x * blockDim.x + threadIdx.x; i < n; i += (int64_t)gridDim.x * blockDim.x) {
-        const uint32_t j = post_idx[i];
-        const bool hi = j >= (uint32_t)half_tile;
-        const uint32_t w15 = (uint32_t)max(1ll, __double2ll_rn(post_val[i] * 32768.0));
-        post_pk[i] = make_uint2(((hi ? j - (uint32_t)half_tile : j) << 2) | ((hi ? 0x3244u : 0x4432u) << 16), w15);
-    }
-}
-
 struct BlockParams {
     const int32_t *a_indptr; const int32_t *a_indices; const double *a_data; int n_from;
     const int32_t *perm; const BlockDesc *descs; int n_desc;
@@ -777,20 +756,32 @@
     if (g > cap) g = cap;
     return (int)g;
 }
-static int64_t pow2_at_least(int64_t n) { int64_t p = 2; while (p < n) p <<= 1; return p; }
 static size_t align256(size_t x) { return (x + 255) & ~(size_t)255; }
+static int bit_width(int64_t x) { int b = 0; while (x > 0) { ++b; x >>= 1; } return b; }
+
+static size_t sort_temp_bytes(int64_t n) {
+    size_t bytes = 0;
+    cub::DoubleBuffer<uint64_t> db(nullptr, nullptr);
+    if (n > 0 && cub::DeviceRadixSort::SortKeys(nullptr, bytes, db, (int64_t)n, 0, 64) != cudaSuccess) bytes = 0;
+    return bytes;
+}
 
 struct BlockWs {
-    size_t term_keys, term_rank, row_keys, perm, pos_ptr, scan_ws, blk_terms, blk_fvdesc, blk_fv, descs, counters, gcnt, glist, total;
+    size_t term_keys, term_alt, term_rank, row_keys, row_alt, sort_tmp, sort_tmp_bytes, perm, pos_ptr, scan_ws, blk_terms, blk_fvdesc, blk_fv,
+        descs, counters, gcnt, glist, total;
 };
 constexpr int B3_GCAP = 192;
 static BlockWs block_ws_layout(int64_t n_from, int64_t nnz_cap, int64_t n_vocab, int n_splits) {
     BlockWs L; size_t o = 0;
-    const int64_t vp = pow2_at_least(n_vocab), np = pow2_at_least(n_from);
     const int64_t n_groups = (n_from + 3) / 4;
-    L.term_keys = o; o += align256((size_t)vp * 8);
+    L.term_keys = o; o += align256((size_t)(n_vocab + 1) * 8);
+    L.term_alt = o; o += align256((size_t)(n_vocab + 1) * 8);
     L.term_rank = o; o += align256((size_t)(n_vocab + 1) * 4);
-    L.row_keys = o; o += align256((size_t)np * 8);
+    L.row_keys = o; o += align256((size_t)(n_from + 1) * 8);
+    L.row_alt = o; o += align256((size_t)(n_from + 1) * 8);
+    const size_t st_v = sort_temp_bytes(n_vocab), st_r = sort_temp_bytes(n_from);
+    L.sort_tmp_bytes = st_v > st_r ? st_v : st_r;
+    L.sort_tmp = o; o += align256(L.sort_tmp_bytes);
     L.perm = o; o += align256((size_t)(n_from + 1) * 4);
     L.pos_ptr = o; o += align256((size_t)(n_from + 2) * 4);
     L.scan_ws = o; o += align256((size_t)pfz_scan_ws_bytes(n_from + 2));
@@ -819,17 +810,8 @@
     return (int64_t)block_ws_layout(n_from, nnz_cap_from, n_vocab, n_splits).gcnt;
 }
 
-int pfz_index_pack_q26(const uint16_t *post_idx, const double *post_val, const int32_t *nnz_dev, void *post_pk, void *stream) {
-    blk_pack_kernel<<<SM_COUNT * 8, 256, 0, as_stream(stream)>>>(post_idx, post_val, nnz_dev, reinterpret_cast<uint2 *>(post_pk));
-    PFZ_LAUNCH_OK();
-    return 0;
-}
-
-int pfz_index_pack_q15(const uint16_t *post_idx, const double *post_val, const int32_t *nnz_dev, int32_t tile, void *post_pk, void *stream) {
-    PFZ_REQUIRE(tile >= 256 && tile <= 8192 && (tile % 256) == 0, "pfz_index_pack_q15: tile %d must be a multiple of 256 in 256..8192", tile);
-    blk_pack15_kernel<<<SM_COUNT * 8, 256, 0, as_stream(stream)>>>(post_idx, post_val, nnz_dev, tile / 2, reinterpret_cast<uint2 *>(post_pk));
-    PFZ_LAUNCH_OK();
-    return 0;
+int64_t pfz_spcos_block_perm_offset(int32_t n_from, int64_t nnz_cap_from, int32_t n_vocab, int32_t n_splits) {
+    return (int64_t)block_ws_layout(n_from, nnz_cap_from, n_vocab, n_splits).perm;
 }
 
 int pfz_spcos_topk_block(const int32_t *a_indptr, const int32_t *a_indices, const double *a_data, int32_t n_from, int64_t nnz_cap_from,
@@ -862,18 +844,26 @@
     uint2 *blk_fv = reinterpret_cast<uint2 *>(w + L.blk_fv);
     BlockDesc *descs = reinterpret_cast<BlockDesc *>(w + L.descs);
     int32_t *counters = reinterpret_cast<int32_t *>(w + L.counters);
-    const int64_t vp = pow2_at_least(n_vocab), np = pow2_at_least(n_from);
     const int n_groups = (n_from + block_rows - 1) / block_rows;
-
-    blk_term_key_kernel<<<blk_grid(vp, 256, SM_COUNT * 8), 256, 0, st>>>(seg, n_vocab, n_tiles, term_keys, vp);
+    cub::DoubleBuffer<uint64_t> tk(term_keys, reinterpret_cast<uint64_t *>(w + L.term_alt));
+    cub::DoubleBuffer<uint64_t> rk(row_keys, reinterpret_cast<uint64_t *>(w + L.row_alt));
+    size_t tmp_bytes = L.sort_tmp_bytes;
+
+    if (n_vocab > 0) {
+        const int term_bits = bit_width(n_vocab - 1), key_bits = term_bits + bit_width(n_to);
+        blk_term_key_kernel<<<blk_grid(n_vocab, 256, SM_COUNT * 8), 256, 0, st>>>(seg, n_vocab, n_tiles, n_to, term_bits, term_keys);
+        PFZ_LAUNCH_OK();
+        PFZ_CUDA_OK(cub::DeviceRadixSort::SortKeys(w + L.sort_tmp, tmp_bytes, tk, (int64_t)n_vocab, 0, key_bits, st));
+        PFZ_LAUNCH_OK();
+        blk_term_rank_kernel<<<blk_grid(n_vocab, 256, SM_COUNT * 8), 256, 0, st>>>(tk.Current(), n_vocab, term_bits, term_rank);
+        PFZ_LAUNCH_OK();
+    }
+    blk_row_key_kernel<<<blk_grid(n_from, 256, SM_COUNT * 16), 256, 0, st>>>(a_indptr, a_indices, term_rank, n_from, row_keys, n_from);
     PFZ_LAUNCH_OK();
-    if (pfz_sort_u64(term_keys, vp, stream)) return 1;
-    blk_term_rank_kernel<<<blk_grid(n_vocab, 256, SM_COUNT * 8), 256, 0, st>>>(term_keys, n_vocab, term_rank);
+    tmp_bytes = L.sort_tmp_bytes;
+    PFZ_CUDA_OK(cub::DeviceRadixSort::SortKeys(w + L.sort_tmp, tmp_bytes, rk, (int64_t)n_from, 0, 64, st));
     PFZ_LAUNCH_OK();
-    blk_row_key_kernel<<<blk_grid(np, 256, SM_COUNT * 16), 256, 0, st>>>(a_indptr, a_indices, term_rank, n_from, row_keys, np);
-    PFZ_LAUNCH_OK();
-    if (pfz_sort_u64(row_keys, np, stream)) return 1;
-    blk_perm_kernel<<<blk_grid(n_from + 1, 256, SM_COUNT * 16), 256, 0, st>>>(row_keys, a_indptr, n_from, perm, pos_ptr);
+    blk_perm_kernel<<<blk_grid(n_from + 1, 256, SM_COUNT * 16), 256, 0, st>>>(rk.Current(), a_indptr, n_from, perm, pos_ptr);
     PFZ_LAUNCH_OK();
     if (scan_exclusive_i32(pos_ptr, pos_ptr, (int64_t)n_from + 1, w + L.scan_ws, st)) return 1;
     const int row_stride = tile * (acc_bits == 16 ? 2 : 4) + 128;
diff --git a/polyfuzz_b200/csrc/pfz_tfidf.cu b/polyfuzz_b200/csrc/pfz_tfidf.cu
--- a/polyfuzz_b200/csrc/pfz_tfidf.cu
+++ b/polyfuzz_b200/csrc/pfz_tfidf.cu
@@ -145,6 +145,7 @@
     __shared__ uint64_t s_keys[WPB][CAP];
     __shared__ uint32_t s_sym[WPB][CAP + MAX_N];
     const int w = threadIdx.x >> 5;
+    if (blockIdx.x == 0 && threadIdx.x == 0) row_cnt[n_rows] = 0;
     for (int r = blockIdx.x * WPB + w; r < n_rows; r += gridDim.x * WPB) {
         const int64_t o0 = occ_ptr[r];
         const int64_t slots = occ_ptr[r + 1] - o0;
@@ -295,6 +296,33 @@
     for (int64_t i = (int64_t)blockIdx.x * blockDim.x + threadIdx.x; i < V && i < cap; i += (int64_t)gridDim.x * blockDim.x) {
         int32_t nxt = (i + 1 < V) ? head_at[i + 1] : (int32_t)(*n_keys);
         df[i] = nxt - head_at[i];
+    }
+}
+
+__global__ void __launch_bounds__(256) fit_stats_kernel(const int32_t *__restrict__ df, const int32_t *__restrict__ n_vocab, int64_t cap,
+                                                        const int32_t *__restrict__ cnt_a, int n_a, const int32_t *__restrict__ cnt_b, int n_b,
+                                                        unsigned long long *__restrict__ stats) {
+    __shared__ unsigned long long s_sum[8];
+    __shared__ int s_max[8];
+    const int64_t nv = min((int64_t)*n_vocab, cap);
+    const int64_t n = max(nv, (int64_t)max(n_a, n_b));
+    unsigned long long sum = 0;
+    int mx = 0;
+    for (int64_t i = (int64_t)blockIdx.x * blockDim.x + threadIdx.x; i < n; i += (int64_t)gridDim.x * blockDim.x) {
+        if (i < nv) { const unsigned long long d = (unsigned)df[i]; sum += d * d; }
+        if (i < n_a) mx = max(mx, cnt_a[i]);
+        if (i < n_b) mx = max(mx, cnt_b[i]);
+    }
+#pragma unroll
+    for (int o = 16; o; o >>= 1) { sum += __shfl_xor_sync(FULL, sum, o); mx = max(mx, __shfl_xor_sync(FULL, mx, o)); }
+    const int w = threadIdx.x >> 5;
+    if (lane_id() == 0) { s_sum[w] = sum; s_max[w] = mx; }
+    __syncthreads();
+    if (threadIdx.x == 0) {
+        for (int v = 1; v < (int)(blockDim.x >> 5); ++v) { sum += s_sum[v]; mx = max(mx, s_max[v]); }
+        if (blockIdx.x == 0) stats[0] = (unsigned long long)nv;
+        atomicAdd(&stats[1], sum);
+        atomicMax(&stats[2], (unsigned long long)mx);
     }
 }
 
@@ -399,9 +427,12 @@
         long double cs = 1; for (int i = 0; i < hi; ++i) cs *= (long double)base;
         PFZ_REQUIRE(cs < 18446744073709551615.0L, "pfz_ngram_rows: alphabet %u ^ n %d exceeds 64-bit n-gram codes", base, hi);
     }
-    if (n_rows <= 0) return 0;
+    cudaStream_t st = as_stream(stream);
+    if (n_rows <= 0) {
+        if (n_rows == 0) PFZ_CUDA_OK(cudaMemsetAsync(row_cnt, 0, sizeof(int32_t), st));
+        return 0;
+    }
     const int rs = (flags & PFZ_FLAG_REMOVE_SPACE) ? 1 : 0;
-    cudaStream_t st = as_stream(stream);
     int grid = grid_for((int64_t)n_rows * 32, 256, SM_COUNT * 8);
     if (clean) ngram_rows_warp_kernel<true><<<grid, 256, 0, st>>>(blob, offsets, n_rows, lo, hi, rs, sym_table, base, occ_ptr, codes, tf, row_cnt);
     else       ngram_rows_warp_kernel<false><<<grid, 256, 0, st>>>(blob, offsets, n_rows, lo, hi, rs, sym_table, base, occ_ptr, codes, tf, row_cnt);
@@ -493,14 +524,31 @@
     return 0;
 }
 
+int pfz_fit_stats(const int32_t *df, const int32_t *n_vocab_dev, int64_t cap, const int32_t *row_cnt_a, int32_t n_a, const int32_t *row_cnt_b,
+                  int32_t n_b, int64_t *stats_dev, int64_t *stats_host, void *stream) {
+    PFZ_REQUIRE(cap >= 0 && n_a >= 0 && n_b >= 0 && (n_a == 0 || row_cnt_a) && (n_b == 0 || row_cnt_b), "pfz_fit_stats: bad arguments");
+    cudaStream_t st = as_stream(stream);
+    PFZ_CUDA_OK(cudaMemsetAsync(stats_dev, 0, 3 * sizeof(int64_t), st));
+    const int64_t n = cap > n_a ? (cap > n_b ? cap : n_b) : (n_a > n_b ? n_a : n_b);
+    fit_stats_kernel<<<grid_for(n, 256, SM_COUNT), 256, 0, st>>>(df, n_vocab_dev, cap, row_cnt_a, n_a, row_cnt_b, n_b,
+                                                                 reinterpret_cast<unsigned long long *>(stats_dev));
+    PFZ_LAUNCH_OK();
+    PFZ_CUDA_OK(cudaMemcpyAsync(stats_host, stats_dev, 3 * sizeof(int64_t), cudaMemcpyDeviceToHost, st));
+    return 0;
+}
+
 int pfz_tfidf_emit(const uint64_t *codes, const int32_t *tf, const int64_t *occ_ptr, const int32_t *row_cnt, int32_t n_rows,
-                   const int32_t *rank_dense, const uint64_t *vocab_keys, int32_t n_vocab, const double *idf, int32_t *indptr,
-                   int32_t *indices, double *data, void *ws, void *stream) {
+                   const int32_t *rank_dense, const uint64_t *vocab_keys, int32_t n_vocab, const double *idf, int32_t all_in_vocab,
+                   int32_t *indptr, int32_t *indices, double *data, void *ws, void *stream) {
     PFZ_REQUIRE(n_rows >= 0, "pfz_tfidf_emit: n_rows < 0");
     cudaStream_t st = as_stream(stream);
-    emit_count_kernel<<<grid_for((int64_t)(n_rows + 1) * 32, 256), 256, 0, st>>>(codes, occ_ptr, row_cnt, n_rows, rank_dense, vocab_keys, n_vocab, indptr);
-    PFZ_LAUNCH_OK();
-    if (scan_exclusive_i32(indptr, indptr, (int64_t)n_rows + 1, ws, st)) return 1;
+    if (all_in_vocab) {
+        if (scan_exclusive_i32(row_cnt, indptr, (int64_t)n_rows + 1, ws, st)) return 1;
+    } else {
+        emit_count_kernel<<<grid_for((int64_t)(n_rows + 1) * 32, 256), 256, 0, st>>>(codes, occ_ptr, row_cnt, n_rows, rank_dense, vocab_keys, n_vocab, indptr);
+        PFZ_LAUNCH_OK();
+        if (scan_exclusive_i32(indptr, indptr, (int64_t)n_rows + 1, ws, st)) return 1;
+    }
     if (n_rows > 0) {
         emit_write_kernel<<<grid_for((int64_t)n_rows * 32, 256), 256, 0, st>>>(codes, tf, occ_ptr, row_cnt, n_rows, rank_dense, vocab_keys, n_vocab,
                                                                                   idf, indptr, indices, data);
diff --git a/polyfuzz_b200/engine.py b/polyfuzz_b200/engine.py
--- a/polyfuzz_b200/engine.py
+++ b/polyfuzz_b200/engine.py
@@ -1,5 +1,6 @@
 import ctypes
 import os
+import threading
 
 import numpy as np
 import torch
@@ -130,6 +131,18 @@
 
 
 _IDF_TABLES = {}
+_FIT_STATS_HOST = threading.local()
+
+
+def _fit_stats_host():
+    bufs = getattr(_FIT_STATS_HOST, "bufs", None)
+    if bufs is None:
+        bufs = _FIT_STATS_HOST.bufs = {}
+    key = torch.cuda.current_device()
+    t = bufs.get(key)
+    if t is None:
+        t = bufs[key] = torch.empty(3, dtype=torch.int64).pin_memory()
+    return t
 
 
 def _idf_table(n_docs):
@@ -144,7 +157,7 @@
 
 
 class _Rows:
-    __slots__ = ("n", "occ_ptr", "codes", "tf", "row_cnt", "cap", "_keep")
+    __slots__ = ("n", "occ_ptr", "codes", "tf", "row_cnt", "cap", "in_vocab", "_keep")
 
 
 class NgramTfidf:
@@ -226,7 +239,8 @@
         R.n, R.cap, R.occ_ptr = S.n, S.cap, S.occ_ptr
         R.codes = torch.empty(max(R.cap, 1), dtype=torch.int64, device=_dev())
         R.tf = torch.empty(max(R.cap, 1), dtype=torch.int32, device=_dev())
-        R.row_cnt = torch.zeros(max(R.n, 1), dtype=torch.int32, device=_dev())
+        R.row_cnt = torch.empty(R.n + 1, dtype=torch.int32, device=_dev())
+        R.in_vocab = False
         _lib.call("pfz_ngram_rows", _p(S.d_blob), _p(S.d_off), R.n, self.lo, self.hi, self.flags, _p(d_sym),
                   int(self.base), _p(R.occ_ptr), _p(S.d_long), S.n_long, _p(R.codes), _p(R.tf), _p(R.row_cnt),
                   _stream())
@@ -271,8 +285,10 @@
         d_sym = self._sym_table()
         rows = [self._stage_a(S, d_sym, fit=True) for S in staged]
         n_docs = sum(r.n for r, c in zip(rows, counted) if c)
+        if len(rows) > 2:
+            raise ValueError("the fit takes one or two string lists")
         dev = _dev()
-        d_nv = torch.zeros(1, dtype=torch.int32, device=dev)
+        d_nv = torch.empty(1, dtype=torch.int32, device=dev)
         cs = self.code_space()
         total_cap = sum(r.cap for r in rows)
         if comm is not None:
@@ -316,16 +332,20 @@
         d_tab = _idf_table(n_docs)
         d_idf = torch.empty(d_df.numel(), dtype=torch.float64, device=dev)
         _lib.call("pfz_idf_lookup", _p(d_df), _p(d_nv), int(d_df.numel()), _p(d_tab), int(d_tab.numel()), _p(d_idf), _stream())
-        dfv = d_df.double()
-        vmask = torch.arange(d_df.numel(), device=dev) < d_nv
-        mx = torch.stack([r.row_cnt[:r.n].max() if r.n else torch.zeros((), dtype=torch.int32, device=dev) for r in rows]).max()
-        stats = torch.stack([d_nv[0].double(), torch.where(vmask, dfv * dfv, torch.zeros_like(dfv)).sum(), mx.double()]).cpu().numpy()
-        V = int(stats[0])
+        ra, rb = rows[0], (rows[1] if len(rows) > 1 else None)
+        stats_d = torch.empty(3, dtype=torch.int64, device=dev)
+        stats_h = _fit_stats_host()
+        _lib.call("pfz_fit_stats", _p(d_df), _p(d_nv), int(d_df.numel()), _p(ra.row_cnt), ra.n, _p(rb.row_cnt if rb else None),
+                  rb.n if rb else 0, _p(stats_d), _p(stats_h), _stream())
+        torch.cuda.current_stream().synchronize()
+        V, sum_df_sq, longest = (int(x) for x in stats_h.tolist())
         if V == 0:
             raise ValueError("empty vocabulary; perhaps the documents only contain stop words")
+        for r, c in zip(rows, counted):
+            r.in_vocab = bool(c)
         self._n_vocab = V
-        self._sum_df_sq = float(stats[1])
-        self.max_row_nnz = max(self.max_row_nnz, int(stats[2]))
+        self._sum_df_sq = float(sum_df_sq)
+        self.max_row_nnz = max(self.max_row_nnz, longest)
         self._h_vocab_keys = self._h_df = self._h_idf = None
         self.n_fit_docs = n_docs
         self._d_vocab = d_vocab[:V]
@@ -360,7 +380,8 @@
         data = torch.empty(max(R.cap, 1), dtype=torch.float64, device=dev)
         ws = _ws(_lib.load().pfz_scan_ws_bytes(R.n + 1))
         _lib.call("pfz_tfidf_emit", _p(R.codes), _p(R.tf), _p(R.occ_ptr), _p(R.row_cnt), R.n, _p(self._d_rank),
-                  _p(self._d_vocab), self.n_vocab, _p(self._d_idf), _p(indptr), _p(indices), _p(data), _p(ws), _stream())
+                  _p(self._d_vocab), self.n_vocab, _p(self._d_idf), int(R.in_vocab), _p(indptr), _p(indices), _p(data), _p(ws),
+                  _stream())
         return CsrMatrix(indptr, indices, data, R.n, self.n_vocab)
 
     def density(self):
@@ -385,6 +406,9 @@
 BLOCK_TILE_STEP, BLOCK_TILE_MAX = 128, 4096
 BLOCK_ROWS = int(os.environ.get("PFZ_BLOCK_ROWS", "8"))
 BLOCK_ACC_BITS = int(os.environ.get("PFZ_BLOCK_ACC_BITS", "16"))
+
+
+INDEX_BANK_ORDER, INDEX_BANK_ORDER32, INDEX_PACK_Q15, INDEX_PACK_Q26 = 1, 2, 4, 8
 
 
 class SparseIndex:
@@ -413,21 +437,26 @@
         self.post_idx = torch.empty(cap, dtype=torch.int16, device=dev)
         self.post_val = torch.empty(cap, dtype=torch.float64, device=dev)
         f32 = variant in ("dense32", "block")
-        self.post_val32 = torch.empty(cap, dtype=torch.float32, device=dev) if f32 else None
+        self.post_val32 = torch.empty(cap, dtype=torch.float32, device=dev) if variant == "dense32" else None
         self.term_maxw = torch.empty(max(self.n_vocab, 1), dtype=torch.float32, device=dev) if variant == "dense32" else None
         self.post_pk = torch.empty((cap, 2), dtype=torch.int32, device=dev) if variant in ("block", "hash") else None
         self.csr = csr
         ws = _ws((ncell + 1) * 4 + 512 + _lib.load().pfz_scan_ws_bytes(ncell + 1))
         flags = 0
         if os.environ.get("PFZ_BANK_ORDER", "1") != "0" and variant != "hash":
-            flags = 2 if f32 else 1
+            flags = INDEX_BANK_ORDER32 if f32 else INDEX_BANK_ORDER
+        if variant in ("block", "hash"):
+            flags |= INDEX_PACK_Q15 if self.acc_bits == 16 else INDEX_PACK_Q26
         _lib.call("pfz_index_build", _p(csr.indptr), _p(csr.indices), _p(csr.data), n, self.n_vocab, tile,
-                  self.n_tiles, flags, _p(self.seg), _p(self.post_idx), _p(self.post_val), _p(self.post_val32), _p(self.term_maxw), _p(ws), _stream())
-        if variant in ("block", "hash") and n > 0:
-            if self.acc_bits == 16:
-                _lib.call("pfz_index_pack_q15", _p(self.post_idx), _p(self.post_val), ctypes.c_void_p(self.seg.data_ptr() + 4 * ncell), tile, _p(self.post_pk), _stream())
-            else:
-                _lib.call("pfz_index_pack_q26", _p(self.post_idx), _p(self.post_val), ctypes.c_void_p(self.seg.data_ptr() + 4 * ncell), _p(self.post_pk), _stream())
+                  self.n_tiles, flags, _p(self.seg), _p(self.post_idx), _p(self.post_val), _p(self.post_val32), _p(self.term_maxw),
+                  _p(self.post_pk), _p(ws), _stream())
+
+    def ensure_val32(self):
+        if self.post_val32 is None:
+            self.post_val32 = torch.empty(self.post_val.numel(), dtype=torch.float32, device=self.post_val.device)
+            nnz_dev = ctypes.c_void_p(self.seg.data_ptr() + 4 * self.n_vocab * self.n_tiles)
+            _lib.call("pfz_index_val32", _p(self.post_val), nnz_dev, _p(self.post_val32), _stream())
+        return self.post_val32
 
 
 DENSE32_MAX_ROW_NNZ = 128
@@ -509,6 +538,7 @@
             index._block_err = err
             return oi, ov
         variant = "dense32"
+        index.ensure_val32()
     counter = torch.zeros(n_splits, dtype=torch.int32, device=dev)
     if variant == "hash" and index.post_pk is None:
         raise ValueError("the index was not built for the hash variant")
```
